# BoifZ/VDN-NeRF

Hardware: AMD Instinct MI355X
Metric: rays/sec (512-ray batch, 128 samples/ray) (higher is better)
Workload: dtype bf16; 1 GPU; training step of womsk_white (hierarchical sampling + render forward + backward + gradient all-reduce + Adam): SDF 8x256 + colour 4x256 + NeRF 8x256, 512 rays x (64 coarse + 64 importance + 32 outside) per GPU per step; pixels uniform over the full 800 x 800 frame; samples that enter the loss through exact zeros are skipped: 81 % of the foreground and 56 % of the background points evaluated; rays_per_gpu=512, samples_per_ray=128, outside_samples=32, parallelism=dp1, allreduce_bytes=5636348, background_points_evaluated_last_step=45590, background_points_total=81920, foreground_points_evaluated_last_step=52986, foreground_points_total=65536

## Files before the change

### include/vdn_render.h

```cpp
#ifndef VDN_RENDER_H
#define VDN_RENDER_H
#include <stdint.h>

#ifdef __cplusplus
extern "C" {
#endif

#define VDN_ABI_VERSION 28

int vdn_abi_version(void);

typedef struct {
    const float* g;
    const float* v;
    float* w_eff;
    float* inv_norm;
    int32_t rows, cols;
} VdnWeightNormDesc;
int vdn_weightnorm_materialize(const VdnWeightNormDesc* descs_dev, int n_layers, int max_rows, void* stream);

typedef struct {
    const float* src;
    const float* bias;
    const int32_t* kmap;
// ... 106 lines not shown
    const float* out_upper;
    const float* t_rand;
    const float* t_rand_out;
    float* z;
    float* z_out;
    int32_t B, n_samples, n_outside, z_ld;
} VdnCoarseArgs;
int vdn_coarse_z(const VdnCoarseArgs* args_host, void* stream);

typedef struct {
    const float* rays_o;
    const float* rays_d;
    const float* z;
    const float* sdf;
    const float* u;
    float* new_z;
    float inv_s;
    int32_t B, M, ld, n_imp;
    const float* weights;
    int32_t w_ld, _pad;
} VdnUpsampleArgs;
int vdn_upsample_round(const VdnUpsampleArgs* args_host, void* stream);

typedef struct {
    const float* z;
    const float* sdf;
    const float* new_z;
    const float* new_sdf;
    float* z_out;
    float* sdf_out;
    int32_t B, M, K, ld, ld_out;
} VdnMergeArgs;
int vdn_merge_sorted(const VdnMergeArgs* args_host, void* stream);
int vdn_merge_upsample(const VdnMergeArgs* merge_host, const VdnUpsampleArgs* upsample_host, void* stream);
int vdn_sdf_upsample_bf16(const VdnSdfArgs* sdf_host, const VdnUpsampleArgs* upsample_host, void* stream);
int vdn_sdf_merge_upsample_bf16(const VdnSdfArgs* sdf_host, const VdnMergeArgs* merge_host, const VdnUpsampleArgs* upsample_host, void* stream);

typedef struct {
    const float* z;
    float* dists;
    float* mid_z;
    float sample_dist;
    int32_t B, n, ld;
} VdnSectionArgs;
int vdn_sections(const VdnSectionArgs* args_host, void* stream);

typedef struct {
    const float* rays_o;
    const float* rays_d;
    const float* sdf;
    const float* normals;
    const float* dists;
    const float* mid_z;
    const float* color;
    const float* feat;
    const float* variance;
    const float* bg_density;
    const float* bg_rgb;
    const float* bg_feat;
    const float* bg_dists;
    const float* background_rgb;
    float cos_anneal_ratio;
    int32_t B, N, T, feat_ch;
    float* weights;
    float* alpha_out;
    float* cdf;
    float* inside_sphere;
    float* color_out;
    float* feat_out;
    float* weight_sum;
    float* weight_max;
    float* s_val;
    float* eik_partial;
    float* eik_out;
    const float* cos_anneal_dev;
} VdnCompositeArgs;
int vdn_alpha_composite_fwd(const VdnCompositeArgs* args_host, void* stream);
int vdn_feat_composite(const VdnCompositeArgs* args_host, void* stream);

int vdn_shade_fused_f32(const VdnSdfArgs* sdf_host, const VdnRenderNetArgs* color_host, const VdnCompositeArgs* comp_host,
                        int32_t* ticket, void* stream);
int vdn_sdf_color_train_bf16(const VdnSdfArgs* sdf_host, const void* color_blob, int32_t squeeze_out, void* col_h, void* col_small,
                             float* col_out, void* stream);
int vdn_shade_fused_bf16(const VdnSdfArgs* sdf_host, const void* color_blob, int32_t squeeze_out, const VdnCompositeArgs* comp_host,
                         int32_t* ticket, void* stream);
int vdn_shade_points_bf16(const VdnSdfArgs* sdf_host, const void* color_blob, int32_t squeeze_out, float* col_out, void* stream);

typedef struct {
    const float* rays_o;
    const float* rays_d;
    const float* mid_z;
    const float* normals;
    int32_t B, N;
    float* eik_partial;
    float* eik_out;
} VdnEikonalArgs;
int vdn_eikonal_terms(const VdnEikonalArgs* args_host, void* stream);


typedef struct {
    const char* blob;
    const float* g_out;
    const float* out;
    const void* save_h;
    void* delta_out;
    void* delta_h;
    void* d_feat;
    float* d_normals;
    int32_t acc_feat;
    int32_t acc_normals;
    int32_t P;
    int32_t d_out;
    int32_t squeeze_out;
    const int32_t* active_idx;
    const int32_t* n_active;
    const float* dirs; const float* rays_d;
    int32_t n_per_ray;
    int32_t acc_pts;
    float* d_pts;
    float* d_dirs;
    float* d_extra;
    const void* mask;
} VdnRenderNetBwdArgs;
int vdn_rendernet_bwd_f32(const VdnRenderNetBwdArgs* args_host, void* stream);
int vdn_rendernet_bwd_bf16(const VdnRenderNetBwdArgs* args_host, void* stream);

typedef struct {
    const char* blob;
    const float* g_density;
    const float* g_rgb;
    const float* g_feat;
    const void* save_h;
    const void* save_hv;
    void* delta_o;
    void* delta_v;
    void* delta_head;
    void* delta_h;
    int32_t P;
    const int32_t* active_idx;
    const int32_t* n_active;
    const float* rays_o; const float* rays_d; const float* z;
    int32_t n_per_ray;
    float* d_pts;
    float* d_dirs;
    const void* mask;
    const void* mask_v;
} VdnNerfBwdArgs;
int vdn_nerf_mlp_bwd_f32(const VdnNerfBwdArgs* args_host, void* stream);
int vdn_nerf_mlp_bwd_bf16(const VdnNerfBwdArgs* args_host, void* stream);
typedef struct {
    const float* pts4;
    const float* dirs;
    float* d_pts4;
    float* d_dirs;
    int32_t accumulate;
} VdnNerfInputGradArgs;
int vdn_nerf_mlp_bwd_input_f32(const VdnNerfBwdArgs* args_host, const VdnNerfInputGradArgs* in_host, void* stream);
int vdn_nerf_mlp_bwd_input_bf16(const VdnNerfBwdArgs* args_host, const VdnNerfInputGradArgs* in_host, void* stream);

typedef struct {
    const char* blob;
    const float* pts;
    const float* rays_o;
    const float* rays_d;
    const float* z;
    int32_t n_per_ray;
    int32_t z_ld;
    int32_t P;
    float scale;
    const float* g_normals;
    const void* S;
    const void* V;
    void* UB;
    void* EX;
    int32_t s_from_h;
    const int32_t* active_idx;
    const int32_t* n_active;
} VdnSdfRbarArgs;
int vdn_sdf_bwd_rbar_f32(const VdnSdfRbarArgs* args_host, void* stream);
int vdn_sdf_bwd_rbar_bf16(const VdnSdfRbarArgs* args_host, void* stream);

typedef struct {
    const char* blob;
    const float* g_sdf;
    const void* g_feat;
    const void* S;
    const void* EX;
    void* AB;
    int32_t P;
    float scale;
    int32_t s_from_h;
    const int32_t* active_idx;
    const int32_t* n_active;
    const float* pts; const float* rays_o; const float* rays_d; const float* z;
    int32_t n_per_ray, z_ld;
    const float* g_normals;
    const float* U_pe;
    int32_t acc_pts;
    float* d_pts;
} VdnSdfFbarArgs;
int vdn_sdf_bwd_fbar_f32(const VdnSdfFbarArgs* args_host, void* stream);
int vdn_sdf_bwd_fbar_bf16(const VdnSdfFbarArgs* args_host, void* stream);
int vdn_sdf_bwd_split_bf16(const VdnSdfRbarArgs* rbar_host, const VdnSdfFbarArgs* fbar_host, void* stream);


typedef struct {
    const void* A1; const void* B1;
    const void* A2; const void* B2;
    int32_t lda1, ldb1, lda2, ldb2;
    int32_t P;
    int32_t m_tiles, n_tiles;
    int32_t splits;
    int32_t wg_begin;
    int32_t _pad;
    float* slab;
    float* colsum;
    const int32_t* P_dev;
} VdnDwDesc;
int vdn_dw_gemm_f32(const VdnDwDesc* descs_dev, int n_desc, int total_wgs, void* stream);
int vdn_dw_gemm_bf16(const VdnDwDesc* descs_dev, int n_desc, int total_wgs, void* stream);
int vdn_dw_entry_wgs_f32(int m_tiles, int n_tiles, int splits);
int vdn_dw_entry_wgs_bf16(int m_tiles, int n_tiles, int splits);

typedef struct {
    const float* slab; const float* colsum;
    const int32_t* rmap; const int32_t* cmap;
    float* target; float* btarget;
    int64_t t_stride;
    int32_t splits, M, N;
    int32_t accumulate;
    float scale, bscale;
    const float* xsum;
    int32_t xsplits, xM, xrow;
    float xscale;
} VdnDwFinalizeDesc;
int vdn_dw_finalize(const VdnDwFinalizeDesc* descs_dev, int n_desc, int max_M, int phase, void* stream);

typedef struct {
    const float* g; const float* v; const float* inv_norm; const float* dw_eff;
    float* dg; float* dv;
    int32_t rows, cols;
} VdnWeightNormBwdDesc;
int vdn_weightnorm_bwd(const VdnWeightNormBwdDesc* descs_dev, int n_layers, int max_rows, void* stream);

typedef struct {
    const float* rays_o; const float* rays_d;
    const float* sdf; const float* normals; const float* dists; const float* mid_z;
    const float* color; const float* feat; const float* variance;
    const float* bg_density; const float* bg_rgb; const float* bg_feat; const float* bg_dists;
    const float* background_rgb;
    float cos_anneal_ratio;
    int32_t B, N, T, feat_ch;
    const float* alpha;
    const float* weights;
    const float* eik;
    const float* g_color;
    const float* g_feat;
    const float* g_weights;
    const float* g_eik;
    const float* g_cdf;
    float* d_sdf;
    float* d_normals;
    float* d_color;
    float* d_feat;
    float* d_bg_density;
    float* d_bg_rgb;
    float* d_bg_feat;
    float* d_var_partial;
    float* d_variance;
    float* d_dists;
    float* d_bg_dists;
    float* d_dir_cos;
    float* feat_scratch;
    const float* cos_anneal_dev;
} VdnCompositeBwdArgs;
int vdn_alpha_composite_bwd(const VdnCompositeBwdArgs* args_host, void* stream);

int vdn_composite_train(const VdnCompositeArgs* fwd_host, const VdnCompositeBwdArgs* bwd_host, const float* true_rgb, float* g_color,
                        const int32_t* fg_count, float igr_weight, float grad_scale, void* stream);
int vdn_eikonal_reduce(const float* eik_partial, int32_t B, float* eik_out, void* stream);
int vdn_composite_fwd_train(const VdnCompositeArgs* fwd_host, const float* gt_feats, float* g_feats, float depth_weight, float grad_scale, void* stream);
int vdn_composite_bwd_train(const VdnCompositeBwdArgs* bwd_host, const float* color_out, const float* true_rgb, float* g_color,
                            const int32_t* fg_count, float igr_weight, float grad_scale, void* stream);

typedef struct {
    const float* rays_d;
    const float* mid_z;
    const float* bg_mid;
    const float* d_pts;
    const float* d_dirs;
    const float* d_dists;
    const float* d_dir_cos;
    const float* d_bg_pts;
    const float* d_bg_dirs;
    const float* d_bg_dists;
    int32_t B, N, T;
    float* d_rays_o;
    float* d_rays_d;
    float* d_z;
    float* d_z_out;
} VdnRayAdjointArgs;
int vdn_ray_adjoint(const VdnRayAdjointArgs* args_host, void* stream);

typedef struct {
    const float* color;
    const float* true_rgb;
    const float* mask;
    const float* feats;
    const float* gt_feats;
    const float* weights;
    const float* eik;
    float igr_weight, mask_weight, depth_weight, grad_scale;
    int32_t B, T, C, _pad;
    float* g_color;
    float* g_feats;
    float* g_weights;
    float* g_eik;
    float* out_scalars;
} VdnLossArgs;
int vdn_loss_fwd_bwd(const VdnLossArgs* args_host, void* stream);

int vdn_adam_step(float* param, const float* grad, float* exp_avg, float* exp_avg_sq, int64_t n,
                  float lr, float beta1, float beta2, float eps, int32_t step, void* stream);
int vdn_adam_step_ranges(float* param, const float* grad, float* exp_avg, float* exp_avg_sq, int64_t begin0, int64_t end0,
                         int64_t begin1, int64_t end1, float lr, float beta1, float beta2, float eps, int32_t step, void* stream);

typedef struct {
    const float* pixels_x;
    const float* pixels_y;
    const float* intrinsic_inv;
    const float* pose;
    const float* image;
    const float* mask;
    const float* feats;
    float* out;
    float* near;
    float* far;
    int32_t B, H, W, C, mask_ch, out_ld;
} VdnGenRaysArgs;
int vdn_gen_rays(const VdnGenRaysArgs* args_host, void* stream);

typedef struct {
    const float* rays_o;
    const float* rays_d;
    const float* mid_z;
    int32_t B, N, T;
    int32_t* active_idx;
    int32_t* n_active;
    int32_t* ray_counts;
} VdnBackgroundActiveArgs;
int vdn_background_active(const VdnBackgroundActiveArgs* args_host, void* stream);

typedef struct {
    const float* rays_o;
    const float* rays_d;
    const float* mid_z;
    int32_t B, N;
    float radius;
    int32_t complement;
    int32_t* active_idx;
    int32_t* n_active;
    int32_t* ray_counts;
} VdnForegroundActiveArgs;

typedef struct {
    const float* rays_o; const float* rays_d;
    float* z;
    const float* new_z;
    int32_t M_old, _pad;
    const float* z_out;
    float* z_feed;
    int32_t B, N, T, z_ld;
    float sample_dist, fg_radius;
    float* dists; float* mid_z;
    float* bg_dists; float* bg_mid;
    int32_t* fg_active_idx; int32_t* fg_n_active; int32_t* fg_ray_counts;
    int32_t* bg_active_idx; int32_t* bg_n_active; int32_t* bg_ray_counts;
} VdnTrainPrepArgs;
int vdn_train_prep(const VdnTrainPrepArgs* args_host, void* stream);
int vdn_foreground_active(const VdnForegroundActiveArgs* args_host, void* stream);

typedef struct {
    const float* u;
    float threshold;
    int32_t R;
    int32_t* counts;
    const int64_t* offsets;
    float* tri_pos;
    int64_t* tri_key;
} VdnMeshArgs;
int vdn_mesh_count(const VdnMeshArgs* args_host, void* stream);
int vdn_mesh_emit(const VdnMeshArgs* args_host, void* stream);

typedef struct {
    const float* u;
    double isovalue;
    int32_t R;
    uint8_t* cube_case;
    int32_t* n_verts;
    int32_t* n_tris;
    const int64_t* vert_offsets;
    const int64_t* tri_offsets;
    double* vertices;
    int64_t* triangles;
} VdnMeshMcArgs;
int vdn_mesh_mc_count(const VdnMeshMcArgs* args_host, void* stream);
int vdn_mesh_mc_emit(const VdnMeshMcArgs* args_host, void* stream);

typedef struct {
    const float* X;
    const float* Y;
    const float* Z;
    const int32_t* active;
    float* points;
    int64_t first, n_points;
    int32_t R, brick, nb, A;
} VdnMeshSparseNodesArgs;
int vdn_mesh_sparse_nodes(const VdnMeshSparseNodesArgs* args_host, void* stream);

typedef struct {
    const float* values;
    double isovalue;
    int32_t R, brick, nb, A;
    const int32_t* active;
    const int32_t* brick_map;
    const int32_t* cell_base;
    const int32_t* col_cells;
    const int32_t* row_cells;
    int64_t n_cells;
    uint8_t* cube_case;
    int32_t* n_verts;
    int32_t* n_tris;
    int32_t* missed;
    const int64_t* vert_offsets;
    const int64_t* tri_offsets;
    int64_t V, F;
    double* vertices;
    int64_t* triangles;
} VdnMeshSparseArgs;
int vdn_mesh_sparse_count(const VdnMeshSparseArgs* args_host, void* stream);
int vdn_mesh_sparse_emit(const VdnMeshSparseArgs* args_host, void* stream);

typedef struct {
    const float* vertices;
    const void* triangles;
    double spacing;
    int64_t V, F, S;
    int32_t index_bytes, _pad;
    int32_t* counts;
    int32_t* error;
    const int64_t* offsets;
    float* points;
    int32_t* face;
} VdnSurfArgs;
int vdn_surf_count(const VdnSurfArgs* args_host, void* stream);
int vdn_surf_emit(const VdnSurfArgs* args_host, void* stream);

typedef struct {
    const float* pts;
    int32_t* cell;
// ... 289 lines not shown
```

### vdn-nerf_amd/csrc/k_composite_row.h

```cpp
#pragma once
#include "k_ray_rows.h"

namespace vdn {

struct CompositeGlobalSrc {
    const float* sdf_;
    const float* normals_;
    const float* color_;
    VDN_DEV float sdf(long q, int) const { return sdf_[q]; }
    VDN_DEV float normal(long q, int, int k) const { return normals_[q * 3 + k]; }
    VDN_DEV float color(long q, int, int k) const { return color_[q * 3 + k]; }
};
struct CompositeLdsSrc {
    const float* rows;
    int n;
    VDN_DEV float sdf(long, int i) const { return rows[i]; }
    VDN_DEV float normal(long, int i, int k) const { return rows[(1 + k) * n + i]; }
    VDN_DEV float color(long, int i, int k) const { return rows[(4 + k) * n + i]; }
};

struct RowOut { float num, den, c[3]; };
typedef RowOut EikPair;

template <class Src>
VDN_DEV RowOut composite_row(const CompositeArgs& a, int r, int lane, const Src& src) {
#pragma clang fp contract(off)
    const int N = a.N, T = a.T;
    const bool has_bg = a.bg_density != nullptr;
    float o[3], d[3];
    load_ray(a.rays_o, a.rays_d, r, o, d);
    float inv_s = expf(a.variance[0] * 10.0f);
    inv_s = fminf(fmaxf(inv_s, 1e-6f), 1e6f);
    const float car = a.cos_anneal_dev != nullptr ? a.cos_anneal_dev[0] : a.cos_anneal_ratio;

    float alpha[kEPL], f[kEPL], Tr[kEPL], wgt[kEPL], col[kEPL][3];
    double eik_num = 0.0, eik_den = 0.0;
#pragma unroll
    for (int e = 0; e < kEPL; ++e) {
        const int i = kEPL * lane + e;
        alpha[e] = 0.0f;
        f[e] = 1.0f;
        col[e][0] = col[e][1] = col[e][2] = 0.0f;
        if (i < T) {
            float bg_a = 0.0f;
            if (has_bg) {
                const long q = (long)r * T + i;
                bg_a = 1.0f - expf(-softplus1(a.bg_density[q]) * a.bg_dists[q]);
            }
            if (i < N) {
                const long q = (long)r * N + i;
                const float sdf = src.sdf(q, i), dist = a.dists[q];
                const float g0 = src.normal(q, i, 0), g1 = src.normal(q, i, 1), g2 = src.normal(q, i, 2);
                const float true_cos = d[0] * g0 + d[1] * g1 + d[2] * g2;
                const float iter_cos = -(fmaxf(-true_cos * 0.5f + 0.5f, 0.0f) * (1.0f - car) + fmaxf(-true_cos, 0.0f) * car);
                const float est_next = sdf + iter_cos * dist * 0.5f;
                const float est_prev = sdf - iter_cos * dist * 0.5f;
                const float prev_cdf = sigmoidf_(est_prev * inv_s);
                const float next_cdf = sigmoidf_(est_next * inv_s);
                float al = ((prev_cdf - next_cdf) + 1e-5f) / (prev_cdf + 1e-5f);
                al = fminf(fmaxf(al, 0.0f), 1.0f);
                const float pn = sample_norm(o, d, a.mid_z[q]);
                const float inside = pn < 1.0f ? 1.0f : 0.0f;
                eikonal_add(pn, g0, g1, g2, eik_num, eik_den);
                a.cdf[q] = prev_cdf;
                a.inside_sphere[q] = inside;
                float c0 = src.color(q, i, 0), c1 = src.color(q, i, 1), c2 = src.color(q, i, 2);
                if (has_bg) {
                    const long qb = (long)r * T + i;
                    al = al * inside + bg_a * (1.0f - inside);
                    c0 = c0 * inside + a.bg_rgb[qb * 3] * (1.0f - inside);
                    c1 = c1 * inside + a.bg_rgb[qb * 3 + 1] * (1.0f - inside);
                    c2 = c2 * inside + a.bg_rgb[qb * 3 + 2] * (1.0f - inside);
                }
                alpha[e] = al;
                col[e][0] = c0; col[e][1] = c1; col[e][2] = c2;
            } else {
                const long qb = (long)r * T + i;
                alpha[e] = bg_a;
                col[e][0] = a.bg_rgb[qb * 3]; col[e][1] = a.bg_rgb[qb * 3 + 1]; col[e][2] = a.bg_rgb[qb * 3 + 2];
            }
            f[e] = 1.0f - alpha[e] + 1e-7f;
        }
    }
    ray_excl_cumprod(f, Tr, lane);
    double ws = 0.0, c0 = 0.0, c1 = 0.0, c2 = 0.0;
    float wmax = 0.0f;
#pragma unroll
    for (int e = 0; e < kEPL; ++e) {
        const int i = kEPL * lane + e;
        wgt[e] = 0.0f;
        if (i < T) {
            wgt[e] = alpha[e] * Tr[e];
            a.weights[(long)r * T + i] = wgt[e];
            if (a.alpha_out != nullptr) a.alpha_out[(long)r * T + i] = alpha[e];
            ws += (double)wgt[e];
            c0 += (double)(col[e][0] * wgt[e]);
            c1 += (double)(col[e][1] * wgt[e]);
            c2 += (double)(col[e][2] * wgt[e]);
            wmax = fmaxf(wmax, wgt[e]);
        }
    }
    const float wsum = (float)wave_sum(ws);
    float cr = (float)wave_sum(c0), cg = (float)wave_sum(c1), cb = (float)wave_sum(c2);
    wmax = wave_max(wmax);
    eik_num = wave_sum(eik_num);
    eik_den = wave_sum(eik_den);
    if (a.background_rgb != nullptr) {
        cr = cr + a.background_rgb[0] * (1.0f - wsum);
        cg = cg + a.background_rgb[1] * (1.0f - wsum);
        cb = cb + a.background_rgb[2] * (1.0f - wsum);
    }
    if (lane == 0) {
        a.color_out[r * 3] = cr; a.color_out[r * 3 + 1] = cg; a.color_out[r * 3 + 2] = cb;
        a.weight_sum[r] = wsum;
        a.weight_max[r] = wmax;
        if (a.s_val != nullptr) a.s_val[r] = 1.0f / inv_s;
        if (a.eik_partial != nullptr) {
            a.eik_partial[r * 2] = (float)eik_num;
            a.eik_partial[r * 2 + 1] = (float)eik_den;
        }
    }
    return RowOut{(float)eik_num, (float)eik_den, {cr, cg, cb}};
}

struct FeatRaw { float fg[2], bg[2]; };
struct FeatPair { float f0, f1; };
template <class A>
VDN_DEV FeatRaw feat_load(const A& a, int r, int i, int ch0, int ch1) {
    const int N = a.N, T = a.T, C = a.feat_ch;
    const bool v0 = ch0 < C, v1 = ch1 < C;
    const bool fg = i < N, bg = i < T && (a.bg_density != nullptr || i >= N) && a.bg_feat != nullptr;
    const long qf = ((long)r * N + i) * C, qb = ((long)r * T + i) * C;
    FeatRaw v;
    v.fg[0] = (fg && v0) ? a.feat[qf + ch0] : 0.0f;
    v.fg[1] = (fg && v1) ? a.feat[qf + ch1] : 0.0f;
    v.bg[0] = (bg && v0) ? a.bg_feat[qb + ch0] : 0.0f;
    v.bg[1] = (bg && v1) ? a.bg_feat[qb + ch1] : 0.0f;
    return v;
}
template <class A>
VDN_DEV FeatPair feat_mix(const A& a, int i, const FeatRaw& v, float inside) {
#pragma clang fp contract(off)
    if (i >= a.N) return FeatPair{v.bg[0], v.bg[1]};
    if (a.bg_density == nullptr) return FeatPair{v.fg[0], v.fg[1]};
    return FeatPair{v.fg[0] * inside + v.bg[0] * (1.0f - inside), v.fg[1] * inside + v.bg[1] * (1.0f - inside)};
}
template <class A>
VDN_DEV FeatPair feat_pair(const A& a, int r, int i, int ch0, int ch1, float inside) {
    return feat_mix(a, i, feat_load(a, r, i, ch0, ch1), inside);
}
template <class A>
VDN_DEV void feat_group(const A& a, int r, int i0, int i_end, int ch0, int ch1, const float (&inside)[8], FeatPair (&f)[8]) {
    FeatRaw v[8];
#pragma unroll
    for (int k = 0; k < 8; ++k) v[k] = i0 + k < i_end ? feat_load(a, r, i0 + k, ch0, ch1) : FeatRaw{};
#pragma unroll
    for (int k = 0; k < 8; ++k) f[k] = i0 + k < i_end ? feat_mix(a, i0 + k, v[k], inside[k]) : FeatPair{};
}

inline int composite_fwd_check(const VdnCompositeArgs* a, bool need_alpha_out, bool need_eik_out, bool bwd_bg_ok = true) {
    if (!a || a->B <= 0 || a->N <= 0 || a->T < a->N || a->T > kMaxT) return -1;
    if (!a->rays_o || !a->rays_d || !a->sdf || !a->normals || !a->dists || !a->mid_z || !a->color || !a->variance) return -2;
    if (!a->weights || (need_alpha_out && !a->alpha_out) || !a->cdf || !a->inside_sphere || !a->color_out || !a->weight_sum ||
        !a->weight_max || !a->eik_partial || (need_eik_out && !a->eik_out)) return -3;
    if (a->T > a->N && (!a->bg_density || !a->bg_rgb || !a->bg_dists || !bwd_bg_ok)) return -4;
    return 0;
}
inline bool composite_feat_ok(const VdnCompositeArgs* a) { return a->feat && a->feat_ch > 0 && !(a->T > a->N && !a->bg_feat); }
inline int composite_bwd_check(const VdnCompositeBwdArgs* a, bool need_eik) {
    if (!a || a->B <= 0 || a->N <= 0 || a->T < a->N || a->T > kMaxT) return -1;
    if (!a->rays_o || !a->rays_d || !a->sdf || !a->normals || !a->dists || !a->mid_z || !a->color || !a->variance ||
        !a->alpha || !a->weights || (need_eik && !a->eik)) return -2;
    if (!a->d_sdf || !a->d_normals || !a->d_color || !a->d_var_partial) return -3;
    if (a->T > a->N && (!a->bg_density || !a->bg_rgb || !a->bg_dists || !a->d_bg_density || !a->d_bg_rgb)) return -4;
    if (a->d_feat && (!a->feat || a->feat_ch <= 0 || a->feat_ch > 128)) return -5;
    return 0;
}

}
```

### vdn-nerf_amd/csrc/k_ray_rows.h

```cpp
#pragma once
#include "vdn_common.h"
#include "vdn_kernels.h"

namespace vdn {

constexpr int kRayWaves = 4;
constexpr int kMaxT = 256;
constexpr int kEPL = 4;

VDN_DEV bool ray_of_wave(int B, int& wave, int& lane, int& r) {
    wave = threadIdx.x >> 6;
    lane = threadIdx.x & 63;
    r = blockIdx.x * kRayWaves + wave;
    return r < B;
}
__host__ __device__ inline int ray_blocks(int B) { return (B + kRayWaves - 1) / kRayWaves; }
template <class Kernel, class... Args>
inline void launch_ray_blocks(Kernel kernel, int n_blocks, void* stream, Args... args) {
    hipLaunchKernelGGL(kernel, dim3(n_blocks), dim3(kRayWaves * 64), 0, (hipStream_t)stream, args...);
}
template <class Kernel, class... Args>
inline void launch_rays(Kernel kernel, int B, void* stream, Args... args) {
    launch_ray_blocks(kernel, ray_blocks(B), stream, args...);
}
// ... 160 lines not shown
#pragma clang fp contract(off)
    const int M = a.M, K = a.K;
    for (int i = lane; i < M; i += 64) za[i] = old_src != nullptr ? old_src[i] : a.z[(long)r * a.ld + i];
    for (int j = lane; j < K; j += 64) zb[j] = a.new_z[(long)r * a.K + j];
    __builtin_amdgcn_wave_barrier();
    const bool has_sdf = a.sdf != nullptr;
    bool sorted_here = true;
    for (int i = lane; i + 1 < M; i += 64) sorted_here &= za[i] <= za[i + 1];
    const bool old_sorted = __all(sorted_here);
    float oz[kEPL], os[kEPL];
    int opos[kEPL];
#pragma unroll
    for (int e = 0; e < kEPL; ++e) {
        const int i = lane + 64 * e;
        opos[e] = -1;
        if (i < M) {
            const float v = za[i];
            int cnt = i;
            if (!old_sorted) {
                cnt = 0;
                for (int k = 0; k < M; ++k) cnt += (za[k] < v) | ((za[k] == v) & (k < i));
            }
            for (int j = 0; j < K; ++j) cnt += zb[j] < v;
            opos[e] = cnt;
            oz[e] = v;
            os[e] = has_sdf ? a.sdf[(long)r * a.ld + i] : 0.0f;
        }
    }
    float nz = 0.0f, ns = 0.0f;
    int npos = -1;
    if (lane < K) {
        const float v = zb[lane];
        int cnt = 0;
        if (old_sorted) {
            int lo = 0, hi = M;
            while (lo < hi) {
                const int mid = (lo + hi) >> 1;
                if (za[mid] <= v) lo = mid + 1; else hi = mid;
            }
            cnt = lo;
        } else {
            for (int k = 0; k < M; ++k) cnt += za[k] <= v;
        }
        for (int j = 0; j < K; ++j) cnt += (zb[j] < v) | ((zb[j] == v) & (j < lane));
        npos = cnt;
        nz = v;
        ns = has_sdf ? (new_sdf_src != nullptr ? new_sdf_src[lane] : a.new_sdf[(long)r * a.K + lane]) : 0.0f;
    }
    __builtin_amdgcn_wave_barrier();
#pragma unroll
    for (int e = 0; e < kEPL; ++e) {
        if (opos[e] >= 0) {
            a.z_out[(long)r * a.ld_out + opos[e]] = oz[e];
            if (has_sdf) a.sdf_out[(long)r * a.ld_out + opos[e]] = os[e];
            if (lz != nullptr) { lz[opos[e]] = oz[e]; ls[opos[e]] = os[e]; }
        }
    }
    if (npos >= 0) {
        a.z_out[(long)r * a.ld_out + npos] = nz;
        if (has_sdf) a.sdf_out[(long)r * a.ld_out + npos] = ns;
        if (lz != nullptr) { lz[npos] = nz; ls[npos] = ns; }
    }
}

struct Section { float dist, mid; };
VDN_DEV Section section(const float* z, int i, int n, float sample_dist) {
#pragma clang fp contract(off)
    const float z0 = z[i];
    const float dist = (i + 1 < n) ? z[i + 1] - z0 : sample_dist;
    return Section{dist, z0 + dist * 0.5f};
}

struct ActiveJob {
    const float* rays_o;
    const float* rays_d;
    const float* mid_z;
    int B, N, T;
    float radius;
    bool background;
    bool complement;
    int32_t* active_idx;
    int32_t* n_active;
    int32_t* ray_counts;
};

VDN_DEV bool sample_active(const ActiveJob& a, int r, int s, const float (&o)[3], const float (&d)[3]) {
    if (s >= a.N) return true;
    const float pn = sample_norm(o, d, a.mid_z[(long)r * a.N + s]);
    return a.background ? !(pn < 1.0f) : (pn < a.radius) != a.complement;
}

template <bool FILL>
VDN_DEV void active_list_row(const ActiveJob& a, int r, int lane, const float (&o)[3], const float (&d)[3]) {
    int base = 0;
    if (FILL) {
        int acc = 0;
        for (int i = lane; i < r; i += 64) acc += a.ray_counts[i];
        base = (int)wave_sum((double)acc);
    }
    int n = 0;
    for (int s0 = 0; s0 < a.T; s0 += 64) {
        const int s = s0 + lane;
        const bool act = s < a.T && sample_active(a, r, s, o, d);
        const unsigned long long m = __ballot(act);
        if (FILL && act) a.active_idx[base + n + __popcll(m & ((1ull << lane) - 1ull))] = r * a.T + s;
        n += __popcll(m);
    }
    if (lane == 0) {
        if (!FILL) a.ray_counts[r] = n;
        else if (r == a.B - 1) a.n_active[0] = base + n;
    }
}

}
```

### vdn-nerf_amd/csrc/k_render_bwd.h

```cpp
#pragma once
#include <type_traits>
#include "mlp_engine.h"
#include "vdn_kernels.h"

namespace vdn {

template <class P, int NT_OUT, int EX = 0, bool MASK = false>
__global__ __launch_bounds__(P::kWaves * 64, P::kMinWavesPerEU) void rendernet_bwd_kernel(RenderNetBwdArgs a) {
    using ST = typename P::store_t;
    constexpr int kSlot = P::stride(8);
    extern __shared__ __attribute__((aligned(16))) char smem[];
    WStream<P::kWaves, kSlot> ws;
    ws.init(a.blob, smem, 42 + EX);
    const int lane = ws.lane, c = lane & 31, h = lane >> 5;
    const WorkRow wr = work_row(a.active_idx, a.n_active, a.P, P::kWaves, ws.wave, c);
    if (wr.none) return;
    ws.warm_issue(wr.n_wg, 256 * P::kMinWavesPerEU);
    warm_code_issue((std::is_same<P, BF16>::value) ? kWarmCodeRenderBwd : 0, wr.n_wg, 256 * P::kMinWavesPerEU, ws.warm_dump());
    const bool ok = wr.ok;
    const long p = wr.row, pd = wr.point;
    const long PS = P::plane(a.P, 256);
    const ST* save_h = reinterpret_cast<const ST*>(a.save_h);
    ST* delta_h = reinterpret_cast<ST*>(a.delta_h);
    ST* delta_out = reinterpret_cast<ST*>(a.delta_out);
    ST* d_feat = reinterpret_cast<ST*>(a.d_feat);
    unsigned mk[MASK ? 16 : 1];
    if constexpr (MASK) {
        const unsigned char* m = static_cast<const unsigned char*>(a.mask);
        const long MS = BF16::mask_plane(a.P, 256);
#pragma unroll
        for (int l = 0; l < 4; ++l) BF16::load_mask<4>(m + l * MS, p, h, mk + 4 * l);
    }

    typename P::template Act<8> X, Y;
    if constexpr (NT_OUT == 1) {
        float dl[4];
#pragma unroll
        for (int j = 0; j < 4; ++j) {
            dl[j] = 0.0f;
            if (j < a.d_out) {
                const float o = a.out[pd * a.d_out + j], g = a.g_out[pd * a.d_out + j];
                dl[j] = a.squeeze_out ? g * o * (1.0f - o) : (o > 0.0f ? g : 0.0f);
            }
        }
        const f32x16 t16 = vals_tile<4>(dl, h, 0);
        X.set(0, t16);
        P::store_tile(delta_out, p, 32, 0, h, t16, ok);
    } else {
#pragma unroll
        for (int kt = 0; kt < 3; ++kt) {
            const f32x16 o = F32::load_tile(a.out, pd, 96, kt, h);
            const f32x16 g = F32::load_tile(a.g_out, pd, 96, kt, h);
            f32x16 dl;
#pragma unroll
            for (int t = 0; t < 16; ++t) dl[t] = a.squeeze_out ? g[t] * o[t] * (1.0f - o[t]) : (o[t] > 0.0f ? g[t] : 0.0f);
            X.set(kt, dl);
            P::store_tile(delta_out, p, 96, kt, h, dl, ok);
        }
    }
    auto ldH = [&](int l) VDN_INL { return [=](int nt) VDN_INL { return P::load_tile(save_h + l * PS, p, 256, nt, h); }; };
    auto mask_store = [&](auto& D, int l) VDN_INL {
        return [&D, l, delta_h, PS, p, ok, h](int nt, const f32x16& acc, const f32x16& hv) VDN_INL {
            f32x16 o;
#pragma unroll
            for (int t = 0; t < 16; ++t) o[t] = hv[t] > 0.0f ? acc[t] : 0.0f;
            D.set(nt, o);
            P::store_tile(delta_h + l * PS, p, 256, nt, h, o, ok);
        };
    };
    auto bit_store = [&](auto& D, int l) VDN_INL {
        return [&D, &mk, l, delta_h, PS, p, ok, h](int nt, const f32x16& acc, int) VDN_INL {
            const f32x16 o = BF16::mask_select(mk + 4 * l, nt, acc);
            D.set(nt, o);
            P::store_tile(delta_h + l * PS, p, 256, nt, h, o, ok);
        };
    };
    ws.all_issue = __any(ok);
    if constexpr (MASK) BF16::mask_landed(mk);
    warm_l2_wait();
    ws.start();
    if constexpr (MASK) {
        dense<P, NT_OUT, 8, false>(ws, X, 0, NoPre{}, bit_store(Y, 3), P::kTileOps);
        dense<P, 8, 8, false>(ws, Y, 0, NoPre{}, bit_store(X, 2), P::kTileOps);
        dense<P, 8, 8, false>(ws, X, 0, NoPre{}, bit_store(Y, 1), P::kTileOps);
        dense<P, 8, 8, false>(ws, Y, 0, NoPre{}, bit_store(X, 0), P::kTileOps);
    } else {
        dense<P, NT_OUT, 8, false, kBwdPrefetch>(ws, X, 0, ldH(3), mask_store(Y, 3), P::kTileOps, P::kTileOps);
        dense<P, 8, 8, false, kBwdPrefetch>(ws, Y, 0, ldH(2), mask_store(X, 2), P::kTileOps, P::kTileOps);
        dense<P, 8, 8, false, kBwdPrefetch>(ws, X, 0, ldH(1), mask_store(Y, 1), P::kTileOps, P::kTileOps);
        dense<P, 8, 8, false, kBwdPrefetch>(ws, Y, 0, ldH(0), mask_store(X, 0), P::kTileOps, P::kTileOps);
    }
    f32x16 SM[2];
    dense<P, 8, 10 + EX, false>(ws, X, 0, NoPre{}, [&](int nt, const f32x16& acc, int) VDN_INL {
        if (nt >= 10) {
            if constexpr (EX > 0) {
                f32x16 o = F32::load_tile(a.d_extra, pd, 32 * EX, nt - 10, h);
#pragma unroll
                for (int t = 0; t < 16; ++t) o[t] += acc[t];
                F32::store_tile(a.d_extra, pd, 32 * EX, nt - 10, h, o, ok);
            }
        } else if (nt < 8) {
            f32x16 o = acc;
            if (a.acc_feat) {
                const f32x16 prev = P::load_tile(d_feat, p, 256, nt, h);
#pragma unroll
                for (int t = 0; t < 16; ++t) o[t] += prev[t];
            }
            P::store_tile(d_feat, p, 256, nt, h, o, ok);
        } else {
            SM[nt - 8] = acc;
        }
    });
    float small[33];
    tiles_vals<33, 2>(SM, h, small);
    if (ok && h == 0) {
#pragma unroll
        for (int d = 0; d < 3; ++d) {
            const float prev = a.acc_normals ? a.d_normals[pd * 3 + d] : 0.0f;
            a.d_normals[pd * 3 + d] = prev + small[30 + d];
        }
        if (a.d_pts != nullptr) {
            const long r = pd / a.n_per_ray;
#pragma unroll
            for (int d = 0; d < 3; ++d) {
                const float dir = a.dirs ? a.dirs[pd * 3 + d] : a.rays_d[r * 3 + d];
                float g = small[3 + d];
#pragma unroll
                for (int k = 0; k < 4; ++k) {
                    const float f = (float)(1 << k);
                    float sn, co;
                    sincos_pe<P::kAccurateTrig>(dir * f, sn, co);
                    g += f * (co * small[3 + 3 + 6 * k + d] - sn * small[3 + 3 + 6 * k + 3 + d]);
                }
                const float pp = a.acc_pts ? a.d_pts[pd * 3 + d] : 0.0f;
                const float pg = a.acc_pts ? a.d_dirs[pd * 3 + d] : 0.0f;
                a.d_pts[pd * 3 + d] = pp + small[d];
                a.d_dirs[pd * 3 + d] = pg + g;
            }
        }
    }
}

template <class P>
int launch_rendernet_bwd(const VdnRenderNetBwdArgs* args, void* stream_) {
    hipStream_t stream = (hipStream_t)stream_;
    if (!args || args->P <= 0 || !args->blob || !args->g_out || !args->out || !args->save_h || !args->delta_out ||
        !args->delta_h || !args->d_feat || !args->d_normals) return -1;
    if (!(args->d_out == 96 || (args->d_out >= 1 && args->d_out <= 4))) return -2;
    if (args->d_pts && (!args->d_dirs || (!args->dirs && (!args->rays_d || args->n_per_ray <= 0)))) return -3;
    const int ppw = P::kWaves * 32;
    const int grid = (args->P + ppw - 1) / ppw;
    const size_t lds = 3 * P::stride(8);
    if (args->mask != nullptr) {
        if constexpr (std::is_same<P, BF16>::value) {
            static bool once_m = (allow_big_lds(rendernet_bwd_kernel<P, 1, 0, true>, lds), allow_big_lds(rendernet_bwd_kernel<P, 3, 0, true>, lds),
                                  allow_big_lds(rendernet_bwd_kernel<P, 1, 3, true>, lds), true);
            (void)once_m;
            if (args->d_extra != nullptr) {
                if (args->d_out == 96) return -4;
                hipLaunchKernelGGL((rendernet_bwd_kernel<P, 1, 3, true>), dim3(grid), dim3(P::kWaves * 64), lds, stream, *args);
            } else if (args->d_out == 96) {
                hipLaunchKernelGGL((rendernet_bwd_kernel<P, 3, 0, true>), dim3(grid), dim3(P::kWaves * 64), lds, stream, *args);
            } else {
                hipLaunchKernelGGL((rendernet_bwd_kernel<P, 1, 0, true>), dim3(grid), dim3(P::kWaves * 64), lds, stream, *args);
            }
            return (int)hipGetLastError();
        } else {
            return -5;
        }
    }
    static bool once = (allow_big_lds(rendernet_bwd_kernel<P, 1>, lds), allow_big_lds(rendernet_bwd_kernel<P, 3>, lds),
                        allow_big_lds(rendernet_bwd_kernel<P, 1, 3>, lds), true);
    (void)once;
    if (args->d_extra != nullptr) {
        if (args->d_out == 96) return -4;
        hipLaunchKernelGGL((rendernet_bwd_kernel<P, 1, 3>), dim3(grid), dim3(P::kWaves * 64), lds, stream, *args);
        return (int)hipGetLastError();
    }
    if (args->d_out == 96)
        hipLaunchKernelGGL((rendernet_bwd_kernel<P, 3>), dim3(grid), dim3(P::kWaves * 64), lds, stream, *args);
    else
        hipLaunchKernelGGL((rendernet_bwd_kernel<P, 1>), dim3(grid), dim3(P::kWaves * 64), lds, stream, *args);
    return (int)hipGetLastError();
}

}
```

### vdn-nerf_amd/csrc/k_sdf_fwd2.h

```cpp
#pragma once
#include <cstdlib>
#include "k_ray_rows.h"
#include "k_composite_row.h"
#include "chunk_stream.h"
#include "vdn_kernels.h"

namespace vdn {
namespace sdf2 {

#ifndef VDN_SDF2_PRE
#define VDN_SDF2_PRE 4
#endif
#ifndef VDN_SDF2_GROUP
#define VDN_SDF2_GROUP 2
#endif
#ifndef VDN_SDF2_ABL
#define VDN_SDF2_ABL 0
#endif
#ifndef VDN_SDF2_S16
#define VDN_SDF2_S16 0
#endif
constexpr bool kS16 = VDN_SDF2_S16 != 0;
#ifndef VDN_SDF2_B2
#define VDN_SDF2_B2 2
// ... 108 lines not shown
    using PG = Prog<MODE>;
    using Acc = AccT;
    static constexpr int total = PG::total, kPre = sdf2::kPre, kGroup = sdf2::kGroup, abl = VDN_SDF2_ABL;
    static constexpr int kt(int c) { return PG::kt_of(c); }
    static constexpr bool bias(int c) { return PG::bias_of(c); }
    static constexpr bool b2(int c) { return VDN_SDF2_B2 != 0 && NSLOT >= DEPTH + 2 && (VDN_SDF2_B2 != 2 || c < PG::first_chunk(PG::NL < 9 ? PG::NL : 9)); }
    static constexpr bool certifies(int c) { return !b2(c) || c % 2 == 0; }
    static constexpr int wait(int c) { return b2(c) ? wait_count_b2<MODE, SAVE>(c) : wait_count<MODE, SAVE, DEPTH>(c); }
    static constexpr bool dma_burst(int c) { return sdf2::dma_burst<MODE, SAVE>(c); }
};

#ifndef VDN_SDF2_SP
#define VDN_SDF2_SP 1
#endif
struct SpE { float g, e; };
VDN_DEV SpE softplus_sigma(float t) {
    SpE r;
#if VDN_SDF2_ABL & 1
    r.g = t; r.e = t;
    return r;
#endif
#if VDN_SDF2_SP == 1
    const float w = 1.0f + __builtin_amdgcn_exp2f(t);
    r.g = __builtin_amdgcn_fmed3f(__builtin_amdgcn_logf(w), t, 25.0f);
    r.e = __builtin_amdgcn_rcpf(w);
#else
    const float e = __builtin_amdgcn_exp2f(-fabsf(t));
    r.g = relu0(t) + __builtin_amdgcn_logf(1.0f + e);
    r.e = __builtin_amdgcn_exp2f(-r.g);
#endif
    return r;
}
typedef unsigned u32x4 __attribute__((ext_vector_type(4)));

#ifndef VDN_SDF2_WT_SAVES
#define VDN_SDF2_WT_SAVES 1
#endif
VDN_DEV void plane_store16(unsigned short* p, const u32x4& v) {
#if VDN_SDF2_WT_SAVES
#if VDN_SAVE_NT
    asm volatile("global_store_dwordx4 %0, %1, off sc1 nt\n\ts_nop 1" ::"v"(p), "v"(v) : "memory");
#else
    asm volatile("global_store_dwordx4 %0, %1, off sc1\n\ts_nop 1" ::"v"(p), "v"(v) : "memory");
#endif
#else
    *reinterpret_cast<u32x4*>(p) = v;
#endif
}

VDN_DEV unsigned sigma255_pack(float e0, float e1, float e2, float e3) {
    const unsigned d0 = __builtin_bit_cast(unsigned, __builtin_amdgcn_cvt_pknorm_u16(e0, e1));
    const unsigned d1 = __builtin_bit_cast(unsigned, __builtin_amdgcn_cvt_pknorm_u16(e2, e3));
    return ~__builtin_amdgcn_perm(d1, d0, 0x07050301u);
}
VDN_DEV float ubyte_f32(unsigned w, int b) { return (float)((w >> (8 * b)) & 0xffu); }

template <int NLDS>
struct SStore {
    static constexpr int NREG = kSTiles > NLDS ? (kSTiles - NLDS) : 0;
    u32x4 reg[NREG > 0 ? NREG : 1];
    char* lds;
    template <int T>
    VDN_DEV void put(const u32x4& v) {
        if constexpr (T < NLDS) *reinterpret_cast<u32x4*>(lds + T * 1024) = v;
        else reg[T - NLDS] = v;
    }
    template <int T>
    VDN_DEV u32x4 get() const {
        if constexpr (T < NLDS) return *reinterpret_cast<const u32x4*>(lds + T * 1024);
        else return reg[T - NLDS];
    }
};

constexpr int pair_begin(int gi, int GA) { return gi >= GA ? 8 : gi * 8 / GA; }

struct ShadeExtra {
    const char* color_blob;
    int* ticket;
    int squeeze_out;
    int warm_bytes, warm_bytes2;
    void* col_h;
    void* col_small;
    float* col_out;
    CompositeArgs cm;
};

template <int MODE, bool SAVE, int NSLOT, int DEPTH, int VID = 0, bool UPS = false>
__global__ __launch_bounds__(kWaves * 64, MODE == 0 ? 2 : 1) void sdf_fwd2_kernel(SdfArgs a, UpsampleArgs up, ShadeExtra ex) {
    static_assert(!UPS || MODE == 0, "the up-sampling round follows the sdf-only pass");
    using PG = Prog<MODE>;
    static_assert(MODE != 3 || SAVE, "MODE 3 is the training forward");
    constexpr bool TS = SAVE && (MODE == 1 || MODE == 3);
    constexpr bool FEAT = MODE == 1 || MODE == 3 || (MODE == 2 && SAVE);
    constexpr bool COL = MODE >= 2;
    using P = BF16;
    using ST = unsigned short;
    constexpr int kRing = NSLOT * kStride;
    constexpr int kW8 = 0;
    constexpr int kLdsTotal = MODE >= 1 ? 160 * 1024 : kRing + kW8;
    constexpr int NLDS = MODE >= 1 ? ((kLdsTotal - kRing - kW8) / (kWaves * 1024) < kSTiles ? (kLdsTotal - kRing - kW8) / (kWaves * 1024) : kSTiles) : 0;
    extern __shared__ __attribute__((aligned(16))) char smem[];
    using PL = StepPolicy<MODE, SAVE, NSLOT, DEPTH>;
    cstream::Pipe<kWaves, kStride, NSLOT, DEPTH, MODE >= 2 ? PG::sdf_total : cstream::kNoSplit, kPre> pp;
    pp.init(a.blob, smem, ex.color_blob);
    const int lane = pp.lane, c = lane & 31, h = lane >> 5;
    const WorkRow wr = work_row(a.active_idx, a.n_active, a.P, kWaves, pp.wave, c);
    if (wr.none) return;
    if constexpr (MODE == 1) {
        if (a.tail_max_rows > 0) {
            const long n_rows = a.active_idx != nullptr ? (long)*a.n_active : (long)a.P;
            if (n_rows > a.tail_row0 && n_rows - a.tail_row0 <= a.tail_max_rows && (long)blockIdx.x * (kWaves * 32) >= a.tail_row0) return;
        }
    }
#ifdef VDN_SDF2_STAMP
    const unsigned long long stamp_c0 = __builtin_amdgcn_s_memtime(), stamp_r0 = __builtin_amdgcn_s_memrealtime();
    unsigned long long stamp_p1 = 0, stamp_p2 = 0;
#endif
    const bool ok = wr.ok;
    const long p = wr.row, pd = wr.point;
    const int c16 = lane & 15, q4 = lane >> 4;
    (void)c16; (void)q4;

    float xin[3];
    float px[3] = {0.0f, 0.0f, 0.0f}, dir[3] = {0.0f, 0.0f, 0.0f};
    long sdf_idx = pd;
    float z_keep = 0.0f, sdf_keep = 0.0f;
    if (a.pts != nullptr) {
#pragma unroll
        for (int d = 0; d < 3; ++d) xin[d] = a.pts[pd * 3 + d] * a.scale;
        if constexpr (MODE == 4) {
#pragma unroll
            for (int d = 0; d < 3; ++d) px[d] = a.pts[pd * 3 + d];
        }
    } else {
        const long r = pd / a.n_per_ray;
        const long sidx = pd - r * a.n_per_ray;
        const float z = a.z[r * a.z_ld + sidx];
        z_keep = z;
        sdf_idx = r * a.sdf_ld + sidx;
#pragma unroll
        for (int d = 0; d < 3; ++d) xin[d] = (a.rays_o[r * 3 + d] + a.rays_d[r * 3 + d] * z) * a.scale;
        if constexpr (COL) {
#pragma unroll
            for (int d = 0; d < 3; ++d) {
                dir[d] = a.rays_d[r * 3 + d];
                px[d] = a.rays_o[r * 3 + d] + a.rays_d[r * 3 + d] * z;
            }
        }
    }
    ST* Hs = reinterpret_cast<ST*>(a.H);
    ST* Vs = reinterpret_cast<ST*>(a.V);
    ST* feat = reinterpret_cast<ST*>(a.feat);
    const long PS = P::plane(a.P, 256);
    const long prow = (p >> 5) * (32L * 256) + h * 256 + (p & 31) * 8;
    long prow2[2] = {0, 0};
    if constexpr (kS16) {
        const long n_rows = a.active_idx != nullptr ? (long)*a.n_active : (long)a.P;
#pragma unroll
        for (int ph = 0; ph < 2; ++ph) {
            const long raw = ((long)blockIdx.x * kWaves + pp.wave) * 32 + 16 * ph + c16;
            const long r = raw < n_rows ? raw : (n_rows > 0 ? n_rows - 1 : 0);
            prow2[ph] = (r >> 5) * (32L * 256) + (q4 >> 1) * 512 + (q4 & 1) * 256 + (r & 31) * 8;
        }
    }
    auto piece = [&](int T, int k) VDN_INL -> long { return kS16 ? prow2[k] + T * 1024 : prow + T * 1024 + 512 * k; };
    const float inv_scale = 1.0f / a.scale;
    asm volatile("s_waitcnt vmcnt(0)" ::: "memory");
    char* const wdump = pp.warm_dump();
    warm_l2_issue(a.blob, ex.warm_bytes, wr.n_wg, MODE == 0 ? 512 : 256, wdump);
    warm_l2_issue(COL ? ex.color_blob : nullptr, COL ? ex.warm_bytes2 : 0, wr.n_wg, 256, wdump);
    constexpr int kCode = MODE == 0 ? kWarmCodeSdfFwd2Mode0 : (MODE == 1 ? (SAVE ? kWarmCodeSdfFwd2Save : kWarmCodeSdfFwd2) : (MODE == 3 ? kWarmCodeSdfFwd3 : 0));
    warm_code_issue(ex.warm_bytes > 0 ? kCode : 0, wr.n_wg, MODE == 0 ? 512 : 256, wdump);

    typename P::template Act<9> X, Y;
    typename P::template Act<9> F;
    float nz = 0.0f;
    float col[3] = {0.0f, 0.0f, 0.0f};
    SStore<NLDS> SS;
    SS.lds = smem + kRing + kW8 + pp.wave * (NLDS * 1024) + lane * 16;
    static_assert(!kS16 || MODE == 0 || NLDS * 1024 >= 32 * 272, "exchange scratch");
    static_assert(!kS16 || NSLOT - 1 >= DEPTH, "the last ring slot is free at the start");
    char* const xch = MODE >= 1 ? smem + kRing + kW8 + pp.wave * (NLDS * 1024) : smem + (NSLOT - 1) * kStride + pp.wave * 4096;
    auto to_tile_lanes = [&](bf16x8* fr, auto nf_c) VDN_INL {
        constexpr int NF = decltype(nf_c)::value;
#pragma unroll
        for (int s = 0; s < NF; ++s) *reinterpret_cast<bf16x8*>(xch + s * 1024 + lane * 16) = fr[s];
        asm volatile("s_waitcnt lgkmcnt(0)" ::: "memory");
#pragma unroll
        for (int s = 0; s < NF; ++s)
            fr[s] = *reinterpret_cast<const bf16x8*>(xch + ((s & ~1) + (q4 >> 1)) * 1024 + (q4 & 1) * 512 + (16 * (s & 1) + c16) * 16);
        asm volatile("s_waitcnt lgkmcnt(0)" ::: "memory");
    };

    bf16x8 pe7[2];
    {
        float pe39[39], pe[64];
        posenc<3, 6, false>(xin, pe39);
#pragma unroll
        for (int i = 0; i < 39; ++i) pe[i] = pe39[i] * kC1;
#pragma unroll
        for (int i = 0; i < 25; ++i) pe[39 + i] = fmaf(pe39[i], kC1, -bf16_lo(pack_bf16x2(pe[i], 0.0f)));
#pragma unroll
// ... 114 lines not shown
                                u32x4 o;
                                o[0] = fhold0;
                                o[1] = fhold1;
                                o[2] = pack_bf16x2(acc_prev[4 * q], acc_prev[4 * q + 1]);
                                o[3] = pack_bf16x2(acc_prev[4 * q + 2], acc_prev[4 * q + 3]);
                                if constexpr (FEAT) plane_store16(feat + piece(T, q >> 1), o);
                                if constexpr (COL) F.r[T * 2 + (q >> 1)] = __builtin_bit_cast(bf16x8, o);
                            }
                            const f32x4 w = *(reinterpret_cast<const f32x4*>(pp.template slot<CP + 1>() + kTail) + (8 * T + quad_of(q, lane)));
                            if constexpr (q == 0) sq_v7 = SS.template get<PG::s_tile0(7) + T>();
                            const unsigned sw = sq_v7[q];
                            const float v0 = w[0] * inv_scale * ubyte_f32(sw, 0), v1 = w[1] * inv_scale * ubyte_f32(sw, 1);
                            const float v2 = w[2] * inv_scale * ubyte_f32(sw, 2), v3 = w[3] * inv_scale * ubyte_f32(sw, 3);
                            u32x4 cur = __builtin_bit_cast(u32x4, Y.r[T * 2 + (q >> 1)]);
                            unsigned k0 = pack_bf16x2(v0, v1), k1 = pack_bf16x2(v2, v3);
                            asm volatile("" : "+v"(k0), "+v"(k1));
                            cur[2 * (q & 1)] = k0;
                            cur[2 * (q & 1) + 1] = k1;
                            Y.r[T * 2 + (q >> 1)] = __builtin_bit_cast(bf16x8, cur);
                            if constexpr (TS) {
                                if constexpr ((q & 1) == 0) {
                                    vhold0 = pack_bf16x2(v0 * kVSave, v1 * kVSave);
                                    vhold1 = pack_bf16x2(v2 * kVSave, v3 * kVSave);
                                    asm volatile("" : "+v"(vhold0), "+v"(vhold1));
                                } else {
                                    u32x4 ov;
                                    ov[0] = vhold0;
                                    ov[1] = vhold1;
                                    ov[2] = pack_bf16x2(v0 * kVSave, v1 * kVSave);
                                    ov[3] = pack_bf16x2(v2 * kVSave, v3 * kVSave);
                                    plane_store16(Vs + 7 * PS + piece(T, q >> 1), ov);
                                }
                            }
                        }
                    });
                }
            } else if constexpr (L.kind == SWEEP || (L.kind == SWEEP_SKIP && T < 7)) {
                static_for<PE_ - PB>([&](auto i_c) VDN_INL {
                    constexpr int pr = PB + decltype(i_c)::value;
                    const float v0 = acc_prev[2 * pr] * ubyte_f32(sq_prev[pr >> 1], 2 * (pr & 1));
                    const float v1 = acc_prev[2 * pr + 1] * ubyte_f32(sq_prev[pr >> 1], 2 * (pr & 1) + 1);
                    unsigned pk = pack_bf16x2(v0, v1);
                    asm volatile("" : "+v"(pk));
                    u32x4 cur = __builtin_bit_cast(u32x4, D.r[T * 2 + (pr >> 2)]);
                    cur[pr & 3] = pk;
                    D.r[T * 2 + (pr >> 2)] = __builtin_bit_cast(bf16x8, cur);
                    if constexpr (TS) {
                        unsigned pv = pack_bf16x2(v0 * kVSave, v1 * kVSave);
                        if constexpr ((pr & 3) == 0) {
                            vhold0 = pv;
                            asm volatile("" : "+v"(vhold0));
                        } else if constexpr ((pr & 3) == 1) {
                            vhold1 = pv;
                            asm volatile("" : "+v"(vhold1));
                        } else if constexpr ((pr & 3) == 2) {
                            hold0 = pv;
                            asm volatile("" : "+v"(hold0));
                        } else {
                            u32x4 o;
                            o[0] = vhold0;
                            o[1] = vhold1;
                            o[2] = hold0;
                            o[3] = pv;
                            plane_store16(Vs + L.l * PS + piece(T, pr >> 2), o);
                        }
                    }
                });
            } else if constexpr (L.kind == COL0 || L.kind == COLH) {
                static_for<PE_ - PB>([&](auto i_c) VDN_INL {
                    constexpr int pr = PB + decltype(i_c)::value;
                    float a0 = acc_prev[2 * pr], a1 = acc_prev[2 * pr + 1];
                    if constexpr (L.kind == COL0) {
                        if constexpr ((pr & 1) == 0) w8hold = *(reinterpret_cast<const f32x4*>(pp.template slot<CP + 1>() + kTail) + (8 * T + quad_of(pr >> 1, lane)));
                        const float nzp = kS16 ? nz2[ph_of_pair(pr)] : nz;
                        a0 = fmaf(w8hold[2 * (pr & 1)], nzp, a0);
                        a1 = fmaf(w8hold[2 * (pr & 1) + 1], nzp, a1);
                    }
                    unsigned pk = pack_bf16x2(relu0(a0), relu0(a1));
                    asm volatile("" : "+v"(pk));
                    u32x4 cur = __builtin_bit_cast(u32x4, D.r[T * 2 + (pr >> 2)]);
                    cur[pr & 3] = pk;
                    D.r[T * 2 + (pr >> 2)] = __builtin_bit_cast(bf16x8, cur);
                    if constexpr (MODE == 3 && (pr & 3) == 3)
                        plane_store16(reinterpret_cast<ST*>(ex.col_h) + L.l * PS + piece(T, pr >> 2), cur);
                });
            } else if constexpr (L.kind == COLOUT) {
                if constexpr (PB == 0) {
                    if constexpr (kS16) {
#pragma unroll
                        for (int j = 0; j < 3; ++j) {
                            const float lo = acc_prev[j], hi = __shfl(acc_prev[8 + j], lane & 15);
                            const float x = (lane & 16) ? hi : lo;
                            col[j] = ex.squeeze_out ? sigmoidf_(x) : relu0(x);
                        }
                    } else {
#pragma unroll
                        for (int j = 0; j < 3; ++j) col[j] = ex.squeeze_out ? sigmoidf_(acc_prev[j]) : relu0(acc_prev[j]);
                    }
                }
            }
        }
    };

    static_for<PG::total + 1>([&](auto c_c) VDN_INL {
        constexpr int C = decltype(c_c)::value;
        constexpr int CP = C - 1;
        constexpr int CPs = CP >= 0 ? CP : 0;
        if constexpr (C < PG::total) {
            constexpr int LI = PG::layer_of(C), T = PG::tile_of(C);
            constexpr LayerDesc L = PG::layer(LI);
            constexpr int NS = 2 * L.kt, NG = (NS + kGroup - 1) / kGroup;
#ifdef VDN_SDF2_STAMP
            if constexpr (C == PG::first_chunk(8)) stamp_p1 = __builtin_amdgcn_s_memtime();
            if constexpr (MODE == 1 && C == PG::first_chunk(MODE == 1 ? 9 : 8)) stamp_p2 = __builtin_amdgcn_s_memtime();
#endif
            constexpr bool boundary = CP >= 0 && PG::layer_of(CPs) != LI;
            constexpr int KP = PG::layer(PG::layer_of(CPs)).kind;
            constexpr bool prev_writes_input = boundary && (KP == HID || KP == SWEEP || KP == COL0 || KP == COLH);
            constexpr int GA = prev_writes_input ? ((2 * PG::tile_of(CPs)) / kGroup < NG ? (2 * PG::tile_of(CPs)) / kGroup : NG) : NG;
            static_assert(GA >= 1, "a pending tile needs at least one MFMA group before its reader");
            if constexpr (L.kind == HID && L.l == 4 && T == 0) { X.r[14] = pe7[0]; X.r[15] = pe7[1]; }
            constexpr bool sweep_tile = L.kind == SWEEP || (L.kind == SWEEP_SKIP && T < 7);
            u32x4 sq_next;
            if constexpr (sweep_tile) sq_next = SS.template get<PG::s_tile0(L.l) + T>();
            const auto& Xin = L.kind == COL0 ? F : ((LI & 1) ? Y : X);
            const AccT acc_cur = cstream::chunk_step<PL, C>(pp, Xin, [&](auto g_c, auto) VDN_INL {
                constexpr int gi = decltype(g_c)::value;
                epilogue(std::integral_constant<int, CP>{}, std::integral_constant<int, pair_begin(gi, GA)>{},
                         std::integral_constant<int, pair_begin(gi + 1, GA)>{});
            });
            if constexpr (L.kind == SWEEP_SKIP && T >= 7) UPE[T - 7] = acc_cur;
            if constexpr (L.kind == SWEEP_PE) {
                if constexpr (kS16) UPE[T].add(acc_cur);
                else UPE[T] = acc_cur;
            }
            if constexpr (L.kind == LAST && T == L.nt - 1) {
                const float b0 = *reinterpret_cast<const float*>(pp.template slot<C>() + L.kt * 2048);
                float dot;
                if constexpr (kS16) {
                    float d0 = sdf_dot[0], d1 = sdf_dot[1];
                    d0 += __shfl_xor(d0, 16); d1 += __shfl_xor(d1, 16);
                    d0 += __shfl_xor(d0, 32); d1 += __shfl_xor(d1, 32);
                    dot = (lane & 16) ? d1 : d0;
                } else {
                    dot = sdf_dot[0] + __shfl_xor(sdf_dot[0], 32);
                }
                sdf_keep = fmaf(dot, 1.0f / kC1, b0) * inv_scale;
                if (ok && h == 0) a.sdf[sdf_idx] = sdf_keep;
            }
            acc_prev = acc_cur;
            if constexpr (sweep_tile) sq_prev = sq_next;
            if constexpr ((!kS16 && L.kind == SWEEP_SKIP && T == 8) || (L.kind == SWEEP_PE && T == 1)) pe_backward(kS16 || L.kind == SWEEP_SKIP);
            if constexpr (COL && L.kind == SWEEP_PE && T == 1) {
                float small[32], pe[27];
                if constexpr (MODE == 4) {
                    const float gx = n[0] * a.scale, gy = n[1] * a.scale, gz = n[2] * a.scale;
                    const float inv = -1.0f / fmaxf(sqrtf(gx * gx + gy * gy + gz * gz), 1e-12f);
                    dir[0] = gx * inv;
                    dir[1] = gy * inv;
                    dir[2] = gz * inv;
                }
                posenc<3, 4, P::kAccurateTrig>(dir, pe);
#pragma unroll
                for (int d = 0; d < 3; ++d) small[d] = px[d];
#pragma unroll
                for (int i = 0; i < 27; ++i) small[3 + i] = pe[i];
                small[30] = n[0] * a.scale;
                small[31] = n[1] * a.scale;
                nz = n[2] * a.scale;
                F.set(8, vals_tile<32>(small, h, 0));
                if constexpr (kS16) {
                    to_tile_lanes(&F.r[16], std::integral_constant<int, 2>{});
                    reinterpret_cast<float*>(xch)[c] = nz;
                    asm volatile("s_waitcnt lgkmcnt(0)" ::: "memory");
                    nz2[0] = reinterpret_cast<const float*>(xch)[c16];
                    nz2[1] = reinterpret_cast<const float*>(xch)[16 + c16];
                    asm volatile("s_waitcnt lgkmcnt(0)" ::: "memory");
                }
                if constexpr (MODE == 3) {
                    float s33[33];
#pragma unroll
                    for (int i = 0; i < 32; ++i) s33[i] = small[i];
                    s33[32] = nz;
#pragma unroll
                    for (int kt = 0; kt < 2; ++kt) P::store_tile(reinterpret_cast<ST*>(ex.col_small), p, 64, kt, h, vals_tile<33>(s33, h, kt), true);
                }
            }
        } else {
            epilogue(std::integral_constant<int, CP>{}, std::integral_constant<int, 0>{}, std::integral_constant<int, 8>{});
        }
        __builtin_amdgcn_sched_barrier(0);
    });
    if constexpr (MODE >= 1) {
        if (ok && h == 0) {
#pragma unroll
            for (int d = 0; d < 3; ++d) a.normals[pd * 3 + d] = n[d] * a.scale;
            if constexpr (MODE == 3 || MODE == 4) {
#pragma unroll
                for (int d = 0; d < 3; ++d) ex.col_out[pd * 3 + d] = col[d];
            }
        }
    }
    if constexpr (MODE == 2) {
        asm volatile("s_waitcnt lgkmcnt(0)" ::: "memory");
        __builtin_amdgcn_s_barrier();
        float* rows = reinterpret_cast<float*>(smem);
        if (h == 0) {
            const int i = pp.wave * 32 + c;
            rows[i] = sdf_keep;
#pragma unroll
            for (int d = 0; d < 3; ++d) {
                rows[(1 + d) * 128 + i] = n[d] * a.scale;
                rows[(4 + d) * 128 + i] = col[d];
            }
        }
        asm volatile("s_waitcnt lgkmcnt(0)" ::: "memory");
        __builtin_amdgcn_s_barrier();
        if (pp.wave != 0) return;
        const int ray = blockIdx.x;
        CompositeArgs cm = ex.cm;
        float* eik_partial = cm.eik_partial;
        cm.eik_partial = nullptr;
        const EikPair ep = composite_row(cm, ray, lane, CompositeLdsSrc{rows, 128});
        int old = 0;
        if (lane == 0) {
            typedef float f32x2 __attribute__((ext_vector_type(2)));
            const f32x2 pv = {ep.num, ep.den};
            asm volatile("global_store_dwordx2 %0, %1, off sc1\n\ts_waitcnt vmcnt(0)" ::"v"(eik_partial + 2 * ray), "v"(pv) : "memory");
            old = __hip_atomic_fetch_add(ex.ticket, 1, __ATOMIC_RELAXED, __HIP_MEMORY_SCOPE_AGENT);
        }
        old = __builtin_amdgcn_readfirstlane(old);
        if (old == cm.B - 1) {
            double sn = 0.0, sd = 0.0;
            for (int i = lane; i < cm.B; i += 64) {
                typedef float f32x2 __attribute__((ext_vector_type(2)));
                f32x2 v;
                asm volatile("global_load_dwordx2 %0, %1, off sc1\n\ts_waitcnt vmcnt(0)" : "=v"(v) : "v"(eik_partial + 2 * i) : "memory");
                sn += (double)v[0];
                sd += (double)v[1];
            }
            sn = wave_sum(sn);
            sd = wave_sum(sd);
            if (lane == 0) {
                cm.eik_out[0] = (float)sn / ((float)sd + 1e-5f);
                cm.eik_out[1] = (float)sn;
                cm.eik_out[2] = (float)sd;
                __hip_atomic_store(ex.ticket, 0, __ATOMIC_RELAXED, __HIP_MEMORY_SCOPE_AGENT);
            }
        }
    }
    if constexpr (UPS) {
        asm volatile("s_waitcnt lgkmcnt(0)" ::: "memory");
        __builtin_amdgcn_s_barrier();
        float* rows = reinterpret_cast<float*>(smem) + (pp.wave >> 1) * 3 * kMaxT;
        if (h == 0) {
            rows[(pp.wave & 1) * 32 + c] = z_keep;
            rows[kMaxT + (pp.wave & 1) * 32 + c] = sdf_keep;
        }
        asm volatile("s_waitcnt lgkmcnt(0)" ::: "memory");
        __builtin_amdgcn_s_barrier();
        const int r = blockIdx.x * 2 + (pp.wave >> 1);
        if ((pp.wave & 1) == 0 && r < up.B) upsample_row(up, r, lane, 64, rows, rows + kMaxT, rows + 2 * kMaxT);
    }
#ifdef VDN_SDF2_STAMP
    if (threadIdx.x == 0 && a.PE != nullptr) {
        unsigned long long* o = reinterpret_cast<unsigned long long*>(a.PE) + 8 * blockIdx.x;
        o[0] = stamp_c0; o[1] = __builtin_amdgcn_s_memtime(); o[2] = stamp_r0; o[3] = __builtin_amdgcn_s_memrealtime();
        o[4] = stamp_p1; o[5] = stamp_p2;
    }
#endif
}

template <int MODE, bool SAVE, int NSLOT, int DEPTH, int VID = 0, bool UPS = false>
int launch(const VdnSdfArgs* args, hipStream_t stream, const VdnUpsampleArgs* up = nullptr, const ShadeExtra* ex = nullptr) {
    constexpr size_t lds_min = MODE >= 1 ? 160 * 1024 : NSLOT * kStride;
    static bool once = (allow_big_lds(sdf_fwd2_kernel<MODE, SAVE, NSLOT, DEPTH, VID, UPS>, lds_min), true);
    (void)once;
    const int grid = (args->P + kWaves * 32 - 1) / (kWaves * 32);
    const size_t lds = lds_min;
    static const bool warm = [] { const char* e = getenv("VDN_SDF2_WARM"); return e == nullptr || e[0] != '0'; }();
    ShadeExtra exv = ex != nullptr ? *ex : ShadeExtra{};
    const bool cold = (SAVE && (MODE == 1 || MODE == 3)) || args->cold_start != 0;
// ... 10 lines not shown
```

### vdn-nerf_amd/csrc/rays.hip

```cpp
#include "k_ray_rows.h"
#include "k_composite_row.h"
#include "k_pixel_gather.h"
#include "k_loss_grad.h"

namespace vdn {

__global__ void coarse_z_kernel(CoarseArgs a) {
    const int idx = blockIdx.x * blockDim.x + threadIdx.x;
    const int per = a.n_samples + a.n_outside;
    if (idx >= a.B * per) return;
    const int r = idx / per, j = idx % per;
    const float nearv = a.near[r], farv = a.far[r];
    if (j < a.n_samples) {
        float z = nearv + (farv - nearv) * a.lin_samples[j];
        if (a.t_rand != nullptr) z = z + (a.t_rand[r] - 0.5f) * 2.0f / (float)a.n_samples;
        a.z[(long)r * a.z_ld + j] = z;
    } else {
        const int k = j - a.n_samples;
        const int kk = a.n_outside - 1 - k;
        float zo;
        if (a.t_rand_out != nullptr)
            zo = a.out_lower[kk] + (a.out_upper[kk] - a.out_lower[kk]) * a.t_rand_out[(long)r * a.n_outside + kk];
        else
            zo = a.lin_outside[kk];
// ... 156 lines not shown
#pragma unroll
    for (int r = 0; r < 3; ++r) v[r] = p[r] / nrm;
#pragma unroll
    for (int r = 0; r < 3; ++r) d[r] = a.pose[r * 4 + 0] * v[0] + a.pose[r * 4 + 1] * v[1] + a.pose[r * 4 + 2] * v[2];
    float* o = a.out + (long)i * a.out_ld;
    float org[3];
#pragma unroll
    for (int r = 0; r < 3; ++r) {
        org[r] = a.pose[r * 4 + 3];
        o[r] = org[r];
        o[3 + r] = d[r];
    }
    gather_pixel_row(a, x, y, o);
    if (a.near != nullptr && a.far != nullptr) {
        const float mid = sphere_mid(org, d);
        a.near[i] = mid - 1.0f;
        a.far[i] = mid + 1.0f;
    }
}

}

using namespace vdn;

extern "C" int vdn_gen_rays(const VdnGenRaysArgs* a, void* stream) {
    if (!a || a->B <= 0 || !a->pixels_x || !a->pixels_y || !a->intrinsic_inv || !a->pose || !a->out) return -1;
    if (a->out_ld < 6 || a->H <= 0 || a->W <= 0) return -2;
    if (a->feats && (a->C <= 0 || a->out_ld < 10 + a->C)) return -3;
    if (a->mask && a->mask_ch <= 0) return -4;
    hipLaunchKernelGGL(gen_rays_kernel, dim3((a->B + 255) / 256), dim3(256), 0, (hipStream_t)stream, *a);
    return (int)hipGetLastError();
}

extern "C" int vdn_coarse_z(const VdnCoarseArgs* a, void* stream) {
    if (!a || a->B <= 0 || !a->near || !a->far || !a->z || !a->lin_samples) return -1;
    if (a->n_outside > 0 && (!a->z_out || !a->lin_outside)) return -2;
    if (a->t_rand_out && (!a->out_lower || !a->out_upper)) return -3;
    const int n = a->B * (a->n_samples + a->n_outside);
    hipLaunchKernelGGL(coarse_z_kernel, dim3((n + 255) / 256), dim3(256), 0, (hipStream_t)stream, *a);
    return (int)hipGetLastError();
}

extern "C" int vdn_upsample_round(const VdnUpsampleArgs* a, void* stream) {
    if (!a || a->B <= 0 || !a->z || !a->new_z || !a->u) return -1;
    if (a->weights == nullptr ? (!a->sdf || !a->rays_o || !a->rays_d) : a->w_ld < a->M - 1) return -1;
    if (a->M < 2 || a->M > kMaxT || a->n_imp < 1 || a->n_imp > 64 || a->ld < a->M) return -2;
    launch_rays(upsample_kernel, a->B, stream, *a);
    return (int)hipGetLastError();
}

extern "C" int vdn_merge_sorted(const VdnMergeArgs* a, void* stream) {
    if (!a || a->B <= 0 || !a->z || !a->new_z || !a->z_out) return -1;
    if (a->M < 1 || a->K < 1 || a->K > 64 || a->M + a->K > kMaxT || a->ld < a->M || a->ld_out < a->M + a->K) return -2;
    if (a->sdf && (!a->new_sdf || !a->sdf_out)) return -3;
    launch_rays(merge_kernel, a->B, stream, *a);
    return (int)hipGetLastError();
}

template <bool FILL>
__global__ __launch_bounds__(kRayWaves * 64) void active_list_kernel(ActiveJob a) {
    int wave, lane, r;
    if (!ray_of_wave(a.B, wave, lane, r)) return;
    float o[3], d[3];
    load_ray(a.rays_o, a.rays_d, r, o, d);
    active_list_row<FILL>(a, r, lane, o, d);
}

static int launch_active(const ActiveJob& j, void* stream) {
    launch_rays(active_list_kernel<false>, j.B, stream, j);
    launch_rays(active_list_kernel<true>, j.B, stream, j);
    return (int)hipGetLastError();
}

extern "C" int vdn_background_active(const VdnBackgroundActiveArgs* a, void* stream) {
    if (!a || a->B <= 0 || a->N < 0 || a->T < a->N || !a->rays_o || !a->rays_d || (a->N > 0 && !a->mid_z) ||
        !a->active_idx || !a->n_active || !a->ray_counts) return -1;
    const ActiveJob j = {a->rays_o, a->rays_d, a->mid_z, a->B, a->N, a->T, 1.0f, true, false, a->active_idx, a->n_active, a->ray_counts};
    return launch_active(j, stream);
}

extern "C" int vdn_foreground_active(const VdnForegroundActiveArgs* a, void* stream) {
    if (!a || a->B <= 0 || a->N <= 0 || !a->rays_o || !a->rays_d || !a->mid_z || !(a->radius > 0.0f) ||
        !a->active_idx || !a->n_active || !a->ray_counts) return -1;
    const ActiveJob j = {a->rays_o, a->rays_d, a->mid_z, a->B, a->N, a->N, a->radius, false, a->complement != 0, a->active_idx, a->n_active, a->ray_counts};
    return launch_active(j, stream);
}

template <int PASS>
__global__ __launch_bounds__(kRayWaves * 64) void train_prep_kernel(TrainPrepArgs a) {
    const int wave = threadIdx.x >> 6, lane = threadIdx.x & 63;
    const int nb = ray_blocks(a.B);
    const bool second = PASS == 1 && (int)blockIdx.x >= nb;
    const int r = ((int)blockIdx.x - (second ? nb : 0)) * kRayWaves + wave;
    if (r >= a.B) return;
    float o[3], d[3];
    load_ray(a.rays_o, a.rays_d, r, o, d);
    if (PASS == 0) {
        __shared__ float s_a[kRayWaves][kMaxT], s_b[kRayWaves][kMaxT], s_f[kRayWaves][kMaxT], s_x[kRayWaves][kMaxT], s_z[kRayWaves][kMaxT];
        const float* final_z = nullptr;
        if (a.new_z != nullptr) {
            MergeArgs m1 = {};
            m1.z = a.z; m1.new_z = a.new_z; m1.z_out = a.z;
            m1.B = a.B; m1.M = a.M_old; m1.K = a.N - a.M_old; m1.ld = a.z_ld; m1.ld_out = a.z_ld;
            merge_row(m1, r, lane, s_a[wave], s_b[wave], s_z[wave], s_x[wave]);
            __builtin_amdgcn_wave_barrier();
            final_z = s_z[wave];
        }
        MergeArgs m = {};
        m.z = a.z; m.new_z = a.z_out; m.z_out = a.z_feed;
        m.B = a.B; m.M = a.N; m.K = a.T - a.N; m.ld = a.z_ld; m.ld_out = a.T;
        merge_row(m, r, lane, s_a[wave], s_b[wave], s_f[wave], s_x[wave], final_z);
        __builtin_amdgcn_wave_barrier();
        const float* zi = s_a[wave];
        const float* zf = s_f[wave];
        for (int i = lane; i < a.N; i += 64) {
            const Section sc = section(zi, i, a.N, a.sample_dist);
            a.dists[(long)r * a.N + i] = sc.dist;
            a.mid_z[(long)r * a.N + i] = sc.mid;
        }
        for (int i = lane; i < a.T; i += 64) {
            const Section sc = section(zf, i, a.T, a.sample_dist);
            a.bg_dists[(long)r * a.T + i] = sc.dist;
            a.bg_mid[(long)r * a.T + i] = sc.mid;
        }
        __builtin_amdgcn_s_waitcnt(0);
        __builtin_amdgcn_wave_barrier();
    }
    if (a.fg_active_idx != nullptr && !second)
        active_list_row<PASS == 1>(ActiveJob{a.rays_o, a.rays_d, a.mid_z, a.B, a.N, a.N, a.fg_radius, false, false, a.fg_active_idx, a.fg_n_active, a.fg_ray_counts},
                                   r, lane, o, d);
    if (PASS == 0 || second)
        active_list_row<PASS == 1>(ActiveJob{a.rays_o, a.rays_d, a.mid_z, a.B, a.N, a.T, 1.0f, true, false, a.bg_active_idx, a.bg_n_active, a.bg_ray_counts},
                                   r, lane, o, d);
}

extern "C" int vdn_train_prep(const VdnTrainPrepArgs* a, void* stream) {
    if (!a || a->B <= 0 || a->N <= 0 || a->T <= a->N || a->T > kMaxT || a->z_ld < a->N) return -1;
    if (!a->rays_o || !a->rays_d || !a->z || !a->z_out || !a->z_feed || !a->dists || !a->mid_z || !a->bg_dists || !a->bg_mid) return -2;
    if (a->T - a->N > 64) return -2;
    if (a->new_z && (a->M_old < 1 || a->M_old >= a->N || a->N - a->M_old > 64)) return -2;
    if (!a->bg_active_idx || !a->bg_n_active || !a->bg_ray_counts) return -3;
    if (a->fg_active_idx && (!a->fg_n_active || !a->fg_ray_counts || !(a->fg_radius > 0.0f))) return -4;
    launch_rays(train_prep_kernel<0>, a->B, stream, *a);
    launch_ray_blocks(train_prep_kernel<1>, 2 * ray_blocks(a->B), stream, *a);
    return (int)hipGetLastError();
}

extern "C" int vdn_merge_upsample(const VdnMergeArgs* m, const VdnUpsampleArgs* u, void* stream) {
    if (!m || !u || m->B <= 0 || !m->z || !m->new_z || !m->z_out || !m->sdf || !m->new_sdf || !m->sdf_out) return -1;
    if (m->M < 1 || m->K < 1 || m->K > 64 || m->M + m->K > kMaxT || m->ld < m->M || m->ld_out < m->M + m->K) return -2;
    if (u->B != m->B || u->M != m->M + m->K || u->weights || !u->rays_o || !u->rays_d || !u->u || !u->new_z ||
        u->n_imp < 1 || u->n_imp > 64) return -3;
    launch_rays(merge_upsample_kernel, m->B, stream, *m, *u);
    return (int)hipGetLastError();
}

extern "C" int vdn_sections(const VdnSectionArgs* a, void* stream) {
    if (!a || a->B <= 0 || a->n <= 0 || !a->z || !a->dists || !a->mid_z || a->ld < a->n) return -1;
    const int n = a->B * a->n;
    hipLaunchKernelGGL(sections_kernel, dim3((n + 255) / 256), dim3(256), 0, (hipStream_t)stream, *a);
    return (int)hipGetLastError();
}

extern "C" int vdn_eikonal_terms(const VdnEikonalArgs* a, void* stream) {
    if (!a || a->B <= 0 || a->N <= 0 || a->N > kMaxT) return -1;
    if (!a->rays_o || !a->rays_d || !a->mid_z || !a->normals || !a->eik_partial || !a->eik_out) return -2;
    launch_rays(eikonal_terms_kernel, a->B, stream, *a);
    hipLaunchKernelGGL(eikonal_reduce_kernel, dim3(1), dim3(64), 0, (hipStream_t)stream, a->eik_partial, a->B, a->eik_out);
    return (int)hipGetLastError();
}

extern "C" int vdn_eikonal_reduce(const float* eik_partial, int32_t B, float* eik_out, void* stream) {
    if (!eik_partial || !eik_out || B <= 0) return -1;
    hipLaunchKernelGGL(eikonal_reduce_kernel, dim3(1), dim3(64), 0, (hipStream_t)stream, eik_partial, B, eik_out);
    return (int)hipGetLastError();
}

extern "C" int vdn_feat_composite(const VdnCompositeArgs* a, void* stream) {
    if (!a || a->B <= 0 || a->N <= 0 || a->T < a->N || a->T > kMaxT) return -1;
    if (!a->feat || !a->feat_out || a->feat_ch <= 0 || !a->weights || !a->inside_sphere) return -2;
    if (a->T > a->N && (!a->bg_density || !a->bg_feat)) return -3;
    hipLaunchKernelGGL(feat_composite_kernel, dim3(a->B), dim3(256), 0, (hipStream_t)stream, *a, FeatLoss{});
    return (int)hipGetLastError();
}

extern "C" int vdn_composite_fwd_train(const VdnCompositeArgs* a, const float* gt_feats, float* g_feats, float depth_weight, float grad_scale,
                                       void* stream) {
    if (!gt_feats || !g_feats) return -1;
    if (const int err = composite_fwd_check(a, false, false)) return err;
    if (!a->feat_out || !composite_feat_ok(a)) return -5;
    launch_rays(composite_kernel, a->B, stream, *a);
    hipLaunchKernelGGL(feat_composite_kernel, dim3(a->B), dim3(256), 0, (hipStream_t)stream, *a, FeatLoss{gt_feats, g_feats, depth_weight, grad_scale});
    return (int)hipGetLastError();
}

extern "C" int vdn_alpha_composite_fwd(const VdnCompositeArgs* a, void* stream) {
    if (const int err = composite_fwd_check(a, false, true)) return err;
    if (a->feat_out && !composite_feat_ok(a)) return -5;
    launch_rays(composite_kernel, a->B, stream, *a);
    if (a->feat_out != nullptr)
        hipLaunchKernelGGL(feat_composite_kernel, dim3(a->B), dim3(256), 0, (hipStream_t)stream, *a, FeatLoss{});
    hipLaunchKernelGGL(eikonal_reduce_kernel, dim3(1), dim3(64), 0, (hipStream_t)stream, a->eik_partial, a->B, a->eik_out);
    return (int)hipGetLastError();
}
```

### vdn-nerf_amd/csrc/train_dw_bf16.hip

```cpp
#include "mlp_engine.h"
#include "vdn_kernels.h"

namespace vdn {

constexpr int kDwTileBytes = 2048;
constexpr int kDwStageBytes = 16 * kDwTileBytes;
#ifndef VDN_DW_BUF
#define VDN_DW_BUF 4
#endif
constexpr int kDwBuf = VDN_DW_BUF;
constexpr int kDwWaves = 8;

typedef short s16x4 __attribute__((ext_vector_type(4)));
typedef __attribute__((address_space(3))) char lds_char;
typedef __attribute__((address_space(3))) s16x4 lds_s16x4;

VDN_DEV const char* dw_uniform(const char* p) {
    const unsigned long long v = (unsigned long long)p;
    const unsigned lo = __builtin_amdgcn_readfirstlane((unsigned)v), hi = __builtin_amdgcn_readfirstlane((unsigned)(v >> 32));
    return (const char*)(((unsigned long long)hi << 32) | lo);
}

VDN_DEV void dw_glds16(const char* base_uniform, unsigned lane_off, unsigned lds_wave_base) {
#if VDN_DW_LD_NT == 2
    asm volatile("s_mov_b32 m0, %1\n\ts_nop 0\n\tglobal_load_lds_dwordx4 %0, %2 sc1 nt" ::"v"(lane_off), "s"(lds_wave_base), "s"(base_uniform) : "memory", "m0");
#elif VDN_DW_LD_NT
    asm volatile("s_mov_b32 m0, %1\n\ts_nop 0\n\tglobal_load_lds_dwordx4 %0, %2 nt" ::"v"(lane_off), "s"(lds_wave_base), "s"(base_uniform) : "memory", "m0");
#else
    asm volatile("s_mov_b32 m0, %1\n\ts_nop 0\n\tglobal_load_lds_dwordx4 %0, %2" ::"v"(lane_off), "s"(lds_wave_base), "s"(base_uniform) : "memory", "m0");
#endif
}

VDN_DEV void dw_wait_vm(int n) {
    switch (n) {
        case 0: asm volatile("s_waitcnt vmcnt(0)" ::: "memory"); break;
        case 1: asm volatile("s_waitcnt vmcnt(1)" ::: "memory"); break;
        case 2: asm volatile("s_waitcnt vmcnt(2)" ::: "memory"); break;
        case 3: asm volatile("s_waitcnt vmcnt(3)" ::: "memory"); break;
        case 4: asm volatile("s_waitcnt vmcnt(4)" ::: "memory"); break;
        case 6: asm volatile("s_waitcnt vmcnt(6)" ::: "memory"); break;
        case 8: asm volatile("s_waitcnt vmcnt(8)" ::: "memory"); break;
        case 9: asm volatile("s_waitcnt vmcnt(9)" ::: "memory"); break;
        case 12: asm volatile("s_waitcnt vmcnt(12)" ::: "memory"); break;
        default: asm volatile("s_waitcnt vmcnt(0)" ::: "memory"); break;
    }
}

VDN_DEV bf16x8 dw_frag(const lds_char* p) {
    const s16x4 lo = __builtin_amdgcn_ds_read_tr16_b64_v4i16((lds_s16x4*)(p));
    const s16x4 hi = __builtin_amdgcn_ds_read_tr16_b64_v4i16((lds_s16x4*)(p + 256));
    return bf16x8{lo[0], lo[1], lo[2], lo[3], hi[0], hi[1], hi[2], hi[3]};
}

VDN_DEV int dw_uni(int v) { return __builtin_amdgcn_readfirstlane(v); }

__global__ __launch_bounds__(512, 1) void dw_gemm_bf16_kernel(const DwDesc* descs, int n_desc) {
    extern __shared__ __attribute__((aligned(16))) char smem[];
    const int wg = blockIdx.x;
    int di = 0;
    while (di + 1 < n_desc && descs[di + 1].wg_begin <= wg) ++di;
    const DwDesc& d = descs[dw_uni(di)];
    const int m_tiles = dw_uni(d.m_tiles), n_tiles = dw_uni(d.n_tiles), splits = dw_uni(d.splits);
    const int local = wg - dw_uni(d.wg_begin);
    const int mg = (m_tiles + 7) / 8, ng = max((n_tiles + 7) / 8, 1);
    const int split = local / (mg * ng), blk = local % (mg * ng);
    if (split >= splits) return;
    const int tm = blk / ng, tn = blk % ng;
    const int wave = dw_uni(threadIdx.x >> 6), lane = threadIdx.x & 63, c = lane & 31, h = lane >> 5;
    const int wm = wave >> 1, wn = wave & 1;
    const int a_t0 = tm * 8, b_t0 = tn * 8;
    const int nA = min(8, m_tiles - a_t0), nB = max(0, min(8, n_tiles - b_t0));
    const bool two = d.A2 != nullptr;
    const int seg_splits = two ? splits / 2 : splits;
    const bool seg2 = two && split >= seg_splits;
    const int s_in = seg2 ? split - seg_splits : split;
    int P = dw_uni(d.P);
    if (d.P_dev != nullptr) P = min(P, dw_uni(*d.P_dev));
    int per = (P + seg_splits - 1) / seg_splits;
    per = (per + 127) / 128 * 128;
    const int k_begin = s_in * per, k_end = min(k_begin + per, P);
    const char* A = dw_uniform(reinterpret_cast<const char*>(seg2 ? d.A2 : d.A1));
    const char* Bm = dw_uniform(reinterpret_cast<const char*>(seg2 ? d.B2 : d.B1));
    const long lda = dw_uni(seg2 ? d.lda2 : d.lda1), ldb = dw_uni(seg2 ? d.ldb2 : d.ldb1);
    const int n_stages = k_end > k_begin ? (k_end - k_begin + 31) >> 5 : 0;
    float* slab = d.slab;
    float* colsum = d.colsum;

    const int n_pieces = 2 * (nA + nB);
    const int npw = (n_pieces - wave + kDwWaves - 1) / kDwWaves;
    const unsigned lane_off = ((lane >> 3) & 1) * 1024 + ((lane >> 2) & 1) * 512 + ((lane >> 4) * 4 + (lane & 3)) * 16;
    const unsigned lds0 = (unsigned)(size_t)(lds_char*)smem;
    auto issue_stage = [&](int s) VDN_INL {
        const long blk32 = (k_begin >> 5) + s;
        const unsigned buf = lds0 + (s % kDwBuf) * kDwStageBytes;
#pragma unroll
        for (int i = 0; i < 4; ++i) {
            const int u = wave + i * kDwWaves;
            if (u < n_pieces) {
                const int t = u >> 1, half = u & 1;
                const bool isA = t < nA;
                const char* src = isA ? A + blk32 * (64 * lda) + (long)(a_t0 + t) * 2048
                                      : Bm + blk32 * (64 * ldb) + (long)(b_t0 + t - nA) * 2048;
                const int slot = isA ? t : 8 + (t - nA);
                dw_glds16(src + half * 256, lane_off, buf + slot * kDwTileBytes + half * 1024);
            }
        }
    };

    const int gi = lane & 15, qp = gi >> 2, pp = gi & 3, jj = (lane >> 4) & 1;
    const unsigned frag_off = (2 * h) * 256 + (jj * 8 + (pp & 1) * 4 + qp) * 16 + (pp >> 1) * 8;
    const lds_char* lbase = (lds_char*)smem + frag_off;

    f32x16 acc[2][4];
    f32x16 cs[2];
#pragma unroll
    for (int i = 0; i < 2; ++i) {
        cs[i] = f32x16{0};
#pragma unroll
        for (int j = 0; j < 4; ++j) acc[i][j] = f32x16{0};
    }
    const bool do_colsum = colsum != nullptr && tn == 0 && wn == 0 && !seg2;
    const int mvm = (2 * wm < nA ? 1 : 0) | (2 * wm + 1 < nA ? 2 : 0);
    const int nvm = (4 * wn < nB ? 1 : 0) | (4 * wn + 1 < nB ? 2 : 0) | (4 * wn + 2 < nB ? 4 : 0) | (4 * wn + 3 < nB ? 8 : 0);
    const bf16x8 ones = {0x3F80, 0x3F80, 0x3F80, 0x3F80, 0x3F80, 0x3F80, 0x3F80, 0x3F80};

    auto run = [&](auto full_c) VDN_INL {
        constexpr bool FULL = decltype(full_c)::value;
#pragma unroll
        for (int s = 0; s < kDwBuf - 1; ++s)
            if (s < n_stages) issue_stage(s);
        for (int s = 0; s < n_stages; ++s) {
            const int later = min(n_stages - 1 - s, kDwBuf - 2);
            dw_wait_vm(npw * later);
            asm volatile("s_barrier" ::: "memory");
            if (s + kDwBuf - 1 < n_stages) issue_stage(s + kDwBuf - 1);
            if (s == n_stages - 1 && (k_end & 31)) {
                const int valid = k_end & 31;
                char* buf = smem + (s % kDwBuf) * kDwStageBytes;
                for (int u = threadIdx.x; u < 16 * 256; u += 512) {
                    const int pt = ((u >> 5) & 7) * 4 + ((u >> 1) & 3);
                    if (pt >= valid) *reinterpret_cast<unsigned long long*>(buf + u * 8) = 0ull;
                }
                __syncthreads();
            }
            const lds_char* st = lbase + (s % kDwBuf) * kDwStageBytes;
#pragma unroll
            for (int ks = 0; ks < 2; ++ks) {
                bf16x8 a[2], b[4];
#pragma unroll
                for (int i = 0; i < 2; ++i)
                    if (FULL || (mvm >> i & 1)) a[i] = dw_frag(st + (2 * wm + i) * kDwTileBytes + ks * 1024);
#pragma unroll
                for (int j = 0; j < 4; ++j)
                    if (FULL || (nvm >> j & 1)) b[j] = dw_frag(st + (8 + 4 * wn + j) * kDwTileBytes + ks * 1024);
#pragma unroll
                for (int i = 0; i < 2; ++i) {
                    if (!FULL && !(mvm >> i & 1)) continue;
#pragma unroll
                    for (int j = 0; j < 4; ++j)
                        if (FULL || (nvm >> j & 1)) acc[i][j] = __builtin_amdgcn_mfma_f32_32x32x16_bf16(a[i], b[j], acc[i][j], 0, 0, 0);
                    if (do_colsum) cs[i] = __builtin_amdgcn_mfma_f32_32x32x16_bf16(a[i], ones, cs[i], 0, 0, 0);
                }
            }
        }
    };
    if (mvm == 3 && nvm == 15) run(std::true_type{});
    else run(std::false_type{});

    const int M = m_tiles * 32, N = n_tiles * 32;
#pragma unroll
    for (int i = 0; i < 2; ++i) {
        if (!(mvm >> i & 1)) continue;
        const int mt = a_t0 + 2 * wm + i;
#pragma unroll
        for (int j = 0; j < 4; ++j) {
            if (!(nvm >> j & 1)) continue;
            float* base = slab + ((long)split * M + mt * 32) * N + (b_t0 + 4 * wn + j) * 32 + c;
#pragma unroll
            for (int t = 0; t < 16; ++t) base[(long)rho(t, h) * N] = acc[i][j][t];
        }
        if (colsum != nullptr && tn == 0 && wn == 0 && c == 0) {
#pragma unroll
            for (int t = 0; t < 16; ++t) colsum[(long)split * M + mt * 32 + rho(t, h)] = cs[i][t];
        }
    }
}

}

extern "C" int vdn_dw_entry_wgs_bf16(int m_tiles, int n_tiles, int splits) {
    const int mg = (m_tiles + 7) / 8, ng = n_tiles > 0 ? (n_tiles + 7) / 8 : 1;
    return splits * mg * ng;
}

extern "C" int vdn_dw_gemm_bf16(const VdnDwDesc* descs_dev, int n_desc, int total_wgs, void* stream) {
    using namespace vdn;
    if (!descs_dev || n_desc <= 0 || total_wgs <= 0) return -1;
    static bool once = (allow_big_lds(dw_gemm_bf16_kernel, kDwBuf * kDwStageBytes), true);
    (void)once;
    hipLaunchKernelGGL(dw_gemm_bf16_kernel, dim3(total_wgs), dim3(512), kDwBuf * kDwStageBytes, (hipStream_t)stream, descs_dev, n_desc);
    return (int)hipGetLastError();
}
```

### vdn-nerf_amd/csrc/train_dw_f32.hip

```cpp
#include "vdn_common.h"
#include "vdn_kernels.h"

namespace vdn {

constexpr int kF32StagePts = 32;
constexpr int kF32PanelBytes = kF32StagePts * 128 * 4;

__global__ __launch_bounds__(256, 2) void dw_gemm_f32_kernel(const DwDesc* descs, int n_desc) {
    extern __shared__ __attribute__((aligned(16))) char smem[];
    const int wg = blockIdx.x;
    int di = 0;
    while (di + 1 < n_desc && descs[di + 1].wg_begin <= wg) ++di;
    const DwDesc d = descs[di];
    const int local = wg - d.wg_begin;
    const int mt4 = (d.m_tiles + 3) / 4, nt4 = max((d.n_tiles + 3) / 4, 1);
    const int ntile = mt4 * nt4;
    const int slot = local & 7, round = local >> 3;
    const int split = slot + 8 * (round / ntile);
    const int tile = round % ntile;
    if (split >= d.splits) return;
    const int tm = tile / nt4, tn = tile % nt4;
    const int wave = threadIdx.x >> 6, lane = threadIdx.x & 63, c = lane & 31, h = lane >> 5;
    const int wm = wave >> 1, wn = wave & 1;
    const int m0 = tm * 4 + wm * 2, n0 = tn * 4 + wn * 2;
    const bool mv0 = m0 < d.m_tiles, mv1 = m0 + 1 < d.m_tiles;
    const bool nv0 = n0 < d.n_tiles, nv1 = n0 + 1 < d.n_tiles;
    const bool two = d.A2 != nullptr;
    const int seg_splits = two ? d.splits / 2 : d.splits;
    const bool seg2 = two && split >= seg_splits;
    const int s_in = seg2 ? split - seg_splits : split;
    const long P = d.P_dev != nullptr ? min((long)d.P, (long)*d.P_dev) : (long)d.P;
    long per = (P + seg_splits - 1) / seg_splits;
    per = (per + kF32StagePts - 1) / kF32StagePts * kF32StagePts;
    const long k_begin = (long)s_in * per, k_end = min(k_begin + per, P);
    const float* A = reinterpret_cast<const float*>(seg2 ? d.A2 : d.A1);
    const float* Bm = reinterpret_cast<const float*>(seg2 ? d.B2 : d.B1);
    const int lda = seg2 ? d.lda2 : d.lda1, ldb = seg2 ? d.ldb2 : d.ldb1;

    const bool load_b = wave >= 2;
    const float* src = load_b ? Bm : A;
    const int ld = load_b ? ldb : lda;
    const int ncols = (load_b ? d.n_tiles : d.m_tiles) * 32;
    int col = (load_b ? tn : tm) * 128 + c * 4;
    if (col >= ncols) col = 0;
    const bool have_src = src != nullptr && ncols > 0;
    auto issue = [&](long kbase, int buf) VDN_INL {
        if (!have_src) return;
        char* dst = smem + buf * 2 * kF32PanelBytes + (load_b ? kF32PanelBytes : 0);
#pragma unroll
        for (int i = 0; i < 8; ++i) {
            const int r0 = (wave & 1) * 16 + 2 * i;
            const long row = min(kbase + r0 + h, P - 1);
            glds16(src + row * ld + col, dst + r0 * 512);
        }
    };
    f32x16 acc00 = {0}, acc01 = {0}, acc10 = {0}, acc11 = {0};
    float cs0 = 0.0f, cs1 = 0.0f;
    const bool do_colsum = d.colsum != nullptr && tn == 0 && wn == 0 && !seg2;
    const long n_stages = (k_end - k_begin + kF32StagePts - 1) / kF32StagePts;
    if (n_stages > 0) issue(k_begin, 0);
    for (long t = 0; t < n_stages; ++t) {
        asm volatile("s_waitcnt vmcnt(0)" ::: "memory");
        __syncthreads();
        if (t + 1 < n_stages) issue(k_begin + (t + 1) * kF32StagePts, (t + 1) & 1);
        const float* pa = reinterpret_cast<const float*>(smem + (t & 1) * 2 * kF32PanelBytes);
        const float* pb = pa + kF32PanelBytes / 4;
        const long kb = k_begin + t * kF32StagePts;
#pragma unroll
        for (int ks = 0; ks < kF32StagePts / 2; ++ks) {
            const int r = 2 * ks + h;
            const bool valid = kb + r < k_end;
            float a0 = pa[r * 128 + wm * 64 + c], a1 = pa[r * 128 + wm * 64 + 32 + c];
            float b0 = pb[r * 128 + wn * 64 + c], b1 = pb[r * 128 + wn * 64 + 32 + c];
            if (!valid) { a0 = 0.0f; a1 = 0.0f; b0 = 0.0f; b1 = 0.0f; }
            if (do_colsum) {
                cs0 += a0;
                cs1 += a1;
            }
            if (nv0) {
                acc00 = __builtin_amdgcn_mfma_f32_32x32x2f32(a0, b0, acc00, 0, 0, 0);
                acc10 = __builtin_amdgcn_mfma_f32_32x32x2f32(a1, b0, acc10, 0, 0, 0);
            }
            if (nv1) {
                acc01 = __builtin_amdgcn_mfma_f32_32x32x2f32(a0, b1, acc01, 0, 0, 0);
                acc11 = __builtin_amdgcn_mfma_f32_32x32x2f32(a1, b1, acc11, 0, 0, 0);
            }
        }
    }
    const int M = d.m_tiles * 32, N = d.n_tiles * 32;
    auto put = [&](const f32x16& acc, int mt, int nt) {
        float* base = d.slab + ((long)split * M + mt * 32) * N + nt * 32 + c;
#pragma unroll
        for (int t = 0; t < 16; ++t) base[(long)rho(t, h) * N] = acc[t];
    };
    if (mv0 && nv0) put(acc00, m0, n0);
    if (mv0 && nv1) put(acc01, m0, n0 + 1);
    if (mv1 && nv0) put(acc10, m0 + 1, n0);
    if (mv1 && nv1) put(acc11, m0 + 1, n0 + 1);
    if (d.colsum != nullptr && tn == 0 && wn == 0) {
        cs0 += __shfl_xor(cs0, 32);
        cs1 += __shfl_xor(cs1, 32);
        if (h == 0) {
            if (mv0) d.colsum[(long)split * M + m0 * 32 + c] = cs0;
            if (mv1) d.colsum[(long)split * M + (m0 + 1) * 32 + c] = cs1;
        }
    }
}

__global__ __launch_bounds__(256) void dw_finalize_kernel(const DwFinalizeDesc* descs, int phase) {
    const DwFinalizeDesc d = descs[blockIdx.x];
    if (d.accumulate != phase) return;
    const int i = blockIdx.y * 4 + (threadIdx.x >> 6);
    if (i >= d.M) return;
    const int r = d.rmap[i];
    if (r < 0) return;
    const int lane = threadIdx.x & 63;
    if (d.target != nullptr) {
        const long step = (long)d.M * d.N;
        for (int j = 4 * lane; j < d.N; j += 256) {
            const float* col = d.slab + (long)i * d.N + j;
            f32x4 v[8];
#pragma unroll
            for (int k = 0; k < 8; ++k) v[k] = f32x4{0.0f, 0.0f, 0.0f, 0.0f};
            int s = 0;
            for (; s + 8 <= d.splits; s += 8) {
#pragma unroll
                for (int k = 0; k < 8; ++k) v[k] += *reinterpret_cast<const f32x4*>(col + (s + k) * step);
            }
#pragma unroll
            for (int k = 0; k < 8; ++k)
                if (s + k < d.splits) v[k] += *reinterpret_cast<const f32x4*>(col + (s + k) * step);
            const f32x4 t4 = ((v[0] + v[1]) + (v[2] + v[3])) + ((v[4] + v[5]) + (v[6] + v[7]));
#pragma unroll
            for (int e = 0; e < 4; ++e) {
                const int cc = d.cmap[j + e];
                if (cc < 0) continue;
                float val = d.scale * t4[e];
                if (d.xsum != nullptr && r == d.xrow) {
                    float x = 0.0f;
                    for (int s2 = 0; s2 < d.xsplits; ++s2) x += d.xsum[(long)s2 * d.xM + cc];
                    val += d.xscale * x;
                }
                float* t = d.target + (long)r * d.t_stride + cc;
                *t = d.accumulate ? *t + val : val;
            }
        }
    }
    if (d.btarget != nullptr) {
        float v = 0.0f;
        for (int s = lane; s < d.splits; s += 64) v += d.colsum[(long)s * d.M + i];
#pragma unroll
        for (int off = 32; off > 0; off >>= 1) v += __shfl_xor(v, off);
        if (lane == 0) {
            float* t = d.btarget + r;
            *t = d.accumulate ? *t + d.bscale * v : d.bscale * v;
        }
    }
}

__global__ void weightnorm_bwd_kernel(const WeightNormBwdDesc* descs) {
    const WeightNormBwdDesc d = descs[blockIdx.x];
    const int row = blockIdx.y * 4 + (threadIdx.x >> 6);
    const int lane = threadIdx.x & 63;
    if (row >= d.rows) return;
    const float* v = d.v + (long)row * d.cols;
    const float* dw = d.dw_eff + (long)row * d.cols;
    float dot = 0.0f;
    for (int c = lane; c < d.cols; c += 64) dot += dw[c] * v[c];
#pragma unroll
    for (int off = 32; off > 0; off >>= 1) dot += __shfl_xor(dot, off);
    const float inv = d.inv_norm[row], g = d.g[row];
    float* dv = d.dv + (long)row * d.cols;
    const float k1 = g * inv, k2 = dot * inv * inv;
    for (int c = lane; c < d.cols; c += 64) dv[c] = k1 * (dw[c] - k2 * v[c]);
    if (lane == 0) d.dg[row] = dot * inv;
}

}

extern "C" int vdn_dw_entry_wgs_f32(int m_tiles, int n_tiles, int splits) {
    const int mt4 = (m_tiles + 3) / 4, nt4 = n_tiles > 0 ? (n_tiles + 3) / 4 : 1;
    return 8 * ((splits + 7) / 8) * mt4 * nt4;
}

extern "C" int vdn_dw_gemm_f32(const VdnDwDesc* descs_dev, int n_desc, int total_wgs, void* stream) {
    if (!descs_dev || n_desc <= 0 || total_wgs <= 0) return -1;
    static bool once = (vdn::allow_big_lds(vdn::dw_gemm_f32_kernel, 4 * vdn::kF32PanelBytes), true);
    (void)once;
    hipLaunchKernelGGL(vdn::dw_gemm_f32_kernel, dim3(total_wgs), dim3(256), 4 * vdn::kF32PanelBytes, (hipStream_t)stream, descs_dev, n_desc);
    return (int)hipGetLastError();
}

extern "C" int vdn_dw_finalize(const VdnDwFinalizeDesc* descs_dev, int n_desc, int max_M, int phase, void* stream) {
    if (!descs_dev || n_desc <= 0 || max_M <= 0 || phase < 0 || phase > 1) return -1;
    hipLaunchKernelGGL(vdn::dw_finalize_kernel, dim3(n_desc, (max_M + 3) / 4), dim3(256), 0, (hipStream_t)stream, descs_dev, phase);
    return (int)hipGetLastError();
}

extern "C" int vdn_weightnorm_bwd(const VdnWeightNormBwdDesc* descs_dev, int n_layers, int max_rows, void* stream) {
    if (!descs_dev || n_layers <= 0 || max_rows <= 0) return -1;
    hipLaunchKernelGGL(vdn::weightnorm_bwd_kernel, dim3(n_layers, (max_rows + 3) / 4), dim3(256), 0, (hipStream_t)stream, descs_dev);
    return (int)hipGetLastError();
}
```

### vdn-nerf_amd/csrc/train_rays.hip

```cpp
#include "vdn_common.h"
#include "vdn_kernels.h"
#include "k_composite_row.h"
#include "k_loss_grad.h"

namespace vdn {

__global__ __launch_bounds__(256) void feat_dot_kernel(CompositeBwdArgs a) {
    const int lane = threadIdx.x & 63;
    const long row = (long)blockIdx.x * 4 + (threadIdx.x >> 6);
    const int N = a.N, T = a.T, C = a.feat_ch;
    if (row >= (long)a.B * T) return;
    const int r = (int)(row / T), i = (int)(row - (long)r * T);
    float inside = 0.0f;
    if (i < N && a.bg_density != nullptr) {
        float o[3], d[3];
        load_ray(a.rays_o, a.rays_d, r, o, d);
        inside = sample_norm(o, d, a.mid_z[(long)r * N + i]) < 1.0f ? 1.0f : 0.0f;
    }
    const FeatPair v = feat_pair(a, r, i, lane, lane + 64, inside);
    float part = 0.0f;
    if (lane < C) part += a.g_feat[(long)r * C + lane] * v.f0;
    if (lane + 64 < C) part += a.g_feat[(long)r * C + lane + 64] * v.f1;
#pragma unroll
    for (int off = 32; off > 0; off >>= 1) part += __shfl_xor(part, off);
// ... 13 lines not shown
        const long q = (long)r * N + i;
        const float c = cf[q];
        if (lane < C) a.d_feat[q * C + lane] = c * g0;
        if (lane + 64 < C) a.d_feat[q * C + lane + 64] = c * g1;
    }
    if (a.bg_density != nullptr && a.d_bg_feat != nullptr) {
        const float c = cb[row];
        if (lane < C) a.d_bg_feat[row * C + lane] = c * g0;
        if (lane + 64 < C) a.d_bg_feat[row * C + lane + 64] = c * g1;
    }
}

struct CompositeBwdOvr {
    bool on;
    float gc[3], g_eik, eik_den;
};

VDN_DEV void composite_bwd_row(const CompositeBwdArgs& a, int r, int wave, int lane, const CompositeBwdOvr& ov) {
    const int N = a.N, T = a.T, C = a.feat_ch;
    const bool has_bg = a.bg_density != nullptr;
    const bool has_feat = a.d_feat != nullptr && a.g_feat != nullptr;
    float o[3], d[3], gc[3] = {0.0f, 0.0f, 0.0f};
    load_ray(a.rays_o, a.rays_d, r, o, d);
#pragma unroll
    for (int k = 0; k < 3; ++k) {
        if (ov.on) gc[k] = ov.gc[k];
        else if (a.g_color != nullptr) gc[k] = a.g_color[r * 3 + k];
    }
    const float var = a.variance[0];
    const float inv_s_raw = expf(var * 10.0f);
    const float inv_s = fminf(fmaxf(inv_s_raw, 1e-6f), 1e6f);
    const bool s_unclipped = inv_s_raw >= 1e-6f && inv_s_raw <= 1e6f;
    const float car = a.cos_anneal_dev != nullptr ? a.cos_anneal_dev[0] : a.cos_anneal_ratio;
    const float g_eik = ov.on ? ov.g_eik : (a.g_eik != nullptr ? a.g_eik[0] : 0.0f);
    const float eik_den = ov.on ? ov.eik_den : a.eik[2] + 1e-5f;
    float bgc[3] = {0.0f, 0.0f, 0.0f};
    if (a.background_rgb != nullptr) {
        bgc[0] = a.background_rgb[0]; bgc[1] = a.background_rgb[1]; bgc[2] = a.background_rgb[2];
    }

    __shared__ float s_fd[kRayWaves][kMaxT], s_cf[kRayWaves][kMaxT], s_cb[kRayWaves][kMaxT];
    float gfa = 0.0f, gfb = 0.0f;
    const bool ext_feat = has_feat && a.feat_scratch != nullptr;
    if (ext_feat) {
        for (int i = lane; i < T; i += 64) s_fd[wave][i] = a.feat_scratch[(long)r * T + i];
        __builtin_amdgcn_wave_barrier();
    } else if (has_feat) {
        if (lane < C) gfa = a.g_feat[(long)r * C + lane];
        if (lane + 64 < C) gfb = a.g_feat[(long)r * C + lane + 64];
        for (int i0 = 0; i0 < T; i0 += 8) {
            float insd[8];
            FeatPair v[8];
#pragma unroll
            for (int k = 0; k < 8; ++k) insd[k] = i0 + k < N ? (sample_norm(o, d, a.mid_z[(long)r * N + i0 + k]) < 1.0f ? 1.0f : 0.0f) : 0.0f;
            feat_group(a, r, i0, T, lane, lane + 64, insd, v);
#pragma unroll
            for (int k = 0; k < 8; ++k) {
                const int i = i0 + k;
                if (i >= T) break;
                float part = gfa * v[k].f0 + gfb * v[k].f1;
#pragma unroll
                for (int off = 32; off > 0; off >>= 1) part += __shfl_xor(part, off);
                if (lane == 0) s_fd[wave][i] = part;
            }
        }
        __builtin_amdgcn_wave_barrier();
    }
    float alpha[kEPL], w[kEPL], f[kEPL], Tr[kEPL], Wb[kEPL], ins[kEPL], pn[kEPL];
#pragma unroll
    for (int e = 0; e < kEPL; ++e) {
        const int i = kEPL * lane + e;
        alpha[e] = 0.0f; w[e] = 0.0f; f[e] = 1.0f; Wb[e] = 0.0f; ins[e] = 0.0f; pn[e] = 0.0f;
        if (i < T) {
            const long qt = (long)r * T + i;
            alpha[e] = a.alpha[qt];
            w[e] = a.weights[qt];
            f[e] = 1.0f - alpha[e] + 1e-7f;
            float c0, c1, c2;
            float inside = 0.0f;
            if (i < N) {
                const long q = (long)r * N + i;
                pn[e] = sample_norm(o, d, a.mid_z[q]);
                inside = pn[e] < 1.0f ? 1.0f : 0.0f;
                c0 = a.color[q * 3]; c1 = a.color[q * 3 + 1]; c2 = a.color[q * 3 + 2];
                if (has_bg) {
                    c0 = c0 * inside + a.bg_rgb[qt * 3] * (1.0f - inside);
                    c1 = c1 * inside + a.bg_rgb[qt * 3 + 1] * (1.0f - inside);
                    c2 = c2 * inside + a.bg_rgb[qt * 3 + 2] * (1.0f - inside);
                }
            } else {
                c0 = a.bg_rgb[qt * 3]; c1 = a.bg_rgb[qt * 3 + 1]; c2 = a.bg_rgb[qt * 3 + 2];
            }
            ins[e] = inside;
            float wb = gc[0] * (c0 - bgc[0]) + gc[1] * (c1 - bgc[1]) + gc[2] * (c2 - bgc[2]);
            if (a.g_weights != nullptr) wb += a.g_weights[qt];
            if (has_feat) wb += s_fd[wave][i];
            Wb[e] = wb;
        }
    }
    ray_excl_cumprod(f, Tr, lane);
    double ww[kEPL], suf[kEPL];
#pragma unroll
    for (int e = 0; e < kEPL; ++e) ww[e] = (double)Wb[e] * (double)w[e];
    ray_excl_suffix_sum(ww, suf, lane);
    double dvar = 0.0;
    float ddir[3] = {0.0f, 0.0f, 0.0f};
#pragma unroll
    for (int e = 0; e < kEPL; ++e) {
        const int i = kEPL * lane + e;
        if (i >= T) continue;
        const long qt = (long)r * T + i;
        const float dalpha = Wb[e] * Tr[e] - (float)(suf[e] / (double)f[e]);
        const float wi = w[e];
        float da_in = 0.0f, da_bg = dalpha;
        if (i < N) {
            const long q = (long)r * N + i;
            const float inside = ins[e];
            if (has_bg) {
                da_in = dalpha * inside;
                da_bg = dalpha * (1.0f - inside);
            } else {
                da_in = dalpha;
                da_bg = 0.0f;
            }
            const float cs = has_bg ? inside : 1.0f;
            a.d_color[q * 3] = wi * gc[0] * cs;
            a.d_color[q * 3 + 1] = wi * gc[1] * cs;
            a.d_color[q * 3 + 2] = wi * gc[2] * cs;
            if (has_feat) s_cf[wave][i] = wi * cs;
            const float sdf = a.sdf[q], dist = a.dists[q];
            const float g0 = a.normals[q * 3], g1 = a.normals[q * 3 + 1], g2 = a.normals[q * 3 + 2];
            const float tc = d[0] * g0 + d[1] * g1 + d[2] * g2;
            const float ra = -tc * 0.5f + 0.5f, rb = -tc;
            const float ic = -(fmaxf(ra, 0.0f) * (1.0f - car) + fmaxf(rb, 0.0f) * car);
            const float en = sdf + ic * dist * 0.5f, ep = sdf - ic * dist * 0.5f;
            const float pc = sigmoidf_(ep * inv_s), nc = sigmoidf_(en * inv_s);
            const float raw = ((pc - nc) + 1e-5f) / (pc + 1e-5f);
            const float graw = (raw >= 0.0f && raw <= 1.0f) ? da_in : 0.0f;
            float dpc = graw * (nc / ((pc + 1e-5f) * (pc + 1e-5f)));
            if (a.g_cdf != nullptr) dpc += a.g_cdf[q];
            const float dnc = -graw / (pc + 1e-5f);
            const float dzp = dpc * pc * (1.0f - pc), dzn = dnc * nc * (1.0f - nc);
            const float dep = dzp * inv_s, den = dzn * inv_s;
            dvar += (double)(dzp * ep + dzn * en);
            const float dic = (den - dep) * dist * 0.5f;
            const float dtc = dic * ((ra > 0.0f ? 0.5f * (1.0f - car) : 0.0f) + (rb > 0.0f ? car : 0.0f));
            a.d_sdf[q] = dep + den;
            if (a.d_dists != nullptr) {
                a.d_dists[q] = (den - dep) * ic * 0.5f;
                ddir[0] += dtc * g0; ddir[1] += dtc * g1; ddir[2] += dtc * g2;
            }
            const float relax = pn[e] < 1.2f ? 1.0f : 0.0f;
            const float gn = sqrtf(g0 * g0 + g1 * g1 + g2 * g2);
            const float ke = gn > 0.0f ? g_eik * relax * 2.0f * (gn - 1.0f) / (gn * eik_den) : 0.0f;
            a.d_normals[q * 3] = dtc * d[0] + ke * g0;
            a.d_normals[q * 3 + 1] = dtc * d[1] + ke * g1;
            a.d_normals[q * 3 + 2] = dtc * d[2] + ke * g2;
        }
        if (has_bg) {
            const float cs = (i < N) ? (1.0f - ins[e]) : 1.0f;
            a.d_bg_rgb[qt * 3] = wi * gc[0] * cs;
            a.d_bg_rgb[qt * 3 + 1] = wi * gc[1] * cs;
            a.d_bg_rgb[qt * 3 + 2] = wi * gc[2] * cs;
            if (has_feat && a.d_bg_feat != nullptr) s_cb[wave][i] = wi * cs;
            const float rho_ = a.bg_density[qt], dist = a.bg_dists[qt];
            const float sp = softplus1(rho_);
            const float dsp = rho_ > 20.0f ? 1.0f : sigmoidf_(rho_);
// ... 194 lines not shown
```

### vdn-nerf_amd/csrc/train_sdf_color_bf16.hip

```cpp
#include "k_sdf_fwd2.h"

extern "C" int vdn_sdf_color_train_bf16(const VdnSdfArgs* sa, const void* color_blob, int32_t squeeze_out, void* col_h, void* col_small,
                                        float* col_out, void* stream_) {
    hipStream_t stream = (hipStream_t)stream_;
    if (sa == nullptr || color_blob == nullptr || sa->blob == nullptr || col_h == nullptr || col_small == nullptr || col_out == nullptr) return -1;
    if (sa->pts != nullptr || !sa->rays_o || !sa->rays_d || !sa->z || sa->n_per_ray <= 0 || sa->z_ld < sa->n_per_ray || sa->sdf_ld < sa->n_per_ray) return -2;
    if (!sa->sdf || !sa->feat || !sa->normals || !sa->H || !sa->V || sa->P <= 0) return -3;
    if (sa->U_pe != nullptr || sa->tail_max_rows != 0) return -10;
    vdn::sdf2::ShadeExtra ex{};
    ex.color_blob = static_cast<const char*>(color_blob);
    ex.squeeze_out = squeeze_out;
    ex.col_h = col_h;
    ex.col_small = col_small;
    ex.col_out = col_out;
    return vdn::sdf2::launch<3, true, 4, 3>(sa, stream, nullptr, &ex);
}
```

### vdn-nerf_amd/csrc/vdn_kernels.h

```cpp
#pragma once
#include <hip/hip_runtime.h>
#include "../../include/vdn_render.h"

namespace vdn {
using SdfArgs = ::VdnSdfArgs;
using WeightNormDesc = ::VdnWeightNormDesc;
using ChunkDesc = ::VdnChunkDesc;
using RenderNetArgs = ::VdnRenderNetArgs;
using NerfArgs = ::VdnNerfArgs;
using CoarseArgs = ::VdnCoarseArgs;
using UpsampleArgs = ::VdnUpsampleArgs;
using MergeArgs = ::VdnMergeArgs;
using SectionArgs = ::VdnSectionArgs;
using CompositeArgs = ::VdnCompositeArgs;
using RenderNetBwdArgs = ::VdnRenderNetBwdArgs;
using NerfBwdArgs = ::VdnNerfBwdArgs;
using SdfRbarArgs = ::VdnSdfRbarArgs;
using SdfFbarArgs = ::VdnSdfFbarArgs;
using DwDesc = ::VdnDwDesc;
using DwFinalizeDesc = ::VdnDwFinalizeDesc;
using WeightNormBwdDesc = ::VdnWeightNormBwdDesc;
using CompositeBwdArgs = ::VdnCompositeBwdArgs;
using LossArgs = ::VdnLossArgs;
using RayAdjointArgs = ::VdnRayAdjointArgs;
using TrainPrepArgs = ::VdnTrainPrepArgs;
using GenRaysArgs = ::VdnGenRaysArgs;
using NerfInputGradArgs = ::VdnNerfInputGradArgs;

template <class K>
inline void allow_big_lds(K kernel, size_t bytes) {
    (void)hipFuncSetAttribute(reinterpret_cast<const void*>(kernel), hipFuncAttributeMaxDynamicSharedMemorySize, (int)bytes);
}
}
```

### vdn-nerf_amd/dpt_models/renderer.py

```python
import numpy as np
import torch

from vdn_hip import lib, switches
from vdn_hip.train import PLAN_STATE, background_active
from dpt_models.fields import _require_gpu, _stream


def extract_fields_device(bound_min, bound_max, resolution, query_func, device=None):
    N = 64
    device = device or (bound_min.device if torch.is_tensor(bound_min) and bound_min.is_cuda else torch.device("cuda"))
    lo = [float(v) for v in bound_min]
    hi = [float(v) for v in bound_max]
    X = torch.linspace(lo[0], hi[0], resolution).split(N)
    Y = torch.linspace(lo[1], hi[1], resolution).split(N)
    Z = torch.linspace(lo[2], hi[2], resolution).split(N)
    u = torch.zeros([resolution, resolution, resolution], dtype=torch.float32, device=device)
    with torch.no_grad():
        for xi, xs in enumerate(X):
            for yi, ys in enumerate(Y):
                for zi, zs in enumerate(Z):
                    xx, yy, zz = torch.meshgrid(xs, ys, zs, indexing="ij")
                    pts = torch.stack([xx.reshape(-1), yy.reshape(-1), zz.reshape(-1)], dim=-1).to(device)
                    val = query_func(pts).reshape(len(xs), len(ys), len(zs))
                    u[xi * N: xi * N + len(xs), yi * N: yi * N + len(ys), zi * N: zi * N + len(zs)] = val
# ... 545 lines not shown
                    a.bg_feat = bg_feat.data_ptr()
                lib.call("vdn_feat_composite", a, st)
        else:
            lib.call("vdn_alpha_composite_fwd", a, st)

        self.last_eikonal_terms = eik[1:3]
        return {
            "render_feats": feat_out,
            "color_fine": color,
            "s_val": s_val,
            "cdf_fine": cdf,
            "weight_sum": wsum,
            "weight_max": wmax,
            "gradients": normals.view(B, N, 3),
            "weights": weights,
            "z_vals": bg_mid if O > 0 else mid_z,
            "gradient_error": eik[0],
            "inside_sphere": inside,
        }

    def _fused_shading(self, N, depth_before_color=False):
        cn, sn = self.color_network, self.sdf_network
        return (switches.flag("VDN_SHADE_FUSED") and N == 128 and not depth_before_color
                and sn.precision == cn.precision and sn.precision in ("bf16", "fp32") and cn.conf.get("mode") == "idr"
                and cn.conf.get("d_feature") == 256 and cn.conf.get("d_out") == 3)

    def shade_launches(self):
        vdn = 2 if self.depth_network is not None else 0
        if self._fused_shading(self.n_samples + self.n_importance):
            return 1 + vdn
        return 4 + vdn

    def plan(self, batch, **render_kwargs):
        return RenderPlan(self, batch, **render_kwargs)

    def _all_parameters(self):
        ps = []
        for m in (self.nerf, self.sdf_network, self.deviation_network, self.color_network, self.depth_network):
            if m is not None:
                lib.module_params(m, ps)
        return ps

    def _attach_rays(self, attached, near_d, far_d, z, z_out):
        rays_o, rays_d, near, far = attached
        B, dev = z.shape[0], z.device
        S = self.n_samples
        near, far = near.reshape(B, 1), far.reshape(B, 1)
        z_att = z
        if self.n_importance == 0:
            zc = near + (far - near) * self._consts(dev)["lin_samples"][None, :]
            z_att = z + (zc - zc.detach())
        z_out_att = z_out
        if z_out is not None:
            fd = far_d.reshape(B, 1)
            c = torch.where(fd != 0, (z_out - 1.0 / S) / torch.where(fd != 0, fd, torch.ones_like(fd)), torch.zeros_like(z_out))
            z_out_att = z_out + (far - far.detach()) * c
        return rays_o.contiguous(), rays_d.contiguous(), z_att, z_out_att

    def _engine_for(self, B, dev, params):
        from vdn_hip.train import TrainEngine
        engines = self.__dict__.setdefault("_engines", {})
        nets = (self.nerf, self.sdf_network, self.color_network, self.depth_network)
        pkey = (dev, tuple(p.data_ptr() for p in params), tuple(map(id, params)), self.precision,
                tuple(id(m.__dict__.get("_img")) for m in nets if m is not None))
        key = (B,) + pkey
        eng = engines.pop(key, None)
        if eng is None:
            for k in [k for k in engines if k[1:] != pkey]:
                del engines[k]
            keep = switches.integer("VDN_RENDER_ENGINES")
            while len(engines) >= keep:
                del engines[next(iter(engines))]
            eng = TrainEngine(self, B, dev)
        engines[key] = eng
        return eng

    def _plan_for(self, eng, background_rgb, perturb, t_rand, t_rand_out):
        if not switches.flag("VDN_RENDER_GRAPHS") or torch.cuda.is_current_stream_capturing():
            return None
        O = self.n_outside
        inject = t_rand is not None or t_rand_out is not None
        if inject and (t_rand is None or (O > 0 and t_rand_out is None) or perturb <= 0):
            return None
        key = (background_rgb is not None, float(perturb), inject, switches.signature("train"))
        plans = eng.__dict__.setdefault("_plans", {})
        plan = plans.get(key)
        if plan is None:
            seen = eng.__dict__.setdefault("_plan_seen", {})
            seen[key] = seen.get(key, 0) + 1
            if seen[key] < 2:
                return None
            if seen[key] < 0:
                return None
            while len(plans) >= 4:
                del plans[next(iter(plans))]
            try:
                plan = plans[key] = _TrainPlan(self, eng, key[0], float(perturb), inject)
            except Exception as e:
                import warnings
                seen[key] = -(1 << 30)
                warnings.warn("NeuSRenderer: capturing render() as a HIP graph failed (%s: %s); this configuration keeps the eager "
                              "launches (VDN_RENDER_GRAPHS=0 silences the attempt)" % (type(e).__name__, e))
                return None
        return plan

    def _render_train(self, rays_o, rays_d, z, z_out, background_rgb, cos_anneal_ratio, params, plan=None, eng=None):
        B, dev = rays_o.shape[0], rays_o.device
        if eng is None:
            eng = self._engine_for(B, dev, params)
        if plan is not None:
            eng._plan_call = plan
        bgc = None
        if background_rgb is not None:
            bgc = background_rgb.detach().to(device=dev, dtype=torch.float32).reshape(-1).contiguous()
            if bgc.numel() != 3:
                raise ValueError("background_rgb must have 3 values")
        z = z.contiguous()
        color, feats, weights, eik, cdf, normals, s_val, wsum, wmax, inside, z_ret, eik_terms = _RenderCoreFn.apply(
            eng, rays_o, rays_d, z, z_out, bgc, float(cos_anneal_ratio), *params)
        self.last_eikonal_terms = eik_terms
        return {
            "render_feats": feats if self.depth_network is not None else None,
            "color_fine": color,
            "s_val": s_val,
            "cdf_fine": cdf,
            "weight_sum": wsum,
            "weight_max": wmax,
            "gradients": normals,
            "weights": weights,
            "z_vals": z_ret,
            "gradient_error": eik,
            "inside_sphere": inside,
        }

    def extract_fields(self, bound_min, bound_max, resolution):
        return extract_fields(bound_min, bound_max, resolution, lambda pts: -self.sdf_network.sdf(pts))

    def extract_geometry(self, bound_min, bound_max, resolution, threshold=0.0, method=None, sparse=None):
        return extract_geometry(bound_min, bound_max, resolution=resolution, threshold=threshold,
                                query_func=lambda pts: -self.sdf_network.sdf(pts), method=method, sparse=sparse)

    def extract_colored_geometry(self, bound_min, bound_max, resolution, threshold=0.0, method=None, sparse=None):
        vertices, triangles = self.extract_geometry(bound_min, bound_max, resolution, threshold=threshold, method=method, sparse=sparse)
        normals, colors = self.shade_vertices(vertices)
        return vertices, triangles, normals, colors

    def shade_vertices(self, vertices):
        from vdn_hip import mesh
        dev = lib.first_param(self.sdf_network).device
        x = torch.from_numpy(np.ascontiguousarray(vertices, dtype=np.float32)).reshape(-1, 3).to(dev)
        if x.shape[0] == 0:
            return np.zeros((0, 3), np.float32), np.zeros((0, 3), np.uint8)
        _, g, c = mesh.shade_points(self, x)
        normals = (g / g.norm(dim=-1, keepdim=True).clamp_min(1e-12)).cpu().numpy()
        return normals, mesh.quantize_colors_bgr(c.cpu().numpy())


class RenderPlan:

    def __init__(self, renderer, batch, **render_kwargs):
        if torch.is_grad_enabled() and any(p.requires_grad for p in renderer._all_parameters()):
            raise RuntimeError("RenderPlan is the inference path: build and call it under torch.no_grad()")
        dev = next(renderer.sdf_network.parameters()).device
        self.renderer, self.batch, self.kw = renderer, int(batch), dict(render_kwargs)
        bg = self.kw.get("background_rgb")
        if bg is not None:
            self.kw["background_rgb"] = bg.detach().to(device=dev, dtype=torch.float32).reshape(-1).contiguous().clone()
# ... 44 lines not shown
```

### vdn-nerf_amd/vdn_hip/train.py

```python
import numpy as np
import torch

from . import images, layout, lib, switches

PTS_PER_SPLIT = switches.integer("VDN_DW_SPLIT_PTS")


def _pts_per_split(net, precision="bf16"):
    if precision == "fp32":
        return switches.integer("VDN_DW_SPLIT_PTS_SDF" if net == "sdf" else "VDN_DW_SPLIT_PTS_REST", 2048)
    if net == "sdf":
        return switches.integer("VDN_DW_SPLIT_PTS_SDF", switches.raw("VDN_DW_SPLIT_PTS", 6144))
    rest = switches.raw("VDN_DW_SPLIT_PTS_REST", PTS_PER_SPLIT)
    return switches.integer("VDN_DW_SPLIT_PTS_NERF" if net == "nerf" else "VDN_DW_SPLIT_PTS_HEADS", rest)


_stream = lib.stream_handle


def background_active(rays_o, rays_d, mid_z, T, out=None):
    B, N = mid_z.shape
    dev = mid_z.device
    if out is None:
        out = (torch.empty(B * T, dtype=torch.int32, device=dev), torch.empty(1, dtype=torch.int32, device=dev),
# ... 117 lines not shown
    sfx = "_f32" if precision == "fp32" else "_bf16"
    all_maps, moff = [], 0
    slab_elems, cs_elems, wg = 0, 0, 0
    lay = []
    for e in ent:
        mt = len(e["rmap"]) // 32
        nt = 0 if e["cmap"] is None else len(e["cmap"]) // 32
        segs = 2 if e.get("A2") is not None else 1
        K = e["Pn"] * segs
        pps = _pts_per_split(e["net"], precision)
        splits = max(1, (K + pps - 1) // pps)
        if segs == 2:
            splits += splits % 2
        lay.append((mt, nt, splits, slab_elems, cs_elems, moff, wg))
        all_maps.append(np.asarray(e["rmap"], np.int32))
        moff += mt * 32
        if nt:
            all_maps.append(np.asarray(e["cmap"], np.int32))
            moff += nt * 32
        slab_elems += splits * mt * 32 * nt * 32
        cs_elems += splits * mt * 32
        wg += lib.call_value("vdn_dw_entry_wgs" + sfx, mt, nt, splits)
    return lay, all_maps, slab_elems, cs_elems, wg


def dw_tables(ent, lay, nets, precision, slab, colsum, maps, p_dev, sdf_scale):
    dw = np.zeros(len(ent), dtype=lib.struct_dtype("VdnDwDesc"))
    fin = np.zeros(len(ent), dtype=lib.struct_dtype("VdnDwFinalizeDesc"))
    P4 = lambda spec: spec[0].data_ptr() + spec[0].element_size() * (spec[1] + layout.col_offset_elems(spec[2], precision))
    for i, e in enumerate(ent):
        mt, nt, splits, so, co, mo, wg0 = lay[i]
        d = dw[i]
        d["A1"], d["lda1"] = P4(e["A"]), e["A"][3]
        if e["B"] is not None:
            d["B1"], d["ldb1"] = P4(e["B"]), e["B"][3]
        if e.get("A2") is not None:
            d["A2"], d["lda2"], d["B2"], d["ldb2"] = P4(e["A2"]), e["A2"][3], P4(e["B2"]), e["B2"][3]
        d["P"], d["m_tiles"], d["n_tiles"], d["splits"], d["wg_begin"] = e["Pn"], mt, nt, splits, wg0
        d["P_dev"] = p_dev[i]
        d["slab"] = slab.data_ptr() + 4 * so
        want_cs = e["bias"] or e.get("extra_row0")
        d["colsum"] = colsum.data_ptr() + 4 * co if want_cs else 0
        net = nets[e["net"]]
        fd = fin[i]
        fd["slab"], fd["colsum"] = d["slab"], d["colsum"]
        fd["rmap"] = maps.data_ptr() + 4 * mo
        fd["cmap"] = maps.data_ptr() + 4 * (mo + mt * 32)
        fd["splits"], fd["M"], fd["N"] = splits, mt * 32, nt * 32
        fd["scale"] = e["scale"]
        if e.get("extra_row0"):
            main = next(k for k, x in enumerate(ent) if x["net"] == e["net"] and x["name"] == e["name"] and not x.get("extra_row0"))
            fm = fin[main]
            fm["xsum"], fm["xsplits"], fm["xM"], fm["xrow"] = d["colsum"], splits, mt * 32, 0
            fm["xscale"] = 1.0 / sdf_scale
            fd["slab"], fd["colsum"] = 0, 0
        else:
            tgt = net.dw_target(e["name"])
            fd["target"], fd["t_stride"] = tgt.data_ptr(), tgt.shape[1]
            if e["bias"]:
                bt = net.bias_target(e["name"])
                fd["btarget"], fd["bscale"] = bt.data_ptr(), 1.0
    return dw, fin


def weightnorm_table(nets):
    rows = []
    for key, net in nets.items():
        for name, (g, v, b) in net.img.matrices.items():
            if g is not None:
                rows.append((key, g, v, net.img.inv_norm[net.img.r_off[name]:], net.dweff_view(name), net.grads[id(g)], net.grads[id(v)]))
    wn = np.zeros(len(rows), dtype=lib.struct_dtype("VdnWeightNormBwdDesc"))
    for i, (key, g, v, inv, dwe, dg, dv) in enumerate(rows):
        wn[i]["g"], wn[i]["v"], wn[i]["inv_norm"], wn[i]["dw_eff"] = g.data_ptr(), v.data_ptr(), inv.data_ptr(), dwe.data_ptr()
        wn[i]["dg"], wn[i]["dv"], wn[i]["rows"], wn[i]["cols"] = dg.data_ptr(), dv.data_ptr(), v.shape[0], v.shape[1]
    return wn, [r[0] for r in rows]


class DwGroup:

    def __init__(self, dw, n_dw, wgs, fin, n_fin, max_m, phase1, wn, n_wn, wn_rows):
        self.dw, self.n_dw, self.wgs = dw, n_dw, wgs
        self.fin, self.n_fin, self.max_m, self.phase1 = fin, n_fin, max_m, phase1
        self.wn, self.n_wn, self.wn_rows = wn, n_wn, wn_rows

    def launch_gemm(self, sfx, stream):
        lib.call("vdn_dw_gemm" + sfx, lib.ptr(self.dw), self.n_dw, self.wgs, stream)

    def launch(self, sfx, stream, gemm_event=None, event_stream=None):
        if self.n_dw:
            self.launch_gemm(sfx, stream)
        if gemm_event is not None:
            gemm_event.record(event_stream if event_stream is not None else lib.current_stream())
        for phase in range((2 if self.phase1 else 1) if self.n_fin else 0):
            lib.call("vdn_dw_finalize", lib.ptr(self.fin), self.n_fin, self.max_m, phase, stream)
        if self.n_wn:
            lib.call("vdn_weightnorm_bwd", lib.ptr(self.wn), self.n_wn, self.wn_rows, stream)


def dw_group(dw, fin, wn, lo, hi, total_wgs, dev, extra_fin=None, wn_idx=(), dw_dev=None):
    up = lambda a: torch.from_numpy(a.view(np.uint8).copy()).to(dev)
    wg_lo, wg_hi = (int(dw[i]["wg_begin"]) if i < len(dw) else total_wgs for i in (lo, hi))
    if lo == 0 and dw_dev is not None:
        tab = dw_dev
    else:
        sub = dw[lo:hi].copy()
        sub["wg_begin"] -= wg_lo
        tab = up(sub)
    f = fin[lo:hi] if extra_fin is None else np.concatenate([fin[lo:hi], extra_fin])
    w = wn[list(wn_idx)]
    return DwGroup(tab, hi - lo, wg_hi - wg_lo, up(f), len(f), int(fin[lo:hi]["M"].max()), bool((f["accumulate"] != 0).any()),
                   up(w) if len(w) else None, len(w), int(w["rows"].max()) if len(w) else 1)


PLAN_STATE = ("_ctx", "_fg_compact", "_bg_compact", "_composite_bwd_done", "_bwd_train", "_pending", "_ray_grads", "_color_fused",
              "_car_dev", "_fwd_rays", "_fused_keep")


class TrainEngine:
    def __init__(self, renderer, B, dev):
        self.r = renderer
        self.B, self.dev = B, dev
        S, I, O = renderer.n_samples, renderer.n_importance, renderer.n_outside
        self.N = S + I
        self.T = self.N + O
        self.P = B * self.N
        self.Q = B * self.T
        self.wdepth = renderer.depth_network is not None
        self.dbc = renderer.color_network.conf["d_feature"] == 352
        if self.dbc and not self.wdepth:
            raise ValueError("a d_feature = 352 colour network needs a depth_network (renderer.py:245-248)")
        use_side = switches.flag("VDN_SIDE_STREAM") and torch.device(dev).type == "cuda"
        self._side = shared_stream(dev, "side") if use_side else None
        self._ev_fork = torch.cuda.Event() if use_side else None
        self._ev_join = torch.cuda.Event() if use_side else None
        self._side2 = shared_stream(dev, "side2") if (use_side and renderer.depth_network is not None) else None
        self._ev_fork2 = torch.cuda.Event() if self._side2 is not None else None
        self._ev_join2 = torch.cuda.Event() if self._side2 is not None else None
        self._ev_heads = torch.cuda.Event() if use_side else None
        self._ctx = self._fwd_rays = self._car_dev = self._bwd_train = self._fused_keep = None
        self._pending = self._ray_grads = self._color_fused = self._composite_bwd_done = False
        self._fg_compact = self._bg_compact = False
        self.generation = 0
        self._bwd_warm = False
        self._bwd_args_keep = self.join_hook = self.sdf_probe = self._out_strided = self._clone_slots = None
        precs = {m.precision for m in (renderer.nerf, renderer.sdf_network, renderer.color_network, renderer.depth_network) if m is not None}
        if len(precs) != 1:
            raise ValueError("all networks of a renderer must share one precision, got %s" % sorted(precs))
        self.precision = precs.pop()
        self.sfx = "_f32" if self.precision == "fp32" else "_bf16"
        self._fmt = images.FMT_F32 if self.precision == "fp32" else images.FMT_BF16
        sdt =torch.float32 if self.precision == "fp32" else torch.bfloat16
        f = lambda *shape: torch.empty(*shape, dtype=torch.float32, device=dev)
        fs = lambda *shape: torch.empty(*shape, dtype=sdt, device=dev)
        P, Q, N, T = self.P, self.Q, self.N, self.T
        Pp, Qp = layout.rows(P, self.precision), layout.rows(Q, self.precision)
        self.Pp, self.Qp = Pp, Qp
        w = self.w = {}
        w["dists"] = f(B, N)
        fz = lambda *shape: torch.zeros(*shape, dtype=torch.float32, device=dev)
        slots, n_out = {}, 0
        for name, shape in (("color", (B, 3)), ("weights", (B, T)), ("eik", (3,)), ("feat_out", (B, 96) if self.wdepth else None),
                            ("cdf", (B, N)), ("normals", (P, 3)), ("inside", (B, N)), ("s_val", (B, 1)),
                            ("bg_mid", (B, T) if O > 0 else None), ("mid_z", (B, N)), ("wsum", (B, 1)), ("wmax", (B, 1))):
            if shape is not None:
                slots[name] = (n_out, shape)
                n_out += (int(np.prod(shape)) + 63) // 64 * 64
        self._out_arena, self._out_slots = fz(n_out), slots
        out = lambda name: self._out_arena[slots[name][0]:slots[name][0] + int(np.prod(slots[name][1]))].view(slots[name][1])
        w["sdf"], w["feat"], w["normals"], w["mid_z"] = fz(P), fs(Pp, 256), out("normals"), out("mid_z")
        w["fg_active"] = (torch.zeros(P, dtype=torch.int32, device=dev), torch.zeros(1, dtype=torch.int32, device=dev),
                          torch.zeros(B, dtype=torch.int32, device=dev))
        w["H"], w["V"], w["PE"] = fs(8, Pp, 256), fs(8, Pp, 256), fs(Pp, 64)
        if self.precision == "fp32":
            w["S"] = fs(8, Pp, 256)
        w["col_out"], w["col_h"], w["col_small"] = fz(P, 3), fs(4, Pp, 256), fs(Pp, 64)
        if self.wdepth:
            w["vdn_out"], w["vdn_h"], w["vdn_small"] = fz(P, 96), fs(4, Pp, 256), fs(Pp, 64)
        if self.dbc:
            w["col_extra"] = fs(Pp, 96)
        self.relu_mask = self.precision == "bf16" and switches.flag("VDN_RELU_MASK")
        fm = lambda *shape: torch.empty(*shape, dtype=torch.uint8, device=dev) if self.relu_mask else None
        w["col_mask"] = fm(4, Pp * 32)
        if self.wdepth:
            w["vdn_mask"] = fm(4, Pp * 32)
        if O > 0:
            w["z_feed"], w["bg_dists"], w["bg_mid"] = f(B, T), f(B, T), out("bg_mid")
            w["bg_density"], w["bg_rgb"] = torch.zeros(Q, device=dev), torch.zeros(Q, 3, device=dev)
            w["bg_feat"] = torch.zeros(Q, 96, device=dev) if self.wdepth else None
            w["bg_active"] = (torch.zeros(Q, dtype=torch.int32, device=dev), torch.zeros(1, dtype=torch.int32, device=dev),
                              torch.zeros(B, dtype=torch.int32, device=dev))
            w["nf_h"], w["nf_pe"], w["nf_feature"], w["nf_vpe"], w["nf_hv"] = fs(8, Qp, 256), fs(Qp, 96), fs(Qp, 256), fs(Qp, 32), fs(Qp, 128)
            w["nf_mask"], w["nf_mask_v"] = fm(8, Qp * 32), fm(Qp * 16)
        w["weights"], w["alpha"], w["cdf"], w["inside"] = out("weights"), f(B, T), out("cdf"), out("inside")
        w["color"], w["wsum"], w["wmax"], w["s_val"] = out("color"), out("wsum"), out("wmax"), out("s_val")
        w["eik_partial"], w["eik"] = f(B, 2), out("eik")
        w["feat_out"] = out("feat_out") if self.wdepth else None
        w["d_sdf"], w["d_normals"], w["d_color"], w["d_featvec"] = f(P), f(P, 3), f(P, 3), fs(Pp, 256)
        w["d_vdn"] = f(P, 96) if self.wdepth else None
        w["feat_scratch"] = f(B * (2 * T + N)) if self.wdepth else None
        w["d_var_partial"], w["d_variance"] = f(B), f(1)
        w["col_dout"], w["col_dh"] = fs(Pp, 32), fs(4, Pp, 256)
        if self.wdepth:
            w["vdn_dout"], w["vdn_dh"] = fs(Pp, 96), fs(4, Pp, 256)
        w["UB"], w["EX"], w["AB"] = fs(Pp * 2144), fs(8, Pp, 256), fs(Pp * 2336)
        if O > 0:
            w["d_bg_density"], w["d_bg_rgb"] = f(Q), f(Q, 3)
            w["d_bg_feat"] = f(Q, 96) if self.wdepth else None
            w["nf_do"], w["nf_dv"], w["nf_dhead"], w["nf_dh"] = fs(Qp, 128 if self.wdepth else 32), fs(Qp, 128), fs(Qp, 288), fs(8, Qp, 256)
        self.params = renderer._all_parameters()
        total = sum(p.numel() for p in self.params)
        self._grad_flat = torch.zeros(total, dtype=torch.float32, device=dev)
        views, off = {}, 0
        for p in self.params:
            views[id(p)] = self._grad_flat[off:off + p.numel()].view(p.shape)
            off += p.numel()
        self.grad_views = views
        self.nets = {"sdf": _Net(renderer.sdf_network, dev, views), "color": _Net(renderer.color_network, dev, views)}
        if self.wdepth:
            self.nets["vdn"] = _Net(renderer.depth_network, dev, views)
        if O > 0:
            self.nets["nerf"] = _Net(renderer.nerf, dev, views)
        self._build_dw_plan()

    def _build_dw_plan(self):
        w, P, Q = self.w, self.P, self.Q
        Pp, Qp, prec = self.Pp, self.Qp, self.precision
        ent = sdf_dw_entries(w["H"], w["V"], w["PE"], w["UB"], w["AB"], P, Pp, prec)
        ent += rendering_dw_entries("color", self.nets["color"].img.streams["fwd"][0].kmap, w["col_dh"], w["col_dout"], w["col_h"],
                                    w["col_small"], w["feat"], w.get("col_extra"), P, 3)
        if self.wdepth:
            ent += rendering_dw_entries("vdn", self.nets["vdn"].img.streams["fwd"][0].kmap, w["vdn_dh"], w["vdn_dout"], w["vdn_h"],
                                        w["vdn_small"], w["feat"], None, P, 96)
        if "nerf" in self.nets:
            ent += nerf_dw_entries(self.nets["nerf"].img.streams, w["nf_dh"], w["nf_h"], w["nf_pe"], w["nf_dhead"], w["nf_dv"],
                                   w["nf_feature"], w["nf_vpe"], w["nf_do"], w["nf_hv"], Q, self.wdepth)

        dev = self.dev
        lay, all_maps, slab_elems, cs_elems, wg = dw_layout(ent, prec)
        self.maps = torch.from_numpy(np.concatenate(all_maps)).to(dev)
        self.slab = torch.empty(max(slab_elems, 1), dtype=torch.float32, device=dev)
        self.colsum = torch.empty(max(cs_elems, 1), dtype=torch.float32, device=dev)
        self.dw_list_kind = ["bg" if e["net"] == "nerf" else "fg" for e in ent]
        p_dev = [(w["bg_active"] if k == "bg" else w["fg_active"])[1].data_ptr() for k in self.dw_list_kind]
        dw, fin = dw_tables(ent, lay, self.nets, prec, self.slab, self.colsum, self.maps, p_dev, float(self.r.sdf_network.scale))
        wn, wn_net = weightnorm_table(self.nets)
        vfin = np.zeros(1, dtype=fin.dtype)
        self._var_map = torch.zeros(1, dtype=torch.int32, device=dev)
        vfin[0]["colsum"], vfin[0]["rmap"] = w["d_var_partial"].data_ptr(), self._var_map.data_ptr()
        vfin[0]["btarget"], vfin[0]["bscale"] = self.grad_views[id(self.r.deviation_network.variance)].data_ptr(), 1.0
        vfin[0]["splits"], vfin[0]["M"], vfin[0]["N"] = self.B, 1, 0
        n_sdf = sum(1 for e in ent if e["net"] == "sdf")
        n_heads_end = n_sdf + sum(1 for e in ent if e["net"] not in ("sdf", "nerf"))
        ranges = {"all": (0, len(ent)), "sdf": (0, n_sdf), "rest": (n_sdf, len(ent)), "heads": (n_sdf, n_heads_end),
                  "nerf": (n_heads_end, len(ent))}
        dw_dev = torch.from_numpy(dw.view(np.uint8)).to(dev)
        self.groups = {}
        for g, (lo, hi) in ranges.items():
            if hi > lo:
                own = {e["net"] for e in ent[lo:hi]}
                self.groups[g] = dw_group(dw, fin, wn, lo, hi, wg, dev, vfin if lo == 0 else None,
                                          [i for i, k in enumerate(wn_net) if k in own], dw_dev)
        self._param_ptrs = self._ptr_key()

    @property
    def grad_flat(self):
        if self.join_hook is not None:
            self.join_hook()
        return self._grad_flat

    def _ptr_key(self):
        return tuple(p.data_ptr() for net in self.nets.values() for p in lib.module_params(net.module))

    def _ray_workspaces(self):
        w, B, N, T, P, Q, dev = self.w, self.B, self.N, self.T, self.P, self.Q, self.dev
        if "U_pe" not in w:
            f = lambda *shape: torch.zeros(*shape, dtype=torch.float32, device=dev)
            w["U_pe"], w["d_pts"], w["d_dirs"] = f(P, 39), f(P, 3), f(P, 3)
            w["d_dists"], w["d_dir_cos"] = f(B, N), f(B, 3)
            w["d_rays_o"], w["d_rays_d"], w["d_z"] = f(B, 3), f(B, 3), f(B, N)
            if self.r.n_outside > 0:
                w["d_bg_pts"], w["d_bg_dirs"], w["d_bg_dists"], w["d_z_out"] = f(Q, 3), f(Q, 3), f(B, T), f(B, T - N)
        return w

    def forward(self, rays_o, rays_d, z, z_out, background_rgb, cos_anneal_ratio, skip_far=False, ray_grads=False, pending_merge=None,
                after_sdf=None, fuse_loss=None, before_heads=None, rest_normals=False, cos_anneal_dev=None, ray_grads_compact=False):
        r, w, B, N, T = self.r, self.w, self.B, self.N, self.T
        st = _stream()
        if ray_grads and skip_far and not ray_grads_compact:
            raise ValueError("ray gradients need every inside sample evaluated (skip_far=False)")
        self._ray_grads = bool(ray_grads)
        self._car_dev = cos_anneal_dev
        self._fwd_rays = (rays_o, rays_d)
        if ray_grads:
            self._ray_workspaces()
        for net in self.nets.values():
            net.img = net.module._images(join=before_heads is None)
        if self._ptr_key() != self._param_ptrs:
            raise RuntimeError("parameters were re-allocated after the training engine was built; rebuild it")
        if any(net.img.fmt != self._fmt for net in self.nets.values()):
            raise RuntimeError("a network's precision changed after the training engine was built (%s); rebuild it" % self.precision)
        sample_dist = 2.0 / r.n_samples
        O = r.n_outside
        self._fg_compact = bool(skip_far) and O > 0 and switches.flag("VDN_FG_COMPACT")
        self._color_fused = (self.precision == "bf16" and not self.dbc and not ray_grads and "c2" in self.nets["color"].img.blobs
                             and r.color_network.conf["d_out"] == 3 and switches.flag("VDN_TRAIN_COLOR_FUSED")
                             and not self._tail_wanted())
        self._bg_compact = O > 0 and switches.flag("VDN_BG_COMPACT")
        fused_prep = self._bg_compact and switches.flag("VDN_FUSED_PREP")
        if pending_merge is not None and not fused_prep:
            new_z, M_old = pending_merge
            m = lib.VdnMergeArgs()
            m.z, m.new_z, m.z_out = z.data_ptr(), new_z.data_ptr(), z.data_ptr()
            m.B, m.M, m.K, m.ld, m.ld_out = B, M_old, N - M_old, z.stride(0), z.stride(0)
            lib.call("vdn_merge_sorted", m, st)
            pending_merge = None
        if O > 0 and not fused_prep:
            m = lib.VdnMergeArgs()
            m.z, m.new_z, m.z_out = z.data_ptr(), z_out.data_ptr(), w["z_feed"].data_ptr()
            m.B, m.M, m.K, m.ld, m.ld_out = B, N, O, z.stride(0), T
            lib.call("vdn_merge_sorted", m, st)
        if fused_prep:
            tp = lib.VdnTrainPrepArgs()
            tp.rays_o, tp.rays_d, tp.z, tp.z_out, tp.z_feed = (t.data_ptr() for t in (rays_o, rays_d, z, z_out, w["z_feed"]))
            tp.B, tp.N, tp.T, tp.z_ld, tp.sample_dist, tp.fg_radius = B, N, T, z.stride(0), sample_dist, 1.2
            if pending_merge is not None:
                tp.new_z, tp.M_old = pending_merge[0].data_ptr(), pending_merge[1]
            tp.dists, tp.mid_z, tp.bg_dists, tp.bg_mid = (w[k].data_ptr() for k in ("dists", "mid_z", "bg_dists", "bg_mid"))
            if self._fg_compact:
                tp.fg_active_idx, tp.fg_n_active, tp.fg_ray_counts = (t.data_ptr() for t in w["fg_active"])
            tp.bg_active_idx, tp.bg_n_active, tp.bg_ray_counts = (t.data_ptr() for t in w["bg_active"])
            lib.call("vdn_train_prep", tp, st)
            if fuse_loss is not None and fuse_loss.get("after_prep") is not None:
                fuse_loss["after_prep"](self)
        else:
            a = lib.VdnSectionArgs()
            a.z, a.dists, a.mid_z, a.sample_dist, a.B, a.n, a.ld = z.data_ptr(), w["dists"].data_ptr(), w["mid_z"].data_ptr(), sample_dist, B, N, z.stride(0)
            lib.call("vdn_sections", a, st)
            if self._fg_compact:
                fa = lib.VdnForegroundActiveArgs()
                fa.rays_o, fa.rays_d, fa.mid_z, fa.B, fa.N, fa.radius = rays_o.data_ptr(), rays_d.data_ptr(), w["mid_z"].data_ptr(), B, N, 1.2
                fa.active_idx, fa.n_active, fa.ray_counts = (t.data_ptr() for t in w["fg_active"])
                lib.call("vdn_foreground_active", fa, st)
        if not self._fg_compact:
            w["fg_active"][1].fill_(self.P)
        if O > 0:
            if not fused_prep:
                a = lib.VdnSectionArgs()
                a.z, a.dists, a.mid_z, a.sample_dist, a.B, a.n, a.ld = w["z_feed"].data_ptr(), w["bg_dists"].data_ptr(), w["bg_mid"].data_ptr(), sample_dist, B, T, T
                lib.call("vdn_sections", a, st)
            n = lib.VdnNerfArgs()
            n.blob = self.nets["nerf"].img.blobs["fwd"].data_ptr()
            n.rays_o, n.rays_d, n.z, n.n_per_ray, n.P = rays_o.data_ptr(), rays_d.data_ptr(), w["bg_mid"].data_ptr(), T, self.Q
            n.density, n.rgb = w["bg_density"].data_ptr(), w["bg_rgb"].data_ptr()
            n.feat = w["bg_feat"].data_ptr() if w["bg_feat"] is not None else None
            n.save_h, n.save_pe, n.save_feature, n.save_vpe, n.save_hv = (w[k].data_ptr() for k in ("nf_h", "nf_pe", "nf_feature", "nf_vpe", "nf_hv"))
            if self.relu_mask:
                n.save_mask, n.save_mask_v = w["nf_mask"].data_ptr(), w["nf_mask_v"].data_ptr()
            if self._bg_compact:
                if not fused_prep:
                    background_active(rays_o, rays_d, w["mid_z"], T, out=w["bg_active"])
                n.active_idx, n.n_active = w["bg_active"][0].data_ptr(), w["bg_active"][1].data_ptr()
            else:
                w["bg_active"][1].fill_(self.Q)
            self._fork()
            lib.call("vdn_nerf_mlp_fwd" + self.sfx, n, self._side_handle(st))
            if rest_normals and self._fg_compact:
                self._sdf_rest(rays_o, rays_d, self._side_handle(st))
            self._side_done()
        if self._color_fused and before_heads is not None:
            before_heads()
            before_heads = None
        self._sdf_forward(rays_o, rays_d)
        if after_sdf is not None:
            after_sdf(self)

        def rnet(net, out, save_h, small, d_out, module, stream=None):
            c = lib.VdnRenderNetArgs()
            c.blob = self.nets[net].img.blobs["fwd"].data_ptr()
            c.rays_o, c.rays_d, c.z, c.n_per_ray = rays_o.data_ptr(), rays_d.data_ptr(), w["mid_z"].data_ptr(), N
            c.normals, c.feat, c.out = w["normals"].data_ptr(), w["feat"].data_ptr(), out.data_ptr()
            c.save_h, c.save_small = save_h.data_ptr(), small.data_ptr()
            if self.relu_mask:
                c.save_mask = w[net[:3] + "_mask"].data_ptr()
            c.P, c.d_out, c.squeeze_out = self.P, d_out, int(module.squeeze_out)
            if net == "color" and self.dbc:
                c.extra, c.save_extra = w["vdn_out"].data_ptr(), w["col_extra"].data_ptr()
            lib.call("vdn_rendernet_fwd" + self.sfx, self._fg(c), st if stream is None else stream)
        if before_heads is not None:
            before_heads()
        vdn_beside = self.wdepth and self._side2 is not None and not self.dbc
        if self.wdepth:
            if vdn_beside:
                self._ev_fork2.record(lib.current_stream())
                self._side2.wait_event(self._ev_fork2)
                rnet("vdn", w["vdn_out"], w["vdn_h"], w["vdn_small"], 96, r.depth_network, stream=self._side2.cuda_stream)
                self._ev_join2.record(self._side2)
            else:
                rnet("vdn", w["vdn_out"], w["vdn_h"], w["vdn_small"], 96, r.depth_network)
        if not self._color_fused:
            rnet("color", w["col_out"], w["col_h"], w["col_small"], 3, r.color_network)
        if vdn_beside:
            lib.current_stream().wait_event(self._ev_join2)

        c = self._composite_common(lib.VdnCompositeArgs(), rays_o, rays_d, background_rgb, cos_anneal_ratio)
        c.weights, c.alpha_out, c.cdf, c.inside_sphere = w["weights"].data_ptr(), w["alpha"].data_ptr(), w["cdf"].data_ptr(), w["inside"].data_ptr()
        c.color_out, c.weight_sum, c.weight_max, c.s_val = w["color"].data_ptr(), w["wsum"].data_ptr(), w["wmax"].data_ptr(), w["s_val"].data_ptr()
        c.eik_partial, c.eik_out = w["eik_partial"].data_ptr(), w["eik"].data_ptr()
        if self.wdepth:
            c.feat_out = w["feat_out"].data_ptr()
        self._join()
        self._ctx = (rays_o, rays_d, background_rgb, cos_anneal_ratio, z)
        self._composite_bwd_done = False
        self._bwd_train = None
        if fuse_loss is not None and fuse_loss.get("before_composite") is not None:
            if not (fused_prep and self._fg_compact):
                raise RuntimeError("fuse_loss with a global foreground count needs the fused step preparation and the work lists")
            fuse_loss["before_composite"]()
        fg_count = lib.ptr(fuse_loss["fg_count"] if (fuse_loss is not None and fuse_loss.get("fg_count") is not None) else w["fg_active"][1])
        if fuse_loss is not None and self._fg_compact and self.wdepth and fuse_loss.get("gt_feats") is not None and not ray_grads:
            lib.call("vdn_composite_fwd_train", c, lib.ptr(fuse_loss["gt_feats"]), lib.ptr(fuse_loss["g_feats"]),
                     float(fuse_loss["depth_weight"]), float(fuse_loss["grad_scale"]), st)
            self._bwd_train = fuse_loss
        elif fuse_loss is not None and self._fg_compact and not self.wdepth and not ray_grads:
            cb = self._composite_bwd_args(None, None, None, None, None)
            self._fused_keep = (c, cb, fuse_loss)
            lib.call("vdn_composite_train", c, cb, lib.ptr(fuse_loss["true_rgb"]), lib.ptr(fuse_loss["g_color"]), fg_count,
                     float(fuse_loss["igr_weight"]), float(fuse_loss["grad_scale"]), st)
            self._composite_bwd_done = True
        else:
            lib.call("vdn_alpha_composite_fwd", c, st)
        self.generation += 1
        return w

    def _fg(self, args):
        if self._fg_compact:
            args.active_idx, args.n_active = self.w["fg_active"][0].data_ptr(), self.w["fg_active"][1].data_ptr()
        return args

    def _fork(self):
        if self._side is not None:
            self._ev_fork.record(lib.current_stream())
            self._side.wait_event(self._ev_fork)

    def _side_handle(self, main_handle):
        return main_handle if self._side is None else self._side.cuda_stream

    def _side_done(self):
        if self._side is not None:
            self._ev_join.record(self._side)
            self._pending = True

    def _join(self):
        if self._side is not None and self._pending:
            lib.current_stream().wait_event(self._ev_join)
            self._pending = False

    def _tail_wanted(self):
        tail_default = "1" if self._side is None else "0"
        return (self.precision == "bf16" and self._fg_compact and switches.flag("VDN_SDF_TAIL", tail_default)
                and not self._ray_grads)

    def _sdf_args(self, rays_o, rays_d, feat):
        w, N, img = self.w, self.N, self.nets["sdf"].img
        s = lib.VdnSdfArgs()
        s.blob = img.blobs["full"].data_ptr()
        s.rays_o, s.rays_d, s.z, s.n_per_ray, s.z_ld, s.sdf_ld = rays_o.data_ptr(), rays_d.data_ptr(), w["mid_z"].data_ptr(), N, N, N
        s.P, s.scale = self.P, float(self.r.sdf_network.scale)
        s.sdf, s.feat, s.normals = w["sdf"].data_ptr(), feat.data_ptr(), w["normals"].data_ptr()
        s.w8row = img.weff_view("lin8").data_ptr()
        return s

    def _sdf_rest(self, rays_o, rays_d, stream):
        w, N = self.w, self.N
        if "fg_rest" not in w:
            w["fg_rest"] = (torch.zeros(self.P, dtype=torch.int32, device=self.dev), torch.zeros(1, dtype=torch.int32, device=self.dev),
                            torch.zeros(self.B, dtype=torch.int32, device=self.dev))
        fa = lib.VdnForegroundActiveArgs()
        fa.rays_o, fa.rays_d, fa.mid_z, fa.B, fa.N, fa.radius = rays_o.data_ptr(), rays_d.data_ptr(), w["mid_z"].data_ptr(), self.B, N, 1.2
        fa.complement = 1
        fa.active_idx, fa.n_active, fa.ray_counts = (t.data_ptr() for t in w["fg_rest"])
        lib.call("vdn_foreground_active", fa, stream)
        s = self._sdf_args(rays_o, rays_d, w["d_featvec"])
        if "S" in w:
            if "S_rest" not in w:
                w["S_rest"] = torch.empty_like(w["S"])
            s.S = w["S_rest"].data_ptr()
        s.active_idx, s.n_active = w["fg_rest"][0].data_ptr(), w["fg_rest"][1].data_ptr()
        lib.call("vdn_sdf_mlp_fwd" + self.sfx, 1, s, stream)

    def _sdf_forward(self, rays_o, rays_d):
        r, w = self.r, self.w
        s = self._sdf_args(rays_o, rays_d, w["feat"])
        if "S" in w:
            s.S = w["S"].data_ptr()
        s.H, s.V, s.PE = w["H"].data_ptr(), w["V"].data_ptr(), w["PE"].data_ptr()
        if self._ray_grads:
            s.U_pe = w["U_pe"].data_ptr()
        tail = self._tail_wanted()
        fused = self._color_fused and not tail
        if tail:
            row0 = switches.integer("VDN_SDF_TAIL_ROW0", 128 * torch.cuda.get_device_properties(self.dev).multi_processor_count)
            tail = self.P > row0
            if tail:
                s.tail_row0, s.tail_max_rows = row0, switches.integer("VDN_SDF_TAIL_MAX")

        def launch():
            if fused:
                cimg = self.nets["color"].img
                lib.call("vdn_sdf_color_train_bf16", self._fg(s), lib.ptr(cimg.blobs["c2"]), int(r.color_network.squeeze_out),
                         lib.ptr(w["col_h"]), lib.ptr(w["col_small"]), lib.ptr(w["col_out"]), _stream())
                return
            lib.call("vdn_sdf_mlp_fwd" + self.sfx, 1, self._fg(s), _stream())
            if tail:
                lib.call("vdn_sdf_fwd_tail_bf16", s, _stream())
        probe = self.sdf_probe
        if probe is None:
            launch()
            return
        e0, e1 = torch.cuda.Event(enable_timing=True), torch.cuda.Event(enable_timing=True)
        e0.record()
        launch()
        e1.record()
        probe.append((e0, e1, w["fg_active"][1].clone() if self._fg_compact else None))

    def _dw_rows(self):
        n = {"bg": int(self.w["bg_active"][1].item()) if "bg_active" in self.w else 0, "fg": int(self.w["fg_active"][1].item())}
        tab = np.frombuffer(self.groups["all"].dw.cpu().numpy().tobytes(), dtype=lib.struct_dtype("VdnDwDesc"))
        return tab, [min(int(d["P"]), n[k]) for d, k in zip(tab, self.dw_list_kind)]

    def dw_bytes(self):
        esz = 4 if self.precision == "fp32" else 2
        total = 0
        tab, rows = self._dw_rows()
        for d, r in zip(tab, rows):
            segs = 2 if d["A2"] else 1
            total += segs * r * 32 * (int(d["m_tiles"]) + int(d["n_tiles"])) * esz
            total += int(d["splits"]) * int(d["m_tiles"]) * 32 * int(d["n_tiles"]) * 32 * 4
        return total

    def dw_flops(self):
        tab, rows = self._dw_rows()
        return sum(2.0 * (2 if d["A2"] else 1) * r * int(d["m_tiles"]) * 32 * int(d["n_tiles"]) * 32 for d, r in zip(tab, rows))

    def _launch_dw(self):
        self.groups["all"].launch_gemm(self.sfx, _stream())

    def _launch_dw_groups(self):
        for group in ("sdf", "rest"):
            if group in self.groups:
                self.groups[group].launch_gemm(self.sfx, _stream())

    def side_weight_grads(self, group, after=None, gemm_event=None):
        if self._side is None:
            self.weight_grads(group, _stream())
            return None
        if after is not None:
            self._side.wait_event(after)
        elif group != "nerf":
            self._side.wait_event(self._ev_heads)
        self.weight_grads(group, self._side.cuda_stream, gemm_event, event_stream=self._side)
        self._pending = False
        return self._side

    def weight_grads(self, group, stream, gemm_event=None, event_stream=None):
        self.groups[group].launch(self.sfx, stream, gemm_event, event_stream)

    def _composite_common(self, c, rays_o, rays_d, background_rgb, cos_anneal_ratio):
        w, r = self.w, self.r
        c.rays_o, c.rays_d, c.sdf, c.normals = rays_o.data_ptr(), rays_d.data_ptr(), w["sdf"].data_ptr(), w["normals"].data_ptr()
        c.dists, c.mid_z, c.color = w["dists"].data_ptr(), w["mid_z"].data_ptr(), w["col_out"].data_ptr()
        c.variance = r.deviation_network.variance.data_ptr()
        if self.wdepth:
            c.feat, c.feat_ch = w["vdn_out"].data_ptr(), 96
        if r.n_outside > 0:
            c.bg_density, c.bg_rgb, c.bg_dists = w["bg_density"].data_ptr(), w["bg_rgb"].data_ptr(), w["bg_dists"].data_ptr()
            if self.wdepth:
                c.bg_feat = w["bg_feat"].data_ptr()
        if background_rgb is not None:
            c.background_rgb = background_rgb.data_ptr()
        c.cos_anneal_ratio = float(cos_anneal_ratio)
        if self._car_dev is not None:
            c.cos_anneal_dev = self._car_dev.data_ptr()
        c.B, c.N, c.T = self.B, self.N, self.T
        return c

    def _composite_bwd_args(self, g_color, g_feat, g_weights, g_eik, g_cdf):
        r, w = self.r, self.w
        rays_o, rays_d, background_rgb, car, z = self._ctx
        c = self._composite_common(lib.VdnCompositeBwdArgs(), rays_o, rays_d, background_rgb, car)
        c.alpha, c.weights, c.eik = w["alpha"].data_ptr(), w["weights"].data_ptr(), w["eik"].data_ptr()
        c.g_cdf = g_cdf.data_ptr() if g_cdf is not None else None
        c.g_color = g_color.data_ptr() if g_color is not None else None
        c.g_feat = g_feat.data_ptr() if (g_feat is not None and self.wdepth) else None
        c.g_weights = g_weights.data_ptr() if g_weights is not None else None
        c.g_eik = g_eik.data_ptr() if g_eik is not None else None
        c.d_sdf, c.d_normals, c.d_color = w["d_sdf"].data_ptr(), w["d_normals"].data_ptr(), w["d_color"].data_ptr()
        if self.wdepth:
            c.d_feat = w["d_vdn"].data_ptr()
            c.feat_scratch = w["feat_scratch"].data_ptr()
            if g_feat is None:
                w["d_vdn"].zero_()
        if r.n_outside > 0:
            c.d_bg_density, c.d_bg_rgb = w["d_bg_density"].data_ptr(), w["d_bg_rgb"].data_ptr()
            if self.wdepth:
                c.d_bg_feat = w["d_bg_feat"].data_ptr()
                if g_feat is None:
                    w["d_bg_feat"].zero_()
        c.d_var_partial = w["d_var_partial"].data_ptr()
        if self._ray_grads:
            c.d_dists, c.d_dir_cos = w["d_dists"].data_ptr(), w["d_dir_cos"].data_ptr()
            if r.n_outside > 0:
                c.d_bg_dists = w["d_bg_dists"].data_ptr()
        self._bwd_args_keep = (g_color, g_feat, g_weights, g_eik, g_cdf)
        return c

    def backward(self, g_color, g_feat, g_weights, g_eik, g_cdf=None, g_gradients=None, defer_rest=False, gemm_event=None,
                 fork_event=None, heads_event=True):
        r, w, st = self.r, self.w, _stream()
        self._bwd_warm = True
        rays_o, rays_d, background_rgb, car, z = self._ctx
        keep = [t.contiguous() if t is not None else None for t in (g_color, g_feat, g_weights, g_eik, g_cdf, g_gradients)]
        g_color, g_feat, g_weights, g_eik, g_cdf, g_gradients = keep
        if (g_cdf is not None or g_gradients is not None) and self._fg_compact:
            raise ValueError("adjoints of cdf_fine / gradients need every inside sample evaluated (skip_far=False)")
        use_vdn = self.wdepth and g_feat is not None
        rg = self._ray_grads
        if self._composite_bwd_done:
            self._composite_bwd_done = False
        elif self._bwd_train is not None:
            fl, self._bwd_train = self._bwd_train, None
            c = self._composite_bwd_args(None, g_feat, None, None, None)
            lib.call("vdn_composite_bwd_train", c, lib.ptr(w["color"]), lib.ptr(fl["true_rgb"]), lib.ptr(fl["g_color"]),
                     lib.ptr(fl["fg_count"] if fl.get("fg_count") is not None else w["fg_active"][1]),
                     float(fl["igr_weight"]), float(fl["grad_scale"]), st)
        else:
            c = self._composite_bwd_args(g_color, g_feat, g_weights, g_eik, g_cdf)
            lib.call("vdn_alpha_composite_bwd", c, st)
        if g_gradients is not None:
            w["d_normals"].add_(g_gradients.reshape(self.P, 3))
        if r.n_outside > 0:
            nb = lib.VdnNerfBwdArgs()
            nb.blob = self.nets["nerf"].img.blobs["bwd"].data_ptr()
            nb.g_density, nb.g_rgb = w["d_bg_density"].data_ptr(), w["d_bg_rgb"].data_ptr()
            nb.g_feat = w["d_bg_feat"].data_ptr() if self.wdepth else None
            nb.save_h, nb.save_hv = w["nf_h"].data_ptr(), w["nf_hv"].data_ptr()
            if self.relu_mask:
                nb.mask, nb.mask_v = w["nf_mask"].data_ptr(), w["nf_mask_v"].data_ptr()
            nb.delta_o, nb.delta_v, nb.delta_head, nb.delta_h = (w[k].data_ptr() for k in ("nf_do", "nf_dv", "nf_dhead", "nf_dh"))
            nb.P = self.Q
            if self._bg_compact:
                nb.active_idx, nb.n_active = w["bg_active"][0].data_ptr(), w["bg_active"][1].data_ptr()
            if rg:
                w["d_bg_pts"].zero_()
                w["d_bg_dirs"].zero_()
                nb.rays_o, nb.rays_d, nb.z, nb.n_per_ray = rays_o.data_ptr(), rays_d.data_ptr(), w["bg_mid"].data_ptr(), self.T
                nb.d_pts, nb.d_dirs = w["d_bg_pts"].data_ptr(), w["d_bg_dirs"].data_ptr()
            if fork_event is not None and self._side is not None:
                self._side.wait_event(fork_event)
            else:
                self._fork()
            lib.call("vdn_nerf_mlp_bwd" + self.sfx, nb, self._side_handle(st))
            split_dw = (not defer_rest and self._side is not None and not rg and switches.flag("VDN_BWD_SPLIT_DW")
                        and all(k in self.groups for k in ("sdf", "heads", "nerf")))
            if split_dw:
                self.weight_grads("nerf", self._side.cuda_stream)
            self._side_done()

        def rnet_bwd(net, g_out, out, save_h, dout, dh, d_out, module, accumulate):
            b = lib.VdnRenderNetBwdArgs()
            b.blob = self.nets[net].img.blobs["bwd"].data_ptr()
            b.g_out, b.out, b.save_h = g_out.data_ptr(), out.data_ptr(), save_h.data_ptr()
            if self.relu_mask and not (net == "color" and self._color_fused):
                b.mask = w[net[:3] + "_mask"].data_ptr()
            b.delta_out, b.delta_h = dout.data_ptr(), dh.data_ptr()
            b.d_feat, b.d_normals = w["d_featvec"].data_ptr(), w["d_normals"].data_ptr()
            b.acc_feat, b.acc_normals = int(accumulate), 1
            b.P, b.d_out, b.squeeze_out = self.P, d_out, int(module.squeeze_out)
            if net == "color" and self.dbc:
                b.d_extra = w["d_vdn"].data_ptr()
            if rg:
                b.rays_d, b.n_per_ray, b.acc_pts = rays_d.data_ptr(), self.N, int(accumulate)
                b.d_pts, b.d_dirs = w["d_pts"].data_ptr(), w["d_dirs"].data_ptr()
            lib.call("vdn_rendernet_bwd" + self.sfx, self._fg(b), st)
        if rg and self._fg_compact:
            w["d_pts"].zero_()
            w["d_dirs"].zero_()
        rnet_bwd("color", w["d_color"], w["col_out"], w["col_h"], w["col_dout"], w["col_dh"], 3, r.color_network, False)
        if self.wdepth:
            rnet_bwd("vdn", w["d_vdn"], w["vdn_out"], w["vdn_h"], w["vdn_dout"], w["vdn_dh"], 96, r.depth_network, True)
        if defer_rest and self._side is not None and heads_event:
            self._ev_heads.record(lib.current_stream())

        rb = lib.VdnSdfRbarArgs()
        img = self.nets["sdf"].img
        rb.blob = img.blobs["full"].data_ptr()
        rb.rays_o, rb.rays_d, rb.z, rb.n_per_ray, rb.z_ld = rays_o.data_ptr(), rays_d.data_ptr(), w["mid_z"].data_ptr(), self.N, self.N
        rb.P, rb.scale = self.P, float(r.sdf_network.scale)
        s_from_h = 2 if self.precision == "bf16" else 0
        s_planes = w["H"] if s_from_h else w["S"]
        rb.g_normals, rb.S, rb.V, rb.UB, rb.EX = w["d_normals"].data_ptr(), s_planes.data_ptr(), w["V"].data_ptr(), w["UB"].data_ptr(), w["EX"].data_ptr()
        rb.s_from_h = s_from_h
        one_launch = self.precision == "bf16" and not rg and switches.flag("VDN_SDF_BWD_SPLIT")
        fb = lib.VdnSdfFbarArgs()
        fb.blob = img.blobs["fbar"].data_ptr()
        fb.g_sdf, fb.g_feat, fb.S, fb.EX, fb.AB = w["d_sdf"].data_ptr(), w["d_featvec"].data_ptr(), s_planes.data_ptr(), w["EX"].data_ptr(), w["AB"].data_ptr()
        fb.P, fb.scale, fb.s_from_h = self.P, float(r.sdf_network.scale), s_from_h
        if rg:
            fb.rays_o, fb.rays_d, fb.z, fb.n_per_ray, fb.z_ld = rays_o.data_ptr(), rays_d.data_ptr(), w["mid_z"].data_ptr(), self.N, self.N
            fb.g_normals, fb.U_pe, fb.acc_pts, fb.d_pts = w["d_normals"].data_ptr(), w["U_pe"].data_ptr(), 1, w["d_pts"].data_ptr()
        if not (one_launch and lib.try_call("vdn_sdf_bwd_split_bf16", self._fg(rb), self._fg(fb), st)):
            lib.call("vdn_sdf_bwd_rbar" + self.sfx, self._fg(rb), st)
            lib.call("vdn_sdf_bwd_fbar" + self.sfx, self._fg(fb), st)

        if defer_rest:
            if rg:
                raise ValueError("defer_rest is the Trainer's path: no ray gradients there")
            self.weight_grads("sdf", st, gemm_event)
            return self._grad_flat
        if r.n_outside > 0 and split_dw:
            self.weight_grads("sdf", st)
            self.weight_grads("heads", st)
            self._join()
        else:
            self._join()
            self.groups["all"].launch(self.sfx, st)
        if rg:
            ra = lib.VdnRayAdjointArgs()
            ra.rays_d, ra.mid_z = rays_d.data_ptr(), w["mid_z"].data_ptr()
            ra.d_pts, ra.d_dirs, ra.d_dists, ra.d_dir_cos = (w[k].data_ptr() for k in ("d_pts", "d_dirs", "d_dists", "d_dir_cos"))
            ra.B, ra.N, ra.T = self.B, self.N, self.T
            if r.n_outside > 0:
                ra.bg_mid = w["bg_mid"].data_ptr()
                ra.d_bg_pts, ra.d_bg_dirs, ra.d_bg_dists, ra.d_z_out = (w[k].data_ptr() for k in ("d_bg_pts", "d_bg_dirs", "d_bg_dists", "d_z_out"))
            ra.d_rays_o, ra.d_rays_d, ra.d_z = w["d_rays_o"].data_ptr(), w["d_rays_d"].data_ptr(), w["d_z"].data_ptr()
            lib.call("vdn_ray_adjoint", ra, st)
        return self._grad_flat

    def outputs_clone(self):
        a = self._out_arena.clone()
        if self._out_strided is None:
            self._out_strided = [(k, tuple(sh), tuple(torch.empty(sh, device="meta").stride()), o) for k, (o, sh) in self._out_slots.items()]
        st, base = a.untyped_storage(), a.storage_offset()
        return {k: torch.empty(0, dtype=torch.float32, device=a.device).set_(st, base + o, sh, sd) for k, sh, sd, o in self._out_strided}

    def param_grads(self, clone=True):
        if self.join_hook is not None:
            self.join_hook()
        if not clone:
            return [self.grad_views[id(p)] for p in self.params]
        if self._clone_slots is None:
            slots, off = [], 0
            for p in self.params:
                slots.append((tuple(p.shape), tuple(self.grad_views[id(p)].stride()), off))
                off += (p.numel() + 63) // 64 * 64
            self._clone_slots, self._clone_total = slots, off
            self._grad_list = [self.grad_views[id(p)] for p in self.params]
        flat = torch.empty(self._clone_total, dtype=torch.float32, device=self._grad_flat.device)
        out = [flat.as_strided(sh, st, o) for sh, st, o in self._clone_slots]
        torch._foreach_copy_(out, self._grad_list)
        return out
```

Baseline: 422,900 rays/s.

## Skip colour-head work for foreground points outside the unit sphere

Splits the compacted foreground active list into two classes: points inside an inner radius (unit sphere) and points in the shell between it and the outer radius. Only the first class runs the colour/depth heads forward and backward and their weight-gradient GEMM rows. The SDF still runs on all foreground points. When a background model exists, outside points get their colour forced to zero in compositing and their feature loads skipped, since their colour enters the loss only through zero weight. Buffers become zero-initialised, and the backward pass zero-fills d_feat rows for skipped points so no stale values leak into later stages. This adds complexity and relies on the claim that shell points contribute exactly zero to the loss.

```diff
diff --git a/include/vdn_render.h b/include/vdn_render.h
--- a/include/vdn_render.h
+++ b/include/vdn_render.h
@@ -212,6 +212,8 @@
                         int32_t* ticket, void* stream);
 int vdn_sdf_color_train_bf16(const VdnSdfArgs* sdf_host, const void* color_blob, int32_t squeeze_out, void* col_h, void* col_small,
                              float* col_out, void* stream);
+int vdn_sdf_color_train_rows_bf16(const VdnSdfArgs* sdf_host, const void* color_blob, int32_t squeeze_out, void* col_h, void* col_small,
+                                  float* col_out, const int32_t* n_color_rows, void* stream);
 int vdn_shade_fused_bf16(const VdnSdfArgs* sdf_host, const void* color_blob, int32_t squeeze_out, const VdnCompositeArgs* comp_host,
                          int32_t* ticket, void* stream);
 int vdn_shade_points_bf16(const VdnSdfArgs* sdf_host, const void* color_blob, int32_t squeeze_out, float* col_out, void* stream);
@@ -251,6 +253,7 @@
     float* d_dirs;
     float* d_extra;
     const void* mask;
+    const int32_t* n_rows_all;
 } VdnRenderNetBwdArgs;
 int vdn_rendernet_bwd_f32(const VdnRenderNetBwdArgs* args_host, void* stream);
 int vdn_rendernet_bwd_bf16(const VdnRenderNetBwdArgs* args_host, void* stream);
@@ -349,6 +352,8 @@
 } VdnDwDesc;
 int vdn_dw_gemm_f32(const VdnDwDesc* descs_dev, int n_desc, int total_wgs, void* stream);
 int vdn_dw_gemm_bf16(const VdnDwDesc* descs_dev, int n_desc, int total_wgs, void* stream);
+int vdn_dw_gemm_rows_f32(const VdnDwDesc* descs_dev, int n_desc, int total_wgs, const int32_t* cap_rows, int cap_lo, int cap_hi, void* stream);
+int vdn_dw_gemm_rows_bf16(const VdnDwDesc* descs_dev, int n_desc, int total_wgs, const int32_t* cap_rows, int cap_lo, int cap_hi, void* stream);
 int vdn_dw_entry_wgs_f32(int m_tiles, int n_tiles, int splits);
 int vdn_dw_entry_wgs_bf16(int m_tiles, int n_tiles, int splits);
 
@@ -491,6 +496,9 @@
     int32_t* active_idx;
     int32_t* n_active;
     int32_t* ray_counts;
+    float inner_radius;
+    int32_t _pad_inner;
+    int32_t* n_inner;
 } VdnForegroundActiveArgs;
 
 typedef struct {
@@ -506,6 +514,7 @@
     float* bg_dists; float* bg_mid;
     int32_t* fg_active_idx; int32_t* fg_n_active; int32_t* fg_ray_counts;
     int32_t* bg_active_idx; int32_t* bg_n_active; int32_t* bg_ray_counts;
+    float fg_inner_radius; int32_t _pad_inner; int32_t* fg_n_inner;
 } VdnTrainPrepArgs;
 int vdn_train_prep(const VdnTrainPrepArgs* args_host, void* stream);
 int vdn_foreground_active(const VdnForegroundActiveArgs* args_host, void* stream);
diff --git a/vdn-nerf_amd/csrc/k_composite_row.h b/vdn-nerf_amd/csrc/k_composite_row.h
--- a/vdn-nerf_amd/csrc/k_composite_row.h
+++ b/vdn-nerf_amd/csrc/k_composite_row.h
@@ -64,7 +64,8 @@
                 eikonal_add(pn, g0, g1, g2, eik_num, eik_den);
                 a.cdf[q] = prev_cdf;
                 a.inside_sphere[q] = inside;
-                float c0 = src.color(q, i, 0), c1 = src.color(q, i, 1), c2 = src.color(q, i, 2);
+                const bool heads = !has_bg || pn < 1.0f;
+                float c0 = heads ? src.color(q, i, 0) : 0.0f, c1 = heads ? src.color(q, i, 1) : 0.0f, c2 = heads ? src.color(q, i, 2) : 0.0f;
                 if (has_bg) {
                     const long qb = (long)r * T + i;
                     al = al * inside + bg_a * (1.0f - inside);
@@ -126,10 +127,10 @@
 struct FeatRaw { float fg[2], bg[2]; };
 struct FeatPair { float f0, f1; };
 template <class A>
-VDN_DEV FeatRaw feat_load(const A& a, int r, int i, int ch0, int ch1) {
+VDN_DEV FeatRaw feat_load(const A& a, int r, int i, int ch0, int ch1, float inside) {
     const int N = a.N, T = a.T, C = a.feat_ch;
     const bool v0 = ch0 < C, v1 = ch1 < C;
-    const bool fg = i < N, bg = i < T && (a.bg_density != nullptr || i >= N) && a.bg_feat != nullptr;
+    const bool fg = i < N && (a.bg_density == nullptr || inside != 0.0f), bg = i < T && (a.bg_density != nullptr || i >= N) && a.bg_feat != nullptr;
     const long qf = ((long)r * N + i) * C, qb = ((long)r * T + i) * C;
     FeatRaw v;
     v.fg[0] = (fg && v0) ? a.feat[qf + ch0] : 0.0f;
@@ -147,13 +148,13 @@
 }
 template <class A>
 VDN_DEV FeatPair feat_pair(const A& a, int r, int i, int ch0, int ch1, float inside) {
-    return feat_mix(a, i, feat_load(a, r, i, ch0, ch1), inside);
+    return feat_mix(a, i, feat_load(a, r, i, ch0, ch1, inside), inside);
 }
 template <class A>
 VDN_DEV void feat_group(const A& a, int r, int i0, int i_end, int ch0, int ch1, const float (&inside)[8], FeatPair (&f)[8]) {
     FeatRaw v[8];
 #pragma unroll
-    for (int k = 0; k < 8; ++k) v[k] = i0 + k < i_end ? feat_load(a, r, i0 + k, ch0, ch1) : FeatRaw{};
+    for (int k = 0; k < 8; ++k) v[k] = i0 + k < i_end ? feat_load(a, r, i0 + k, ch0, ch1, inside[k]) : FeatRaw{};
 #pragma unroll
     for (int k = 0; k < 8; ++k) f[k] = i0 + k < i_end ? feat_mix(a, i0 + k, v[k], inside[k]) : FeatPair{};
 }
diff --git a/vdn-nerf_amd/csrc/k_ray_rows.h b/vdn-nerf_amd/csrc/k_ray_rows.h
--- a/vdn-nerf_amd/csrc/k_ray_rows.h
+++ b/vdn-nerf_amd/csrc/k_ray_rows.h
@@ -266,6 +266,8 @@
     int32_t* active_idx;
     int32_t* n_active;
     int32_t* ray_counts;
+    float inner;
+    int32_t* n_inner;
 };
 
 VDN_DEV bool sample_active(const ActiveJob& a, int r, int s, const float (&o)[3], const float (&d)[3]) {
@@ -275,7 +277,46 @@
 }
 
 template <bool FILL>
+VDN_DEV void active_list_row_classes(const ActiveJob& a, int r, int lane, const float (&o)[3], const float (&d)[3]) {
+    int base0 = 0, base1 = 0, total0 = 0;
+    if (FILL) {
+        int acc0 = 0, acc1 = 0, all0 = 0;
+        for (int i = lane; i < a.B; i += 64) {
+            const int c0 = a.ray_counts[i];
+            all0 += c0;
+            if (i < r) { acc0 += c0; acc1 += a.ray_counts[a.B + i]; }
+        }
+        base0 = (int)wave_sum((double)acc0);
+        total0 = (int)wave_sum((double)all0);
+        base1 = total0 + (int)wave_sum((double)acc1);
+    }
+    int n0 = 0, n1 = 0;
+    for (int s0 = 0; s0 < a.N; s0 += 64) {
+        const int s = s0 + lane;
+        const float pn = s < a.N ? sample_norm(o, d, a.mid_z[(long)r * a.N + s]) : 2.0f * a.radius;
+        const bool in0 = s < a.N && pn < a.inner, in1 = s < a.N && pn < a.radius && !(pn < a.inner);
+        const unsigned long long m0 = __ballot(in0), m1 = __ballot(in1), below = (1ull << lane) - 1ull;
+        if (FILL && in0) a.active_idx[base0 + n0 + __popcll(m0 & below)] = r * a.N + s;
+        if (FILL && in1) a.active_idx[base1 + n1 + __popcll(m1 & below)] = r * a.N + s;
+        n0 += __popcll(m0);
+        n1 += __popcll(m1);
+    }
+    if (lane == 0) {
+        if (!FILL) {
+            a.ray_counts[r] = n0;
+            a.ray_counts[a.B + r] = n1;
+        } else if (r == a.B - 1) {
+            const int total = base1 + n1;
+            a.n_active[0] = total;
+            a.n_inner[0] = total0;
+            a.n_inner[1] = min(total, (total0 + 127) / 128 * 128);
+        }
+    }
+}
+
+template <bool FILL>
 VDN_DEV void active_list_row(const ActiveJob& a, int r, int lane, const float (&o)[3], const float (&d)[3]) {
+    if (a.inner > 0.0f) return active_list_row_classes<FILL>(a, r, lane, o, d);
     int base = 0;
     if (FILL) {
         int acc = 0;
diff --git a/vdn-nerf_amd/csrc/k_render_bwd.h b/vdn-nerf_amd/csrc/k_render_bwd.h
--- a/vdn-nerf_amd/csrc/k_render_bwd.h
+++ b/vdn-nerf_amd/csrc/k_render_bwd.h
@@ -14,7 +14,19 @@
     ws.init(a.blob, smem, 42 + EX);
     const int lane = ws.lane, c = lane & 31, h = lane >> 5;
     const WorkRow wr = work_row(a.active_idx, a.n_active, a.P, P::kWaves, ws.wave, c);
-    if (wr.none) return;
+    if (wr.none) {
+        if (a.n_rows_all != nullptr && !a.acc_feat) {
+            const WorkRow wz = work_row(a.active_idx, a.n_rows_all, a.P, P::kWaves, ws.wave, c);
+            if (!wz.none) {
+                f32x16 zero;
+#pragma unroll
+                for (int t = 0; t < 16; ++t) zero[t] = 0.0f;
+#pragma unroll
+                for (int nt = 0; nt < 8; ++nt) P::store_tile(reinterpret_cast<typename P::store_t*>(a.d_feat), wz.row, 256, nt, h, zero, wz.ok);
+            }
+        }
+        return;
+    }
     ws.warm_issue(wr.n_wg, 256 * P::kMinWavesPerEU);
     warm_code_issue((std::is_same<P, BF16>::value) ? kWarmCodeRenderBwd : 0, wr.n_wg, 256 * P::kMinWavesPerEU, ws.warm_dump());
     const bool ok = wr.ok;
@@ -148,6 +160,7 @@
         !args->delta_h || !args->d_feat || !args->d_normals) return -1;
     if (!(args->d_out == 96 || (args->d_out >= 1 && args->d_out <= 4))) return -2;
     if (args->d_pts && (!args->d_dirs || (!args->dirs && (!args->rays_d || args->n_per_ray <= 0)))) return -3;
+    if (args->n_rows_all && (!args->active_idx || !args->n_active || !args->acc_normals || args->d_pts)) return -6;
     const int ppw = P::kWaves * 32;
     const int grid = (args->P + ppw - 1) / ppw;
     const size_t lds = 3 * P::stride(8);
diff --git a/vdn-nerf_amd/csrc/k_sdf_fwd2.h b/vdn-nerf_amd/csrc/k_sdf_fwd2.h
--- a/vdn-nerf_amd/csrc/k_sdf_fwd2.h
+++ b/vdn-nerf_amd/csrc/k_sdf_fwd2.h
@@ -214,6 +214,7 @@
     void* col_h;
     void* col_small;
     float* col_out;
+    const int32_t* n_col_rows;
     CompositeArgs cm;
 };
 
@@ -250,6 +251,7 @@
 #endif
     const bool ok = wr.ok;
     const long p = wr.row, pd = wr.point;
+    const bool col_wg = MODE != 3 || ex.n_col_rows == nullptr || (long)blockIdx.x * (kWaves * 32) < (long)*ex.n_col_rows;
     const int c16 = lane & 15, q4 = lane >> 4;
     (void)c16; (void)q4;
 
@@ -530,7 +532,7 @@
                     cur[pr & 3] = pk;
                     D.r[T * 2 + (pr >> 2)] = __builtin_bit_cast(bf16x8, cur);
                     if constexpr (MODE == 3 && (pr & 3) == 3)
-                        plane_store16(reinterpret_cast<ST*>(ex.col_h) + L.l * PS + piece(T, pr >> 2), cur);
+                        if (col_wg) plane_store16(reinterpret_cast<ST*>(ex.col_h) + L.l * PS + piece(T, pr >> 2), cur);
                 });
             } else if constexpr (L.kind == COLOUT) {
                 if constexpr (PB == 0) {
@@ -631,7 +633,7 @@
                     for (int i = 0; i < 32; ++i) s33[i] = small[i];
                     s33[32] = nz;
 #pragma unroll
-                    for (int kt = 0; kt < 2; ++kt) P::store_tile(reinterpret_cast<ST*>(ex.col_small), p, 64, kt, h, vals_tile<33>(s33, h, kt), true);
+                    for (int kt = 0; kt < 2; ++kt) P::store_tile(reinterpret_cast<ST*>(ex.col_small), p, 64, kt, h, vals_tile<33>(s33, h, kt), col_wg);
                 }
             }
         } else {
@@ -645,7 +647,7 @@
             for (int d = 0; d < 3; ++d) a.normals[pd * 3 + d] = n[d] * a.scale;
             if constexpr (MODE == 3 || MODE == 4) {
 #pragma unroll
-                for (int d = 0; d < 3; ++d) ex.col_out[pd * 3 + d] = col[d];
+                for (int d = 0; d < 3; ++d) if (col_wg) ex.col_out[pd * 3 + d] = col[d];
             }
         }
     }
diff --git a/vdn-nerf_amd/csrc/rays.hip b/vdn-nerf_amd/csrc/rays.hip
--- a/vdn-nerf_amd/csrc/rays.hip
+++ b/vdn-nerf_amd/csrc/rays.hip
@@ -262,7 +262,9 @@
 extern "C" int vdn_foreground_active(const VdnForegroundActiveArgs* a, void* stream) {
     if (!a || a->B <= 0 || a->N <= 0 || !a->rays_o || !a->rays_d || !a->mid_z || !(a->radius > 0.0f) ||
         !a->active_idx || !a->n_active || !a->ray_counts) return -1;
-    const ActiveJob j = {a->rays_o, a->rays_d, a->mid_z, a->B, a->N, a->N, a->radius, false, a->complement != 0, a->active_idx, a->n_active, a->ray_counts};
+    if ((a->inner_radius != 0.0f || a->n_inner) && (!(a->inner_radius > 0.0f) || !(a->inner_radius <= a->radius) || !a->n_inner || a->complement)) return -2;
+    const ActiveJob j = {a->rays_o, a->rays_d, a->mid_z, a->B, a->N, a->N, a->radius, false, a->complement != 0, a->active_idx, a->n_active, a->ray_counts,
+                         a->inner_radius, a->n_inner};
     return launch_active(j, stream);
 }
 
@@ -307,7 +309,8 @@
         __builtin_amdgcn_wave_barrier();
     }
     if (a.fg_active_idx != nullptr && !second)
-        active_list_row<PASS == 1>(ActiveJob{a.rays_o, a.rays_d, a.mid_z, a.B, a.N, a.N, a.fg_radius, false, false, a.fg_active_idx, a.fg_n_active, a.fg_ray_counts},
+        active_list_row<PASS == 1>(ActiveJob{a.rays_o, a.rays_d, a.mid_z, a.B, a.N, a.N, a.fg_radius, false, false, a.fg_active_idx, a.fg_n_active, a.fg_ray_counts,
+                                             a.fg_inner_radius, a.fg_n_inner},
                                    r, lane, o, d);
     if (PASS == 0 || second)
         active_list_row<PASS == 1>(ActiveJob{a.rays_o, a.rays_d, a.mid_z, a.B, a.N, a.T, 1.0f, true, false, a.bg_active_idx, a.bg_n_active, a.bg_ray_counts},
@@ -321,6 +324,8 @@
     if (a->new_z && (a->M_old < 1 || a->M_old >= a->N || a->N - a->M_old > 64)) return -2;
     if (!a->bg_active_idx || !a->bg_n_active || !a->bg_ray_counts) return -3;
     if (a->fg_active_idx && (!a->fg_n_active || !a->fg_ray_counts || !(a->fg_radius > 0.0f))) return -4;
+    if ((a->fg_inner_radius != 0.0f || a->fg_n_inner) &&
+        (!a->fg_active_idx || !(a->fg_inner_radius > 0.0f) || !(a->fg_inner_radius <= a->fg_radius) || !a->fg_n_inner)) return -4;
     launch_rays(train_prep_kernel<0>, a->B, stream, *a);
     launch_ray_blocks(train_prep_kernel<1>, 2 * ray_blocks(a->B), stream, *a);
     return (int)hipGetLastError();
diff --git a/vdn-nerf_amd/csrc/train_dw_bf16.hip b/vdn-nerf_amd/csrc/train_dw_bf16.hip
--- a/vdn-nerf_amd/csrc/train_dw_bf16.hip
+++ b/vdn-nerf_amd/csrc/train_dw_bf16.hip
@@ -54,7 +54,7 @@
 
 VDN_DEV int dw_uni(int v) { return __builtin_amdgcn_readfirstlane(v); }
 
-__global__ __launch_bounds__(512, 1) void dw_gemm_bf16_kernel(const DwDesc* descs, int n_desc) {
+__global__ __launch_bounds__(512, 1) void dw_gemm_bf16_kernel(const DwDesc* descs, int n_desc, DwRowCap cap) {
     extern __shared__ __attribute__((aligned(16))) char smem[];
     const int wg = blockIdx.x;
     int di = 0;
@@ -76,6 +76,7 @@
     const int s_in = seg2 ? split - seg_splits : split;
     int P = dw_uni(d.P);
     if (d.P_dev != nullptr) P = min(P, dw_uni(*d.P_dev));
+    if (cap.rows != nullptr && dw_uni(di) >= cap.lo && dw_uni(di) < cap.hi) P = dw_uni(min(P, max(dw_uni(*cap.rows), 0)));
     int per = (P + seg_splits - 1) / seg_splits;
     per = (per + 127) / 128 * 128;
     const int k_begin = s_in * per, k_end = min(k_begin + per, P);
@@ -193,11 +194,21 @@
     return splits * mg * ng;
 }
 
-extern "C" int vdn_dw_gemm_bf16(const VdnDwDesc* descs_dev, int n_desc, int total_wgs, void* stream) {
+static int dw_gemm_bf16(const VdnDwDesc* descs_dev, int n_desc, int total_wgs, vdn::DwRowCap cap, void* stream) {
     using namespace vdn;
     if (!descs_dev || n_desc <= 0 || total_wgs <= 0) return -1;
     static bool once = (allow_big_lds(dw_gemm_bf16_kernel, kDwBuf * kDwStageBytes), true);
     (void)once;
-    hipLaunchKernelGGL(dw_gemm_bf16_kernel, dim3(total_wgs), dim3(512), kDwBuf * kDwStageBytes, (hipStream_t)stream, descs_dev, n_desc);
+    hipLaunchKernelGGL(dw_gemm_bf16_kernel, dim3(total_wgs), dim3(512), kDwBuf * kDwStageBytes, (hipStream_t)stream, descs_dev, n_desc, cap);
     return (int)hipGetLastError();
 }
+
+extern "C" int vdn_dw_gemm_bf16(const VdnDwDesc* descs_dev, int n_desc, int total_wgs, void* stream) {
+    return dw_gemm_bf16(descs_dev, n_desc, total_wgs, vdn::DwRowCap{nullptr, 0, 0}, stream);
+}
+
+extern "C" int vdn_dw_gemm_rows_bf16(const VdnDwDesc* descs_dev, int n_desc, int total_wgs, const int32_t* cap_rows, int cap_lo, int cap_hi,
+                                     void* stream) {
+    if (!cap_rows || cap_lo < 0 || cap_hi < cap_lo || cap_hi > n_desc) return -2;
+    return dw_gemm_bf16(descs_dev, n_desc, total_wgs, vdn::DwRowCap{cap_rows, cap_lo, cap_hi}, stream);
+}
diff --git a/vdn-nerf_amd/csrc/train_dw_f32.hip b/vdn-nerf_amd/csrc/train_dw_f32.hip
--- a/vdn-nerf_amd/csrc/train_dw_f32.hip
+++ b/vdn-nerf_amd/csrc/train_dw_f32.hip
@@ -6,7 +6,7 @@
 constexpr int kF32StagePts = 32;
 constexpr int kF32PanelBytes = kF32StagePts * 128 * 4;
 
-__global__ __launch_bounds__(256, 2) void dw_gemm_f32_kernel(const DwDesc* descs, int n_desc) {
+__global__ __launch_bounds__(256, 2) void dw_gemm_f32_kernel(const DwDesc* descs, int n_desc, DwRowCap cap) {
     extern __shared__ __attribute__((aligned(16))) char smem[];
     const int wg = blockIdx.x;
     int di = 0;
@@ -29,7 +29,8 @@
     const int seg_splits = two ? d.splits / 2 : d.splits;
     const bool seg2 = two && split >= seg_splits;
     const int s_in = seg2 ? split - seg_splits : split;
-    const long P = d.P_dev != nullptr ? min((long)d.P, (long)*d.P_dev) : (long)d.P;
+    long P = d.P_dev != nullptr ? min((long)d.P, (long)*d.P_dev) : (long)d.P;
+    if (cap.rows != nullptr && di >= cap.lo && di < cap.hi) P = min(P, max((long)*cap.rows, 0L));
     long per = (P + seg_splits - 1) / seg_splits;
     per = (per + kF32StagePts - 1) / kF32StagePts * kF32StagePts;
     const long k_begin = (long)s_in * per, k_end = min(k_begin + per, P);
@@ -183,12 +184,22 @@
     return 8 * ((splits + 7) / 8) * mt4 * nt4;
 }
 
-extern "C" int vdn_dw_gemm_f32(const VdnDwDesc* descs_dev, int n_desc, int total_wgs, void* stream) {
+static int dw_gemm_f32(const VdnDwDesc* descs_dev, int n_desc, int total_wgs, vdn::DwRowCap cap, void* stream) {
     if (!descs_dev || n_desc <= 0 || total_wgs <= 0) return -1;
     static bool once = (vdn::allow_big_lds(vdn::dw_gemm_f32_kernel, 4 * vdn::kF32PanelBytes), true);
     (void)once;
-    hipLaunchKernelGGL(vdn::dw_gemm_f32_kernel, dim3(total_wgs), dim3(256), 4 * vdn::kF32PanelBytes, (hipStream_t)stream, descs_dev, n_desc);
+    hipLaunchKernelGGL(vdn::dw_gemm_f32_kernel, dim3(total_wgs), dim3(256), 4 * vdn::kF32PanelBytes, (hipStream_t)stream, descs_dev, n_desc, cap);
     return (int)hipGetLastError();
+}
+
+extern "C" int vdn_dw_gemm_f32(const VdnDwDesc* descs_dev, int n_desc, int total_wgs, void* stream) {
+    return dw_gemm_f32(descs_dev, n_desc, total_wgs, vdn::DwRowCap{nullptr, 0, 0}, stream);
+}
+
+extern "C" int vdn_dw_gemm_rows_f32(const VdnDwDesc* descs_dev, int n_desc, int total_wgs, const int32_t* cap_rows, int cap_lo, int cap_hi,
+                                    void* stream) {
+    if (!cap_rows || cap_lo < 0 || cap_hi < cap_lo || cap_hi > n_desc) return -2;
+    return dw_gemm_f32(descs_dev, n_desc, total_wgs, vdn::DwRowCap{cap_rows, cap_lo, cap_hi}, stream);
 }
 
 extern "C" int vdn_dw_finalize(const VdnDwFinalizeDesc* descs_dev, int n_desc, int max_M, int phase, void* stream) {
diff --git a/vdn-nerf_amd/csrc/train_rays.hip b/vdn-nerf_amd/csrc/train_rays.hip
--- a/vdn-nerf_amd/csrc/train_rays.hip
+++ b/vdn-nerf_amd/csrc/train_rays.hip
@@ -119,7 +119,8 @@
                 const long q = (long)r * N + i;
                 pn[e] = sample_norm(o, d, a.mid_z[q]);
                 inside = pn[e] < 1.0f ? 1.0f : 0.0f;
-                c0 = a.color[q * 3]; c1 = a.color[q * 3 + 1]; c2 = a.color[q * 3 + 2];
+                const bool heads = !has_bg || inside != 0.0f;
+                c0 = heads ? a.color[q * 3] : 0.0f; c1 = heads ? a.color[q * 3 + 1] : 0.0f; c2 = heads ? a.color[q * 3 + 2] : 0.0f;
                 if (has_bg) {
                     c0 = c0 * inside + a.bg_rgb[qt * 3] * (1.0f - inside);
                     c1 = c1 * inside + a.bg_rgb[qt * 3 + 1] * (1.0f - inside);
diff --git a/vdn-nerf_amd/csrc/train_sdf_color_bf16.hip b/vdn-nerf_amd/csrc/train_sdf_color_bf16.hip
--- a/vdn-nerf_amd/csrc/train_sdf_color_bf16.hip
+++ b/vdn-nerf_amd/csrc/train_sdf_color_bf16.hip
@@ -1,7 +1,7 @@
 #include "k_sdf_fwd2.h"
 
-extern "C" int vdn_sdf_color_train_bf16(const VdnSdfArgs* sa, const void* color_blob, int32_t squeeze_out, void* col_h, void* col_small,
-                                        float* col_out, void* stream_) {
+static int sdf_color_train(const VdnSdfArgs* sa, const void* color_blob, int32_t squeeze_out, void* col_h, void* col_small, float* col_out,
+                           const int32_t* n_color_rows, void* stream_) {
     hipStream_t stream = (hipStream_t)stream_;
     if (sa == nullptr || color_blob == nullptr || sa->blob == nullptr || col_h == nullptr || col_small == nullptr || col_out == nullptr) return -1;
     if (sa->pts != nullptr || !sa->rays_o || !sa->rays_d || !sa->z || sa->n_per_ray <= 0 || sa->z_ld < sa->n_per_ray || sa->sdf_ld < sa->n_per_ray) return -2;
@@ -13,5 +13,17 @@
     ex.col_h = col_h;
     ex.col_small = col_small;
     ex.col_out = col_out;
+    ex.n_col_rows = n_color_rows;
     return vdn::sdf2::launch<3, true, 4, 3>(sa, stream, nullptr, &ex);
 }
+
+extern "C" int vdn_sdf_color_train_bf16(const VdnSdfArgs* sa, const void* color_blob, int32_t squeeze_out, void* col_h, void* col_small,
+                                        float* col_out, void* stream_) {
+    return sdf_color_train(sa, color_blob, squeeze_out, col_h, col_small, col_out, nullptr, stream_);
+}
+
+extern "C" int vdn_sdf_color_train_rows_bf16(const VdnSdfArgs* sa, const void* color_blob, int32_t squeeze_out, void* col_h, void* col_small,
+                                             float* col_out, const int32_t* n_color_rows, void* stream_) {
+    if (n_color_rows == nullptr || sa == nullptr || sa->active_idx == nullptr) return -1;
+    return sdf_color_train(sa, color_blob, squeeze_out, col_h, col_small, col_out, n_color_rows, stream_);
+}
diff --git a/vdn-nerf_amd/csrc/vdn_kernels.h b/vdn-nerf_amd/csrc/vdn_kernels.h
--- a/vdn-nerf_amd/csrc/vdn_kernels.h
+++ b/vdn-nerf_amd/csrc/vdn_kernels.h
@@ -18,6 +18,10 @@
 using SdfRbarArgs = ::VdnSdfRbarArgs;
 using SdfFbarArgs = ::VdnSdfFbarArgs;
 using DwDesc = ::VdnDwDesc;
+struct DwRowCap {
+    const int32_t* rows;
+    int lo, hi;
+};
 using DwFinalizeDesc = ::VdnDwFinalizeDesc;
 using WeightNormBwdDesc = ::VdnWeightNormBwdDesc;
 using CompositeBwdArgs = ::VdnCompositeBwdArgs;
diff --git a/vdn-nerf_amd/dpt_models/renderer.py b/vdn-nerf_amd/dpt_models/renderer.py
--- a/vdn-nerf_amd/dpt_models/renderer.py
+++ b/vdn-nerf_amd/dpt_models/renderer.py
@@ -651,7 +651,7 @@
         inject = t_rand is not None or t_rand_out is not None
         if inject and (t_rand is None or (O > 0 and t_rand_out is None) or perturb <= 0):
             return None
-        key = (background_rgb is not None, float(perturb), inject, switches.signature("train"))
+        key = (background_rgb is not None, float(perturb), inject, switches.signature("train"), bool(eng._heads_inside))
         plans = eng.__dict__.setdefault("_plans", {})
         plan = plans.get(key)
         if plan is None:
diff --git a/vdn-nerf_amd/vdn_hip/train.py b/vdn-nerf_amd/vdn_hip/train.py
--- a/vdn-nerf_amd/vdn_hip/train.py
+++ b/vdn-nerf_amd/vdn_hip/train.py
@@ -223,8 +223,12 @@
         self.dw, self.n_dw, self.wgs = dw, n_dw, wgs
         self.fin, self.n_fin, self.max_m, self.phase1 = fin, n_fin, max_m, phase1
         self.wn, self.n_wn, self.wn_rows = wn, n_wn, wn_rows
+        self.cap = None
 
     def launch_gemm(self, sfx, stream):
+        if self.cap is not None:
+            lib.call("vdn_dw_gemm_rows" + sfx, lib.ptr(self.dw), self.n_dw, self.wgs, lib.ptr(self.cap[0]), self.cap[1], self.cap[2], stream)
+            return
         lib.call("vdn_dw_gemm" + sfx, lib.ptr(self.dw), self.n_dw, self.wgs, stream)
 
     def launch(self, sfx, stream, gemm_event=None, event_stream=None):
@@ -281,6 +285,7 @@
         self._ctx = self._fwd_rays = self._car_dev = self._bwd_train = self._fused_keep = None
         self._pending = self._ray_grads = self._color_fused = self._composite_bwd_done = False
         self._fg_compact = self._bg_compact = False
+        self._heads_inside = True
         self.generation = 0
         self._bwd_warm = False
         self._bwd_args_keep = self.join_hook = self.sdf_probe = self._out_strided = self._clone_slots = None
@@ -309,21 +314,24 @@
         self._out_arena, self._out_slots = fz(n_out), slots
         out = lambda name: self._out_arena[slots[name][0]:slots[name][0] + int(np.prod(slots[name][1]))].view(slots[name][1])
         w["sdf"], w["feat"], w["normals"], w["mid_z"] = fz(P), fs(Pp, 256), out("normals"), out("mid_z")
-        w["fg_active"] = (torch.zeros(P, dtype=torch.int32, device=dev), torch.zeros(1, dtype=torch.int32, device=dev),
-                          torch.zeros(B, dtype=torch.int32, device=dev))
+        self._fg_cnt = torch.zeros(4, dtype=torch.int32, device=dev)
+        w["fg_active"] = (torch.zeros(P, dtype=torch.int32, device=dev), self._fg_cnt[0:1], torch.zeros(2 * B, dtype=torch.int32, device=dev))
+        w["fg_inner"] = self._fg_cnt[1:3]
         w["H"], w["V"], w["PE"] = fs(8, Pp, 256), fs(8, Pp, 256), fs(Pp, 64)
         if self.precision == "fp32":
             w["S"] = fs(8, Pp, 256)
-        w["col_out"], w["col_h"], w["col_small"] = fz(P, 3), fs(4, Pp, 256), fs(Pp, 64)
+        fsz = lambda *shape: torch.zeros(*shape, dtype=sdt, device=dev)
+        w["col_out"], w["col_h"], w["col_small"] = fz(P, 3), fsz(4, Pp, 256), fsz(Pp, 64)
         if self.wdepth:
-            w["vdn_out"], w["vdn_h"], w["vdn_small"] = fz(P, 96), fs(4, Pp, 256), fs(Pp, 64)
+            w["vdn_out"], w["vdn_h"], w["vdn_small"] = fz(P, 96), fsz(4, Pp, 256), fsz(Pp, 64)
         if self.dbc:
-            w["col_extra"] = fs(Pp, 96)
+            w["col_extra"] = fsz(Pp, 96)
         self.relu_mask = self.precision == "bf16" and switches.flag("VDN_RELU_MASK")
         fm = lambda *shape: torch.empty(*shape, dtype=torch.uint8, device=dev) if self.relu_mask else None
-        w["col_mask"] = fm(4, Pp * 32)
+        fmz = lambda *shape: torch.zeros(*shape, dtype=torch.uint8, device=dev) if self.relu_mask else None
+        w["col_mask"] = fmz(4, Pp * 32)
         if self.wdepth:
-            w["vdn_mask"] = fm(4, Pp * 32)
+            w["vdn_mask"] = fmz(4, Pp * 32)
         if O > 0:
             w["z_feed"], w["bg_dists"], w["bg_mid"] = f(B, T), f(B, T), out("bg_mid")
             w["bg_density"], w["bg_rgb"] = torch.zeros(Q, device=dev), torch.zeros(Q, 3, device=dev)
@@ -340,9 +348,9 @@
         w["d_vdn"] = f(P, 96) if self.wdepth else None
         w["feat_scratch"] = f(B * (2 * T + N)) if self.wdepth else None
         w["d_var_partial"], w["d_variance"] = f(B), f(1)
-        w["col_dout"], w["col_dh"] = fs(Pp, 32), fs(4, Pp, 256)
+        w["col_dout"], w["col_dh"] = fsz(Pp, 32), fsz(4, Pp, 256)
         if self.wdepth:
-            w["vdn_dout"], w["vdn_dh"] = fs(Pp, 96), fs(4, Pp, 256)
+            w["vdn_dout"], w["vdn_dh"] = fsz(Pp, 96), fsz(4, Pp, 256)
         w["UB"], w["EX"], w["AB"] = fs(Pp * 2144), fs(8, Pp, 256), fs(Pp * 2336)
         if O > 0:
             w["d_bg_density"], w["d_bg_rgb"] = f(Q), f(Q, 3)
@@ -381,7 +389,7 @@
         self.maps = torch.from_numpy(np.concatenate(all_maps)).to(dev)
         self.slab = torch.empty(max(slab_elems, 1), dtype=torch.float32, device=dev)
         self.colsum = torch.empty(max(cs_elems, 1), dtype=torch.float32, device=dev)
-        self.dw_list_kind = ["bg" if e["net"] == "nerf" else "fg" for e in ent]
+        self.dw_list_kind = ["bg" if e["net"] == "nerf" else ("fg" if e["net"] == "sdf" else "heads") for e in ent]
         p_dev = [(w["bg_active"] if k == "bg" else w["fg_active"])[1].data_ptr() for k in self.dw_list_kind]
         dw, fin = dw_tables(ent, lay, self.nets, prec, self.slab, self.colsum, self.maps, p_dev, float(self.r.sdf_network.scale))
         wn, wn_net = weightnorm_table(self.nets)
@@ -401,6 +409,9 @@
                 own = {e["net"] for e in ent[lo:hi]}
                 self.groups[g] = dw_group(dw, fin, wn, lo, hi, wg, dev, vfin if lo == 0 else None,
                                           [i for i, k in enumerate(wn_net) if k in own], dw_dev)
+                c_lo, c_hi = max(lo, n_sdf) - lo, min(hi, n_heads_end) - lo
+                if c_hi > c_lo:
+                    self.groups[g].cap = (w["fg_inner"][1:2], c_lo, c_hi)
         self._param_ptrs = self._ptr_key()
 
     @property
@@ -464,6 +475,8 @@
             tp = lib.VdnTrainPrepArgs()
             tp.rays_o, tp.rays_d, tp.z, tp.z_out, tp.z_feed = (t.data_ptr() for t in (rays_o, rays_d, z, z_out, w["z_feed"]))
             tp.B, tp.N, tp.T, tp.z_ld, tp.sample_dist, tp.fg_radius = B, N, T, z.stride(0), sample_dist, 1.2
+            if self._fg_compact:
+                tp.fg_inner_radius, tp.fg_n_inner = self._inner_radius(ray_grads), w["fg_inner"].data_ptr()
             if pending_merge is not None:
                 tp.new_z, tp.M_old = pending_merge[0].data_ptr(), pending_merge[1]
             tp.dists, tp.mid_z, tp.bg_dists, tp.bg_mid = (w[k].data_ptr() for k in ("dists", "mid_z", "bg_dists", "bg_mid"))
@@ -481,9 +494,10 @@
                 fa = lib.VdnForegroundActiveArgs()
                 fa.rays_o, fa.rays_d, fa.mid_z, fa.B, fa.N, fa.radius = rays_o.data_ptr(), rays_d.data_ptr(), w["mid_z"].data_ptr(), B, N, 1.2
                 fa.active_idx, fa.n_active, fa.ray_counts = (t.data_ptr() for t in w["fg_active"])
+                fa.inner_radius, fa.n_inner = self._inner_radius(ray_grads), w["fg_inner"].data_ptr()
                 lib.call("vdn_foreground_active", fa, st)
         if not self._fg_compact:
-            w["fg_active"][1].fill_(self.P)
+            self._fg_cnt.fill_(self.P)
         if O > 0:
             if not fused_prep:
                 a = lib.VdnSectionArgs()
@@ -526,7 +540,7 @@
             c.P, c.d_out, c.squeeze_out = self.P, d_out, int(module.squeeze_out)
             if net == "color" and self.dbc:
                 c.extra, c.save_extra = w["vdn_out"].data_ptr(), w["col_extra"].data_ptr()
-            lib.call("vdn_rendernet_fwd" + self.sfx, self._fg(c), st if stream is None else stream)
+            lib.call("vdn_rendernet_fwd" + self.sfx, self._fg_heads(c), st if stream is None else stream)
         if before_heads is not None:
             before_heads()
         vdn_beside = self.wdepth and self._side2 is not None and not self.dbc
@@ -578,6 +592,14 @@
             args.active_idx, args.n_active = self.w["fg_active"][0].data_ptr(), self.w["fg_active"][1].data_ptr()
         return args
 
+    def _fg_heads(self, args):
+        if self._fg_compact:
+            args.active_idx, args.n_active = self.w["fg_active"][0].data_ptr(), self.w["fg_inner"][1:2].data_ptr()
+        return args
+
+    def _inner_radius(self, ray_grads):
+        return 1.0 if (self._heads_inside and not ray_grads) else 1.2
+
     def _fork(self):
         if self._side is not None:
             self._ev_fork.record(lib.current_stream())
@@ -648,6 +670,10 @@
         def launch():
             if fused:
                 cimg = self.nets["color"].img
+                if self._fg_compact:
+                    lib.call("vdn_sdf_color_train_rows_bf16", self._fg(s), lib.ptr(cimg.blobs["c2"]), int(r.color_network.squeeze_out),
+                             lib.ptr(w["col_h"]), lib.ptr(w["col_small"]), lib.ptr(w["col_out"]), lib.ptr(w["fg_inner"][1:2]), _stream())
+                    return
                 lib.call("vdn_sdf_color_train_bf16", self._fg(s), lib.ptr(cimg.blobs["c2"]), int(r.color_network.squeeze_out),
                          lib.ptr(w["col_h"]), lib.ptr(w["col_small"]), lib.ptr(w["col_out"]), _stream())
                 return
@@ -665,7 +691,8 @@
         probe.append((e0, e1, w["fg_active"][1].clone() if self._fg_compact else None))
 
     def _dw_rows(self):
-        n = {"bg": int(self.w["bg_active"][1].item()) if "bg_active" in self.w else 0, "fg": int(self.w["fg_active"][1].item())}
+        cnt = self._fg_cnt.tolist()
+        n = {"bg": int(self.w["bg_active"][1].item()) if "bg_active" in self.w else 0, "fg": cnt[0], "heads": cnt[2]}
         tab = np.frombuffer(self.groups["all"].dw.cpu().numpy().tobytes(), dtype=lib.struct_dtype("VdnDwDesc"))
         return tab, [min(int(d["P"]), n[k]) for d, k in zip(tab, self.dw_list_kind)]
 
@@ -822,7 +849,9 @@
             if rg:
                 b.rays_d, b.n_per_ray, b.acc_pts = rays_d.data_ptr(), self.N, int(accumulate)
                 b.d_pts, b.d_dirs = w["d_pts"].data_ptr(), w["d_dirs"].data_ptr()
-            lib.call("vdn_rendernet_bwd" + self.sfx, self._fg(b), st)
+            if self._fg_compact and not rg:
+                b.n_rows_all = w["fg_active"][1].data_ptr()
+            lib.call("vdn_rendernet_bwd" + self.sfx, self._fg_heads(b), st)
         if rg and self._fg_compact:
             w["d_pts"].zero_()
             w["d_dirs"].zero_()
```

Result: faster. 431,900 rays/s, median of 6 (+2.1%).
